# zju3dv/LoFTR

Measured on AMD Instinct MI355X. Metric: image-pairs/sec @640x480 indoor-ds, higher is better.
Workload: dtype f32; 1 GPU; batch=8 640x480 synthetic grayscale pairs per GPU, indoor_ds dual-softmax (BASELINE configs[1]), full LoFTR.forward = ResNet-FPN backbone (HIP implicit-GEMM / patch convolutions incl. the 7x7 stem) + HIP matching path; weights=seeded random init (no checkpoint on the box), conf_matrix_materialised=True, match_type=dual_softmax, global_batch=8, parallelism=dp1 (pairs sharded; RCCL all-gather of match counts)

## Files before the change

### include/loftr_hip.h

```cpp
#ifndef LOFTR_HIP_H_
#define LOFTR_HIP_H_

#include <stddef.h>
#include <stdint.h>

#ifdef __cplusplus
extern "C" {
#endif

typedef enum {
  LOFTR_OK = 0,
  LOFTR_ERR_BAD_ARG = -1,
  LOFTR_ERR_UNSUPPORTED = -2,
  LOFTR_ERR_WORKSPACE = -3,
  LOFTR_ERR_LAUNCH = -4,
  LOFTR_ERR_NO_DEVICE = -5,
  LOFTR_ERR_COMM = -6,
  LOFTR_ERR_RANGE = -7
} loftr_status;

#define LOFTR_HIP_ABI_VERSION 25

int loftr_hip_abi_version(void);
const char* loftr_hip_status_string(int status);
int loftr_hip_device_check(void);

typedef struct {
  const float* data;
  long sn, sc, sh, sw;
  int H, W;
} loftr_fmap;

int loftr_pos_encode_flatten(const loftr_fmap* feat, const float* pe, int pe_h, int pe_w,
                             float* out, int N, int C, void* stream);

typedef struct {
  const float* q_proj;
  const float* k_proj;
  const float* v_proj;
  const float* merge;
  const float* mlp0;
  const float* mlp2;
  const float* norm1_w;
  const float* norm1_b;
  const float* norm2_w;
  const float* norm2_b;
} loftr_layer_weights;

size_t loftr_encoder_workspace_bytes(int nb, int L, int S, int C);

int loftr_encoder_layer_fwd(const float* x, const float* source, const uint8_t* x_mask,
                            const uint8_t* source_mask, const loftr_layer_weights* w, float* out,
                            int nb, int L, int S, int C, int H, void* ws, size_t ws_bytes,
                            void* stream);

typedef struct {
  float* q_proj; float* k_proj; float* v_proj; float* merge; float* mlp0; float* mlp2;
  float* norm1_w; float* norm1_b; float* norm2_w; float* norm2_b;
} loftr_layer_grads;
size_t loftr_encoder_layer_bwd_workspace_bytes(int nb, int L, int S, int C, int H);
int loftr_encoder_layer_bwd(const float* x, const float* source, const uint8_t* x_mask, const uint8_t* source_mask,
                            const loftr_layer_weights* w, const float* grad_out, float* grad_x, float* grad_source,
                            const loftr_layer_grads* gw, int nb, int L, int S, int C, int H, void* ws, size_t ws_bytes,
                            void* stream);

int loftr_transformer_fwd(float* feat0, float* feat1, const uint8_t* mask0, const uint8_t* mask1,
                          const loftr_layer_weights* layers, const int* layer_is_cross,
                          int n_layers, int N, int L, int S, int C, int H, const void* prepared,
                          size_t prepared_bytes, void* ws, size_t ws_bytes, void* stream);
int loftr_transformer_fwd_padded(float* feat0, float* feat1, const uint8_t* mask0, const uint8_t* mask1,
                                 const loftr_layer_weights* layers, const int* layer_is_cross,
                                 int n_layers, int N, int L, int S, int C, int H, const void* prepared,
                                 size_t prepared_bytes, void* ws, size_t ws_bytes, int skip_padded_tiles, void* stream);
size_t loftr_coarse_plan_bytes(const int* layer_is_cross, int n_layers, int N, int L, int S);
int loftr_coarse_plan_build(const int* layer_is_cross, int n_layers, int N, int L, int S, int order, void* plan,
                            size_t plan_bytes, void* stream);
unsigned loftr_coarse_plan_signature(int n_layers, int N, int L, int S, int order);
int loftr_transformer_fwd_planned(float* feat0, float* feat1, const uint8_t* mask0, const uint8_t* mask1,
                                  const loftr_layer_weights* layers, const int* layer_is_cross,
                                  int n_layers, int N, int L, int S, int C, int H, const void* prepared,
                                  size_t prepared_bytes, void* ws, size_t ws_bytes, const void* plan,
                                  size_t plan_bytes, int plan_order, void* diag, size_t diag_bytes, void* stream);

size_t loftr_transformer_prepared_bytes(int n_layers, int C);
int loftr_transformer_prepare(const loftr_layer_weights* layers, int n_layers, int C, void* prepared,
                              size_t prepared_bytes, void* stream);

typedef struct {
  int N, h0c, w0c, h1c, w1c;
  int C;
  float thr;
  int border_rm;
  float scale;
  const uint8_t* mask0;
  const uint8_t* mask1;
  const float* scale0;
  const float* scale1;
} loftr_coarse_params;

typedef struct {
  int64_t* b_ids;
  int64_t* i_ids;
  int64_t* j_ids;
  float* mconf;
  float* mkpts0_c;
  float* mkpts1_c;
  int32_t* counts;
} loftr_match_out;

size_t loftr_coarse_match_workspace_bytes(int N, int L, int S, int C);

int loftr_coarse_match_dual_softmax(const float* feat_c0, const float* feat_c1,
                                    const loftr_coarse_params* p, float temperature,
                                    float* conf_out, const loftr_match_out* out, void* ws,
                                    size_t ws_bytes, void* stream);

int loftr_coarse_match_sinkhorn(const float* feat_c0, const float* feat_c1,
                                const loftr_coarse_params* p, float bin_score, int iters,
                                int prefilter, float* conf_out, float* assign_out,
                                const loftr_match_out* out, void* ws, size_t ws_bytes,
                                void* stream);


size_t loftr_fine_preprocess_workspace_bytes(int M, int W, int Cf);

int loftr_fine_preprocess(const loftr_fmap* feat_f0, const loftr_fmap* feat_f1,
                          const float* feat_c0, const float* feat_c1, int L, int S, int Cc,
                          const int64_t* b_ids, const int64_t* i_ids, const int64_t* j_ids, int M,
                          int w0c, int w1c, int stride, int W, int Cf,
                          const float* down_w, const float* down_b, const float* merge_w,
                          const float* merge_b, float* out0, float* out1, void* ws,
                          size_t ws_bytes, void* stream);

size_t loftr_fine_preprocess_bwd_workspace_bytes(int M, int W, int Cf, int Cc);
int loftr_fine_preprocess_bwd(const loftr_fmap* feat_f0, const loftr_fmap* feat_f1, const float* feat_c0, const float* feat_c1,
                              int L, int S, int Cc, const int64_t* b_ids, const int64_t* i_ids, const int64_t* j_ids, int M,
                              int w0c, int w1c, int stride, int W, int Cf, const float* down_w, const float* down_b,
                              const float* merge_w, const float* grad_out0, const float* grad_out1, const loftr_fmap* grad_f0,
                              const loftr_fmap* grad_f1, float* grad_c0, float* grad_c1, float* grad_down_w, float* grad_down_b,
                              float* grad_merge_w, float* grad_merge_b, void* ws, size_t ws_bytes, void* stream);

int loftr_pos_encode_flatten_gather(const loftr_fmap* bank, int n_slots, const int32_t* slot_ids, int n,
                                    const float* pe, int pe_h, int pe_w, float* out, int C, void* stream);

int loftr_fine_preprocess_gather(const loftr_fmap* bank_f0, int n_slots0, const int32_t* slot0,
                                 const loftr_fmap* bank_f1, int n_slots1, const int32_t* slot1,
                                 const float* feat_c0, const float* feat_c1, int L, int S, int Cc,
                                 const int64_t* b_ids, const int64_t* i_ids, const int64_t* j_ids, int M,
                                 int w0c, int w1c, int stride, int W, int Cf,
                                 const float* down_w, const float* down_b, const float* merge_w,
                                 const float* merge_b, float* out0, float* out1, void* ws,
                                 size_t ws_bytes, void* stream);

int loftr_window_head(const uint32_t* h_sp0, const uint32_t* h_sp1, int N, int H, int Wm, int Cin,
                      const void* prepared, size_t prepared_bytes, int Cout, const int64_t* b_ids,
                      const int64_t* i_ids, const int64_t* j_ids, int M, int w0c, int w1c, int stride, int W,
                      uint32_t* win0_sp, uint32_t* win1_sp, void* stream);
int loftr_fine_preprocess_window_head(const uint32_t* h_sp0, const uint32_t* h_sp1, int N, int H, int Wm, int Cin,
                                      const void* prepared, size_t prepared_bytes,
                                      const float* feat_c0, const float* feat_c1, int L, int S, int Cc,
                                      const int64_t* b_ids, const int64_t* i_ids, const int64_t* j_ids, int M,
                                      int w0c, int w1c, int stride, int W, int Cf,
                                      const float* down_w, const float* down_b, const float* merge_w,
                                      const float* merge_b, float* out0, float* out1, void* ws, size_t ws_bytes,
                                      void* stream);

int loftr_window_head_first(const uint32_t* t_sp0, const uint32_t* t_sp1, int N, int H, int Wm, int Cin,
                            const void* prepared, size_t prepared_bytes, int Cout, const int64_t* b_ids,
                            const int64_t* i_ids, const int64_t* j_ids, int M, int w0c, int w1c, int stride, int W,
                            uint32_t* nb_sp, void* stream);
int loftr_window_head_last(const uint32_t* nb_sp, int H, int Wm, int Cin, const void* prepared, size_t prepared_bytes,
                           int Cout, const int64_t* b_ids, const int64_t* i_ids, const int64_t* j_ids, int M, int w0c,
                           int w1c, int stride, int W, uint32_t* win0_sp, uint32_t* win1_sp, void* stream);
int loftr_fine_preprocess_window_head2(const uint32_t* t_sp0, const uint32_t* t_sp1, int N, int H, int Wm, int Cin,
                                       const void* prepared0, size_t prepared0_bytes, int Cmid,
                                       const void* prepared1, size_t prepared1_bytes,
                                       const float* feat_c0, const float* feat_c1, int L, int S, int Cc,
                                       const int64_t* b_ids, const int64_t* i_ids, const int64_t* j_ids, int M,
                                       int w0c, int w1c, int stride, int W, int Cf,
                                       const float* down_w, const float* down_b, const float* merge_w,
                                       const float* merge_b, float* out0, float* out1, void* ws, size_t ws_bytes,
                                       uint32_t* nb_sp, void* stream);

int loftr_fine_match(const float* feat_f0, const float* feat_f1, int M, int WW, int C,
                     const float* mkpts1_c, const int64_t* b_ids, float scale,
                     const float* scale1, float* expec_f, float* mkpts1_f, void* stream);

size_t loftr_conv_workspace_bytes(int Cin, int Cout, int KH, int KW);
int loftr_conv_bn_act(const uint32_t* x_sp, int B, int H, int W, int Cin, const float* weight,
                      const long* weight_strides, int Cout, int KH, int KW, int stride, int pad, const float* bn_weight, const float* bn_bias,
                      const float* bn_mean, const float* bn_var, float bn_eps, int act,
                      const uint32_t* residual_sp, uint32_t* y_sp, float* y_f32, void* ws, size_t ws_bytes,
                      const float* x_inv_scale, void* stream);
int loftr_conv_prepare(const float* weight, const long* weight_strides, int Cin, int Cout, int KH, int KW,
                       const float* bn_weight, const float* bn_bias, const float* bn_mean, const float* bn_var,
                       float bn_eps, void* prepared, size_t prepared_bytes, void* stream);
#define LOFTR_CONV_SHARED_GPU 0x100
int loftr_conv_bn_act_prepared(const uint32_t* x_sp, int B, int H, int W, int Cin, const void* prepared,
                               size_t prepared_bytes, int Cout, int KH, int KW, int stride, int pad, int act,
                               const uint32_t* residual_sp, const uint32_t* low_sp, uint32_t* y_sp, float* y_f32,
                               const float* x_inv_scale, void* stream);
size_t loftr_conv_scratch_bytes(int B, int H, int W, int Cout, int KH, int KW, int stride);
int loftr_conv_bn_act_prepared_scratch(const uint32_t* x_sp, int B, int H, int W, int Cin, const void* prepared,
                                       size_t prepared_bytes, int Cout, int KH, int KW, int stride, int pad, int act,
                                       const uint32_t* residual_sp, const uint32_t* low_sp, uint32_t* y_sp, float* y_f32,
                                       const float* x_inv_scale, void* scratch, size_t scratch_bytes, void* stream);
int loftr_stem_conv_bn_relu(const float* x, const long* x_strides, int B, int H, int W, const float* weight,
                            const long* weight_strides, int C0, const float* bn_weight, const float* bn_bias,
                            const float* bn_mean, const float* bn_var, float bn_eps, uint32_t* y_sp, void* stream);
int loftr_upsample2x_add(const uint32_t* low_sp, const uint32_t* lateral_sp, uint32_t* out_sp, int B, int Hl,
                         int Wl, int C, void* stream);
int loftr_conv1x1_upsample_add(const uint32_t* x_sp, int B, int H, int W, int Cin, const float* weight,
                               const long* weight_strides, int Cout, const uint32_t* low_sp, uint32_t* y_sp,
                               void* ws, size_t ws_bytes, void* stream);
int loftr_sp_from_f32(const float* src, uint32_t* dst_sp, long rows, int C, void* stream);
int loftr_sp_from_f32_scaled(const float* src, uint32_t* dst_sp, long rows, int C, float* inv_scale_out, void* stream);
int loftr_sp_to_f32(const uint32_t* src_sp, float* dst, long rows, int C, void* stream);

int loftr_epipolar_errors(const float* mkpts0_f, const float* mkpts1_f, const long* m_bids, const float* T_0to1,
                          const float* K0, const float* K1, long M, int N, float* epi_errs, void* stream);

typedef struct {
  int N, H0, W0, H1, W1, scale;
  int dh0, dw0, dh1, dw1;
  const float* depth0; const float* depth1;
  const float* T_0to1; const float* T_1to0;
  const float* K0; const float* K1;
  const float* scale0; const float* scale1;
  const uint8_t* mask0; const uint8_t* mask1;
} loftr_spvs_params;
size_t loftr_spvs_coarse_workspace_bytes(int N, int L, int S);
int loftr_spvs_coarse(const loftr_spvs_params* p, float* w_pt0_i, float* pt1_i, int64_t* spv_b, int64_t* spv_i, int64_t* spv_j,
                      int32_t* count, float* conf_gt, void* ws, size_t ws_bytes, void* stream);
int loftr_spvs_fine(const float* w_pt0_i, const float* pt1_i, int L, int S, const int64_t* b_ids, const int64_t* i_ids,
                    const int64_t* j_ids, long M, float scale, float radius, const float* scale1, float* expec_f_gt, void* stream);
size_t loftr_loss_workspace_bytes(int N, int L, int S);
int loftr_coarse_loss_sums(const float* conf, int N, int L, int S, int kind, const int64_t* gt_b, const int64_t* gt_i,
                           const int64_t* gt_j, long M, const uint8_t* mask0, const uint8_t* mask1, float alpha, float gamma,
                           double* sums, void* ws, size_t ws_bytes, void* stream);
int loftr_fine_loss_sums(const float* expec_f, int ld, const float* expec_f_gt, long M, int with_std, float correct_thr,
                         double* sums, void* ws, size_t ws_bytes, void* stream);

int loftr_coarse_loss_grad(const float* conf, int N, int L, int S, int kind, const int64_t* gt_b, const int64_t* gt_i,
                           const int64_t* gt_j, long M, const uint8_t* mask0, const uint8_t* mask1, float alpha, float gamma,
                           double pos_scale, double neg_scale, float* grad_conf, void* ws, size_t ws_bytes, void* stream);
int loftr_fine_loss_grad(const float* expec_f, int ld, const float* expec_f_gt, long M, int with_std, float correct_thr,
                         int training, const double* sums, float upstream, float* grad_expec, void* stream);
int loftr_dual_softmax_bwd(const float* feat_c0, const float* feat_c1, const loftr_coarse_params* p, float temperature,
                           const float* grad_conf, float* dsim, void* ws, size_t ws_bytes, void* stream);
int loftr_fine_match_bwd(const float* feat_f0, const float* feat_f1, int M, int WW, int C, const float* grad_expec,
                         float* grad_f0, float* grad_f1, void* stream);
int loftr_head_feat_grads(const float* dsim, long dsim_ld, long dsim_bs, const float* feat_c0, const float* feat_c1,
                          int N, int L, int S, int C, float alpha, float* g0, float* g1, void* stream);
size_t loftr_conv_wgrad_workspace_bytes(int B, int Ho, int Wo, int Cin, int Cout, int KH, int KW);
int loftr_conv_wgrad(const float* dy, const float* x, int B, int H, int W, int Cin, int Cout, int KH, int KW, int stride, int pad,
                     float* dw_taps, void* ws, size_t ws_bytes, void* stream);
size_t loftr_sinkhorn_bwd_workspace_bytes(int N, int L, int S, int C, int iters);
int loftr_sinkhorn_bwd(const float* feat_c0, const float* feat_c1, const loftr_coarse_params* p, float bin_score, int iters,
                       const float* grad_assign, float* z_scratch, float* dZ, float* dbin, void* ws, size_t ws_bytes, void* stream);

int loftr_estimate_pose(const float* kpts0, const float* kpts1, long M, const float* K0, const float* K1, float thresh_px,
                        float conf, unsigned seed, float* R_out, float* t_out, uint8_t* inliers_out, long* n_inliers);
int loftr_five_point(const double* q0, const double* q1, int n, double* E_out, int* n_solutions);

size_t loftr_estimate_pose_batched_workspace_bytes(long M, int P);
int loftr_estimate_pose_batched(const float* mkpts0_f, const float* mkpts1_f, const long* m_bids, long M, const float* K0,
                                const float* K1, int P, float thresh_px, float conf, unsigned seed, float* R_out, float* t_out,
                                uint8_t* inliers_out, long* n_inliers, void* ws, size_t ws_bytes, void* stream);

int loftr_estimate_geometry(const float* kpts0, const float* kpts1, long M, int model, float thresh_px, float conf, unsigned seed,
                            float* mat_out, uint8_t* inliers_out, long* n_inliers);
int loftr_geometry_minimal(const double* p0, const double* p1, int model, double* mats_out, int* n_solutions);

size_t loftr_estimate_geometry_batched_workspace_bytes(long M, int P, int model);
int loftr_estimate_geometry_batched(const float* mkpts0_f, const float* mkpts1_f, const long* m_bids, long M, int P, int model,
                                    float thresh_px, float conf, unsigned seed, float* mat_out, uint8_t* inliers_out,
                                    long* n_inliers, void* ws, size_t ws_bytes, void* stream);

int loftr_estimate_absolute_pose(const float* pts3d, const float* kpts, long M, const float* K, float thresh_px, float conf, unsigned seed,
                                 float* R_out, float* t_out, uint8_t* inliers_out, long* n_inliers);
int loftr_p3p(const double* X, const double* bearings, double* R_out, double* t_out, int* n_solutions);

size_t loftr_estimate_absolute_pose_batched_workspace_bytes(long M, int P);
int loftr_estimate_absolute_pose_batched(const float* pts3d, const float* kpts, const long* m_bids, long M, const float* K, int P,
                                         float thresh_px, float conf, unsigned seed, float* R_out, float* t_out, uint8_t* inliers_out,
                                         long* n_inliers, void* ws, size_t ws_bytes, void* stream);

int loftr_lift_keypoints(const float* kpts, const long* m_bids, long M, const float* depth, int dh, int dw, const float* K, const float* T,
                         int P, float* pts3d_out, uint8_t* valid_out, void* stream);

typedef struct {
  long* kp_offsets; float* keypoints; float* score; int* n_obs;
  long* row_offsets; int* matches; float* match_conf;
  int* track_id; int* track_len; uint8_t* track_ok; long* counts;
} LoftrAtlasOut;

int loftr_atlas_host(const float* kpts0, const float* kpts1, const float* conf, const int* rows, const uint8_t* mask, long M,
                     const int* row_images, long R, int n_images, int gh, int gw, float inv, int min_track_len, const LoftrAtlasOut* out);

int loftr_atlas_observe(const float* kpts0, const float* kpts1, const float* conf, const long* m_bids, const uint8_t* mask, long n,
                        int n_rows, long match_base, long row_base, const int* row_images, int n_images, int gh, int gw, float inv,
                        unsigned long long* grid, float* obs_xy, int* obs_cell, float* m_conf, int* m_row, uint8_t* m_reason, int* status,
                        void* stream);

#define LOFTR_ATLAS_STAGES 7
size_t loftr_atlas_finalize_workspace_bytes(long M, int n_images, int gh, int gw);
int loftr_atlas_finalize(unsigned long long* grid, const float* obs_xy, const int* obs_cell, const float* m_conf, const int* m_row,
                         const uint8_t* m_reason, long M, long R, int n_images, int gh, int gw, int min_track_len, const int* status,
                         const LoftrAtlasOut* out, void* ws, size_t ws_bytes, float* stage_ms, void* stream);

int loftr_triangulate_tracks_host(const long* offsets, long T, const int* obs_image, const float* obs_xy, long N, const double* K,
                                  const double* T_cam_from_world, int n_images, double thresh_px, double cos_min_angle, float* xyz,
                                  int* n_inliers, float* rms_px, float* tri_cos, uint8_t* status, uint8_t* obs_inlier, long* counts);
int loftr_triangulation_pairs(int L, int* pairs, int* n);
#define LOFTR_TRIANGULATE_STAGES 3
size_t loftr_triangulate_tracks_workspace_bytes(long T, long N, int n_images);
int loftr_triangulate_tracks(const long* offsets, long T, const int* obs_image, const float* obs_xy, long N, const double* K,
                             const double* T_cam_from_world, int n_images, double thresh_px, double cos_min_angle, float* xyz,
                             int* n_inliers, float* rms_px, float* tri_cos, uint8_t* status, uint8_t* obs_inlier, long* counts, int group,
                             void* ws, size_t ws_bytes, float* stage_ms, void* stream);

typedef struct {
  const long* kp_offsets; const int* kp_cell; const int* kp_point; const float* xyz;
  long K, P;
  int n_images, gh, gw;
  float inv;
} LoftrModel;
typedef struct {
  float* pts3d; float* kpts; long* q_ids; int* match; int* point; float* conf;
  long* q_offsets; uint8_t* match_reason; long* counts;
} LoftrModelLookupOut;

int loftr_model_cells_host(const long* kp_offsets, int n_images, const float* keypoints, const int* kp_point, long K, long P, int gh, int gw,
                           float inv, int* kp_cell, int* status);
int loftr_model_cells(const long* kp_offsets, int n_images, const float* keypoints, const int* kp_point, long K, long P, int gh, int gw,
                      float inv, int* kp_cell, int* status, void* stream);

int loftr_model_lookup_host(const LoftrModel* model, const float* kpts_db, const float* kpts_q, const float* conf, const int* rows,
                            const uint8_t* mask, long M, const int* row_db, const int* row_query, long R, long Q,
                            const LoftrModelLookupOut* out);
#define LOFTR_MODEL_LOOKUP_STAGES 3
size_t loftr_model_lookup_workspace_bytes(long M, long Q);
int loftr_model_lookup(const LoftrModel* model, const float* kpts_db, const float* kpts_q, const float* conf, const int* rows,
                       const uint8_t* mask, long M, const int* row_db, const int* row_query, long R, long Q, const LoftrModelLookupOut* out,
                       void* ws, size_t ws_bytes, float* stage_ms, void* stream);

#define LOFTR_BUNDLE_MAX_ITERS 1000
#define LOFTR_BUNDLE_MAX_PCG 200
int loftr_bundle_adjust_host(const long* offsets, long T, const int* obs_image, const float* obs_xy, const uint8_t* obs_mask, long N,
                             const float* xyz, const double* K, const double* T_cam_from_world, const uint8_t* fixed, int n_images,
                             const long* cam_offsets, const int* cam_obs, double huber_px, int max_iters, int pcg_iters, double pcg_tol,
                             double ftol, double* T_out, float* xyz_out, uint8_t* obs_active, uint8_t* cam_free, uint8_t* point_active,
                             long* counts);
#define LOFTR_BUNDLE_CLASSES 11
size_t loftr_bundle_adjust_workspace_bytes(long T, long N, int n_images);
int loftr_bundle_adjust(const long* offsets, long T, const int* obs_image, const float* obs_xy, const uint8_t* obs_mask, long N,
                        const float* xyz, const double* K, const double* T_cam_from_world, const uint8_t* fixed, int n_images,
                        const long* cam_offsets, const int* cam_obs, double huber_px, int max_iters, int pcg_iters, double pcg_tol,
                        double ftol, double* T_out, float* xyz_out, uint8_t* obs_active, uint8_t* cam_free, uint8_t* point_active,
                        long* counts, void* ws, size_t ws_bytes, float* class_ms, long* class_launches, void* stream);

int loftr_register_corr_host(const long* offsets, long T, const int* obs_image, const float* obs_xy, long N, const float* xyz,
                             const uint8_t* status, const uint8_t* posed, int n_images, const long* cam_offsets, const int* cam_obs,
                             int min_corr, int* n_corr, int* cand_rank, int* cand_image, long* cand_offsets, float* corr_xyz, float* corr_xy,
                             long* corr_bid, int* corr_obs, long* counts);
#define LOFTR_REGISTER_STAGES 4
#define LOFTR_REGISTER_RANK_BLOCK 256
size_t loftr_register_corr_workspace_bytes(long T, long N, int n_images);
int loftr_register_corr(const long* offsets, long T, const int* obs_image, const float* obs_xy, long N, const float* xyz,
                        const uint8_t* status, const uint8_t* posed, int n_images, const long* cam_offsets, const int* cam_obs,
                        int min_corr, int* n_corr, int* cand_rank, int* cand_image, long* cand_offsets, float* corr_xyz, float* corr_xy,
                        long* corr_bid, int* corr_obs, long* counts, void* ws, size_t ws_bytes, float* stage_ms, void* stream);

size_t loftr_bn_train_workspace_bytes(int N, int C, long HW);
int loftr_bn_train_fwd(const float* x, int N, int C, long HW, int channels_last, const float* gamma, const float* beta, float eps, float* y,
                       float* mean, float* invstd, float* var_unbiased, void* ws, size_t ws_bytes, void* stream);
int loftr_bn_train_bwd(const float* dy, const float* x, int N, int C, long HW, int channels_last, const float* mean, const float* invstd,
                       const float* gamma, float* dx, float* dgamma, float* dbeta, void* ws, size_t ws_bytes, void* stream);
int loftr_act_fwd(const float* a, const float* b, long n, int act, float slope, float* y, void* stream);
int loftr_act_bwd(const float* dy, const float* y, long n, int act, float slope, float* dx, void* stream);
int loftr_upsample2x_bilinear_fwd(const float* x, int N, int C, int H, int W, int channels_last, float* y, void* stream);
int loftr_upsample2x_bilinear_bwd(const float* dy, int N, int C, int H, int W, int channels_last, float* dx, void* stream);

int loftr_resize_linear_u8(const uint8_t* src, int sh, int sw, long src_pitch, uint8_t* dst, int dh, int dw,
                           long dst_pitch, void* stream);
// ... 29 lines not shown
```

### loftr_amd/_lib.py

```python
import ctypes as C
import os

HERE = os.path.dirname(os.path.abspath(__file__))
LIB_PATH = os.environ.get("LOFTR_HIP_LIB") or os.path.join(HERE, "libloftr_hip.so")

_p = C.c_void_p
_i = C.c_int
_f = C.c_float
_sz = C.c_size_t
_l = C.c_long


class LayerWeights(C.Structure):
    _fields_ = [(n, _p) for n in ("q_proj", "k_proj", "v_proj", "merge", "mlp0", "mlp2",
                                  "norm1_w", "norm1_b", "norm2_w", "norm2_b")]


class CoarseParams(C.Structure):
    _fields_ = [("N", _i), ("h0c", _i), ("w0c", _i), ("h1c", _i), ("w1c", _i), ("C", _i),
                ("thr", _f), ("border_rm", _i), ("scale", _f),
                ("mask0", _p), ("mask1", _p), ("scale0", _p), ("scale1", _p)]


class MatchOut(C.Structure):
    _fields_ = [(n, _p) for n in ("b_ids", "i_ids", "j_ids", "mconf", "mkpts0_c", "mkpts1_c", "counts")]


class SpvsParams(C.Structure):
    _fields_ = [(n, _i) for n in ("N", "H0", "W0", "H1", "W1", "scale", "dh0", "dw0", "dh1", "dw1")] + \
               [(n, _p) for n in ("depth0", "depth1", "T_0to1", "T_1to0", "K0", "K1", "scale0", "scale1", "mask0", "mask1")]


class FMap(C.Structure):
    _fields_ = [("data", _p), ("sn", _l), ("sc", _l), ("sh", _l), ("sw", _l), ("H", _i), ("W", _i)]


class AtlasOut(C.Structure):
    _fields_ = [(n, _p) for n in ("kp_offsets", "keypoints", "score", "n_obs", "row_offsets", "matches", "match_conf",
                                  "track_id", "track_len", "track_ok", "counts")]


class Model(C.Structure):
    _fields_ = [(n, _p) for n in ("kp_offsets", "kp_cell", "kp_point", "xyz")] + [("K", _l), ("P", _l), ("n_images", _i), ("gh", _i), ("gw", _i),
                                                                                   ("inv", _f)]


class ModelLookupOut(C.Structure):
    _fields_ = [(n, _p) for n in ("pts3d", "kpts", "q_ids", "match", "point", "conf", "q_offsets", "match_reason", "counts")]


SIGNATURES = {
    "loftr_hip_abi_version": (_i, []),
    "loftr_hip_status_string": (C.c_char_p, [_i]),
    "loftr_hip_device_check": (_i, []),
    "loftr_pos_encode_flatten": (_i, [C.POINTER(FMap), _p, _i, _i, _p, _i, _i, _p]),
    "loftr_encoder_workspace_bytes": (_sz, [_i, _i, _i, _i]),
    "loftr_encoder_layer_fwd": (_i, [_p, _p, _p, _p, C.POINTER(LayerWeights), _p, _i, _i, _i, _i, _i, _p, _sz, _p]),
    "loftr_encoder_layer_bwd_workspace_bytes": (_sz, [_i, _i, _i, _i, _i]),
    "loftr_encoder_layer_bwd": (_i, [_p, _p, _p, _p, C.POINTER(LayerWeights), _p, _p, _p, C.POINTER(LayerWeights), _i, _i, _i, _i, _i, _p, _sz, _p]),
    "loftr_transformer_fwd": (_i, [_p, _p, _p, _p, C.POINTER(LayerWeights), C.POINTER(_i), _i, _i, _i, _i, _i, _i,
                                   _p, _sz, _p, _sz, _p]),
    "loftr_transformer_fwd_padded": (_i, [_p, _p, _p, _p, C.POINTER(LayerWeights), C.POINTER(_i), _i, _i, _i, _i, _i, _i,
                                          _p, _sz, _p, _sz, _i, _p]),
    "loftr_coarse_plan_bytes": (_sz, [C.POINTER(_i), _i, _i, _i, _i]),
    "loftr_coarse_plan_build": (_i, [C.POINTER(_i), _i, _i, _i, _i, _i, _p, _sz, _p]),
    "loftr_coarse_plan_signature": (C.c_uint, [_i, _i, _i, _i, _i]),
    "loftr_transformer_fwd_planned": (_i, [_p, _p, _p, _p, C.POINTER(LayerWeights), C.POINTER(_i), _i, _i, _i, _i, _i, _i,
                                           _p, _sz, _p, _sz, _p, _sz, _i, _p, _sz, _p]),
    "loftr_hip_debug_set": (_i, [C.c_char_p, _i]),
    "loftr_hip_debug_get": (_i, [C.c_char_p, C.POINTER(_i), C.POINTER(_i)]),
    "loftr_transformer_prepared_bytes": (_sz, [_i, _i]),
    "loftr_transformer_prepare": (_i, [C.POINTER(LayerWeights), _i, _i, _p, _sz, _p]),
    "loftr_coarse_match_workspace_bytes": (_sz, [_i, _i, _i, _i]),
    "loftr_coarse_match_dual_softmax": (_i, [_p, _p, C.POINTER(CoarseParams), _f, _p, C.POINTER(MatchOut), _p, _sz, _p]),
    "loftr_coarse_match_sinkhorn": (_i, [_p, _p, C.POINTER(CoarseParams), _f, _i, _i, _p, _p, C.POINTER(MatchOut),
                                         _p, _sz, _p]),
    "loftr_fine_preprocess_workspace_bytes": (_sz, [_i, _i, _i]),
    "loftr_fine_preprocess": (_i, [C.POINTER(FMap), C.POINTER(FMap), _p, _p, _i, _i, _i, _p, _p, _p, _i, _i, _i, _i,
                                   _i, _i, _p, _p, _p, _p, _p, _p, _p, _sz, _p]),
    "loftr_fine_preprocess_bwd_workspace_bytes": (_sz, [_i, _i, _i, _i]),
    "loftr_fine_preprocess_bwd": (_i, [C.POINTER(FMap), C.POINTER(FMap), _p, _p, _i, _i, _i, _p, _p, _p, _i, _i, _i, _i, _i, _i,
                                       _p, _p, _p, _p, _p, C.POINTER(FMap), C.POINTER(FMap), _p, _p, _p, _p, _p, _p, _p, _sz, _p]),
    "loftr_fine_match": (_i, [_p, _p, _i, _i, _i, _p, _p, _f, _p, _p, _p, _p]),
    "loftr_pos_encode_flatten_gather": (_i, [C.POINTER(FMap), _i, _p, _i, _p, _i, _i, _p, _i, _p]),
    "loftr_fine_preprocess_gather": (_i, [C.POINTER(FMap), _i, _p, C.POINTER(FMap), _i, _p, _p, _p, _i, _i, _i, _p, _p, _p, _i, _i, _i, _i,
                                          _i, _i, _p, _p, _p, _p, _p, _p, _p, _sz, _p]),
    "loftr_window_head": (_i, [_p, _p, _i, _i, _i, _i, _p, _sz, _i, _p, _p, _p, _i, _i, _i, _i, _i, _p, _p, _p]),
    "loftr_fine_preprocess_window_head": (_i, [_p, _p, _i, _i, _i, _i, _p, _sz, _p, _p, _i, _i, _i, _p, _p, _p, _i, _i, _i, _i,
                                               _i, _i, _p, _p, _p, _p, _p, _p, _p, _sz, _p]),
    "loftr_window_head_first": (_i, [_p, _p, _i, _i, _i, _i, _p, _sz, _i, _p, _p, _p, _i, _i, _i, _i, _i, _p, _p]),
    "loftr_window_head_last": (_i, [_p, _i, _i, _i, _p, _sz, _i, _p, _p, _p, _i, _i, _i, _i, _i, _p, _p, _p]),
    "loftr_fine_preprocess_window_head2": (_i, [_p, _p, _i, _i, _i, _i, _p, _sz, _i, _p, _sz, _p, _p, _i, _i, _i, _p, _p, _p, _i, _i, _i,
                                                _i, _i, _i, _p, _p, _p, _p, _p, _p, _p, _sz, _p, _p]),
    "loftr_conv_workspace_bytes": (_sz, [_i, _i, _i, _i]),
    "loftr_conv_bn_act": (_i, [_p, _i, _i, _i, _i, _p, C.POINTER(_l), _i, _i, _i, _i, _i, _p, _p, _p, _p, _f, _i, _p, _p, _p, _p, _sz, _p, _p]),
    "loftr_stem_conv_bn_relu": (_i, [_p, C.POINTER(_l), _i, _i, _i, _p, C.POINTER(_l), _i, _p, _p, _p, _p, _f, _p, _p]),
    "loftr_upsample2x_add": (_i, [_p, _p, _p, _i, _i, _i, _i, _p]),
    "loftr_bn_train_workspace_bytes": (_sz, [_i, _i, _l]),
    "loftr_bn_train_fwd": (_i, [_p, _i, _i, _l, _i, _p, _p, _f, _p, _p, _p, _p, _p, _sz, _p]),
    "loftr_bn_train_bwd": (_i, [_p, _p, _i, _i, _l, _i, _p, _p, _p, _p, _p, _p, _p, _sz, _p]),
    "loftr_act_fwd": (_i, [_p, _p, _l, _i, _f, _p, _p]),
    "loftr_act_bwd": (_i, [_p, _p, _l, _i, _f, _p, _p]),
    "loftr_upsample2x_bilinear_fwd": (_i, [_p, _i, _i, _i, _i, _i, _p, _p]),
    "loftr_upsample2x_bilinear_bwd": (_i, [_p, _i, _i, _i, _i, _i, _p, _p]),
    "loftr_resize_linear_u8": (_i, [_p, _i, _i, _l, _p, _i, _i, _l, _p]),
    "loftr_pack_gray_u8": (_i, [_p, _l, _l, _p, _i, _i, _i, _p, _p, _p, _i, _p]),
    "loftr_epipolar_errors": (_i, [_p, _p, _p, _p, _p, _p, _l, _i, _p, _p]),
    "loftr_spvs_coarse_workspace_bytes": (_sz, [_i, _i, _i]),
    "loftr_spvs_coarse": (_i, [C.POINTER(SpvsParams), _p, _p, _p, _p, _p, _p, _p, _p, _sz, _p]),
    "loftr_spvs_fine": (_i, [_p, _p, _i, _i, _p, _p, _p, _l, _f, _f, _p, _p, _p]),
    "loftr_loss_workspace_bytes": (_sz, [_i, _i, _i]),
    "loftr_coarse_loss_sums": (_i, [_p, _i, _i, _i, _i, _p, _p, _p, _l, _p, _p, _f, _f, _p, _p, _sz, _p]),
    "loftr_fine_loss_sums": (_i, [_p, _i, _p, _l, _i, _f, _p, _p, _sz, _p]),
    "loftr_coarse_loss_grad": (_i, [_p, _i, _i, _i, _i, _p, _p, _p, _l, _p, _p, _f, _f, C.c_double, C.c_double, _p, _p, _sz, _p]),
    "loftr_conv_wgrad_workspace_bytes": (_sz, [_i, _i, _i, _i, _i, _i, _i]),
    "loftr_conv_wgrad": (_i, [_p, _p, _i, _i, _i, _i, _i, _i, _i, _i, _i, _p, _p, _sz, _p]),
    "loftr_head_feat_grads": (_i, [_p, C.c_long, C.c_long, _p, _p, _i, _i, _i, _i, _f, _p, _p, _p]),
    "loftr_sinkhorn_bwd_workspace_bytes": (_sz, [_i, _i, _i, _i, _i]),
    "loftr_sinkhorn_bwd": (_i, [_p, _p, C.POINTER(CoarseParams), _f, _i, _p, _p, _p, _p, _p, _sz, _p]),
    "loftr_fine_loss_grad": (_i, [_p, _i, _p, _l, _i, _f, _i, _p, _f, _p, _p]),
    "loftr_dual_softmax_bwd": (_i, [_p, _p, C.POINTER(CoarseParams), _f, _p, _p, _p, _sz, _p]),
    "loftr_fine_match_bwd": (_i, [_p, _p, _i, _i, _i, _p, _p, _p, _p]),
    "loftr_estimate_pose": (_i, [_p, _p, _l, _p, _p, _f, _f, C.c_uint, _p, _p, _p, C.POINTER(_l)]),
    "loftr_five_point": (_i, [_p, _p, _i, _p, C.POINTER(_i)]),
    "loftr_estimate_pose_batched_workspace_bytes": (_sz, [_l, _i]),
    "loftr_estimate_pose_batched": (_i, [_p, _p, _p, _l, _p, _p, _i, _f, _f, C.c_uint, _p, _p, _p, _p, _p, _sz, _p]),
    "loftr_estimate_geometry": (_i, [_p, _p, _l, _i, _f, _f, C.c_uint, _p, _p, C.POINTER(_l)]),
    "loftr_geometry_minimal": (_i, [_p, _p, _i, _p, C.POINTER(_i)]),
    "loftr_estimate_geometry_batched_workspace_bytes": (_sz, [_l, _i, _i]),
    "loftr_estimate_geometry_batched": (_i, [_p, _p, _p, _l, _i, _i, _f, _f, C.c_uint, _p, _p, _p, _p, _sz, _p]),
    "loftr_estimate_absolute_pose": (_i, [_p, _p, _l, _p, _f, _f, C.c_uint, _p, _p, _p, C.POINTER(_l)]),
    "loftr_p3p": (_i, [_p, _p, _p, _p, C.POINTER(_i)]),
    "loftr_estimate_absolute_pose_batched_workspace_bytes": (_sz, [_l, _i]),
    "loftr_estimate_absolute_pose_batched": (_i, [_p, _p, _p, _l, _p, _i, _f, _f, C.c_uint, _p, _p, _p, _p, _p, _sz, _p]),
    "loftr_lift_keypoints": (_i, [_p, _p, _l, _p, _i, _i, _p, _p, _i, _p, _p, _p]),
    "loftr_atlas_host": (_i, [_p, _p, _p, _p, _p, _l, _p, _l, _i, _i, _i, _f, _i, C.POINTER(AtlasOut)]),
    "loftr_atlas_observe": (_i, [_p, _p, _p, _p, _p, _l, _i, _l, _l, _p, _i, _i, _i, _f, _p, _p, _p, _p, _p, _p, _p, _p]),
    "loftr_atlas_finalize_workspace_bytes": (_sz, [_l, _i, _i, _i]),
    "loftr_atlas_finalize": (_i, [_p, _p, _p, _p, _p, _p, _l, _l, _i, _i, _i, _i, _p, C.POINTER(AtlasOut), _p, _sz, _p, _p]),
    "loftr_triangulate_tracks_host": (_i, [_p, _l, _p, _p, _l, _p, _p, _i, C.c_double, C.c_double, _p, _p, _p, _p, _p, _p, _p]),
    "loftr_triangulation_pairs": (_i, [_i, _p, C.POINTER(_i)]),
    "loftr_triangulate_tracks_workspace_bytes": (_sz, [_l, _l, _i]),
    "loftr_triangulate_tracks": (_i, [_p, _l, _p, _p, _l, _p, _p, _i, C.c_double, C.c_double, _p, _p, _p, _p, _p, _p, _p, _i, _p, _sz, _p, _p]),
    "loftr_model_cells_host": (_i, [_p, _i, _p, _p, _l, _l, _i, _i, _f, _p, _p]),
    "loftr_model_cells": (_i, [_p, _i, _p, _p, _l, _l, _i, _i, _f, _p, _p, _p]),
    "loftr_model_lookup_host": (_i, [C.POINTER(Model), _p, _p, _p, _p, _p, _l, _p, _p, _l, _l, C.POINTER(ModelLookupOut)]),
    "loftr_model_lookup_workspace_bytes": (_sz, [_l, _l]),
    "loftr_model_lookup": (_i, [C.POINTER(Model), _p, _p, _p, _p, _p, _l, _p, _p, _l, _l, C.POINTER(ModelLookupOut), _p, _sz, _p, _p]),
    "loftr_bundle_adjust_host": (_i, [_p, _l, _p, _p, _p, _l, _p, _p, _p, _p, _i, _p, _p, C.c_double, _i, _i, C.c_double, C.c_double,
                                      _p, _p, _p, _p, _p, _p]),
    "loftr_bundle_adjust_workspace_bytes": (_sz, [_l, _l, _i]),
    "loftr_bundle_adjust": (_i, [_p, _l, _p, _p, _p, _l, _p, _p, _p, _p, _i, _p, _p, C.c_double, _i, _i, C.c_double, C.c_double,
                                 _p, _p, _p, _p, _p, _p, _p, _sz, _p, _p, _p]),
    "loftr_register_corr_host": (_i, [_p, _l, _p, _p, _l, _p, _p, _p, _i, _p, _p, _i, _p, _p, _p, _p, _p, _p, _p, _p, _p]),
    "loftr_register_corr_workspace_bytes": (_sz, [_l, _l, _i]),
    "loftr_register_corr": (_i, [_p, _l, _p, _p, _l, _p, _p, _p, _i, _p, _p, _i, _p, _p, _p, _p, _p, _p, _p, _p, _p, _p, _sz, _p, _p]),
    "loftr_conv_prepare": (_i, [_p, C.POINTER(_l), _i, _i, _i, _i, _p, _p, _p, _p, _f, _p, _sz, _p]),
    "loftr_conv_bn_act_prepared": (_i, [_p, _i, _i, _i, _i, _p, _sz, _i, _i, _i, _i, _i, _i, _p, _p, _p, _p, _p, _p]),
    "loftr_conv_scratch_bytes": (_sz, [_i, _i, _i, _i, _i, _i, _i]),
    "loftr_conv_bn_act_prepared_scratch": (_i, [_p, _i, _i, _i, _i, _p, _sz, _i, _i, _i, _i, _i, _i, _p, _p, _p, _p, _p, _p, _sz, _p]),
    "loftr_conv1x1_upsample_add": (_i, [_p, _i, _i, _i, _i, _p, C.POINTER(_l), _i, _p, _p, _p, _sz, _p]),
    "loftr_sp_from_f32": (_i, [_p, _p, _l, _i, _p]),
    "loftr_sp_from_f32_scaled": (_i, [_p, _p, _l, _i, _p, _p]),
    "loftr_sp_to_f32": (_i, [_p, _p, _l, _i, _p]),
    "loftr_rccl_unique_id": (_i, [C.c_char_p, _sz]),
    "loftr_rccl_comm_create": (_i, [C.c_char_p, _sz, _i, _i, C.POINTER(_p)]),
    "loftr_rccl_comm_info": (_i, [_p, C.POINTER(_i), C.POINTER(_i)]),
    "loftr_rccl_comm_destroy": (_i, [_p]),
    "loftr_rccl_allgather_counts": (_i, [_p, _p, _p, _i, _p]),
    "loftr_hip_timing_enable": (_i, [C.c_uint]),
    "loftr_hip_range_check_enable": (_i, [_i]),
    "loftr_hip_timing_kernel_count": (_i, []),
    "loftr_hip_timing_kernel_name": (C.c_char_p, [_i]),
    "loftr_hip_timing_read": (_i, [_i, C.POINTER(C.c_double), C.POINTER(C.c_longlong), _i]),
    "loftr_linear_workspace_bytes": (_sz, [_i, _i, _i]),
    "loftr_linear_fwd": (_i, [_p, _p, _p, _i, _i, _i, _p, _sz, _p]),
}

ABI_VERSION = 25
_lib = None


class LoftrHipError(RuntimeError):
    pass


def load():
    global _lib
    if _lib is not None:
        return _lib
    if not os.path.exists(LIB_PATH):
        raise LoftrHipError(
            f"{LIB_PATH} not found: the HIP extension is not built. Run `python -m loftr_amd.build` "
            "(needs hipcc). There is no CPU / PyTorch fallback for the matching path.")
    lib = C.CDLL(LIB_PATH)
    for name, (res, args) in SIGNATURES.items():
        fn = getattr(lib, name, None)
        if fn is None:
            raise LoftrHipError(f"{LIB_PATH} does not export {name}: it predates this binding; rebuild "
                                "(`python -m loftr_amd.build --force`)")
        fn.restype = res
        fn.argtypes = args
    if lib.loftr_hip_abi_version() != ABI_VERSION:
        raise LoftrHipError(f"ABI mismatch: library {lib.loftr_hip_abi_version()} != binding {ABI_VERSION}; rebuild")
    _lib = lib
    return lib


def check(status, what=""):
    if status != 0:
        msg = load().loftr_hip_status_string(status).decode()
        raise LoftrHipError(f"{what or 'libloftr_hip'} failed: {msg} (status {status})")
```

### loftr_amd/csrc/coarse_plan.h

```cpp
#pragma once
#include "gemm.h"

struct PctItem { uint32_t what; uint32_t signal; uint32_t dep[4]; uint32_t sig2[2]; };
constexpr uint32_t PCT_NODEP = 0xffffffffu;
constexpr int PCT_X = 0, PCT_K = 1, PCT_F = 2;
constexpr int PCT_MAX_LAYERS = 8, PCT_MAX_CALLS = 2 * PCT_MAX_LAYERS, PCT_TILE = 128, PCT_CNT0 = 4;
constexpr int PCT_MAX_PAIRS = 256, PCT_MAX_TILES = 4095;

struct PctShape {
  int n_layers, N, T[2];
  int n_calls() const { return 2 * n_layers; }
  int tiles(int img) const { return (T[img] + PCT_TILE - 1) / PCT_TILE; }
  int gmax() const { return tiles(0) > tiles(1) ? tiles(0) : tiles(1); }
  uint32_t xflag(int c, int p, int g) const { return (uint32_t)(PCT_CNT0 + (c * N + p) * gmax() + g); }
  uint32_t kcnt(int c, int p) const { return (uint32_t)(PCT_CNT0 + n_calls() * N * gmax() + c * N + p); }
  uint32_t fcnt(int c, int p) const { return kcnt(c, p) + (uint32_t)(n_calls() * N); }
  size_t n_counters() const { return (size_t)PCT_CNT0 + (size_t)n_calls() * N * (gmax() + 2); }
  void call(int c, int& layer, int& x_img, int& s_img) const {
    const int i = c / 4, k = c % 4;
    layer = 2 * i + (k >= 2); x_img = k & 1; s_img = k < 2 ? (k & 1) : 1 - (k & 1);
  }
  bool standalone_k(int c) const { return c < 2; }
  int folds(int c, int (&out)[2]) const {
    const int k = c % 4;
    int n = 0;
    if (k == 1) out[n++] = c + 1;
    if (k == 2) { out[n++] = c + 1; if (c + 2 < n_calls()) out[n++] = c + 2; }
    if (k == 3 && c + 2 < n_calls()) out[n++] = c + 2;
    for (int i = n; i < 2; ++i) out[i] = -1;
    return n;
  }
  size_t n_items() const {
    size_t n = 0;
    for (int c = 0; c < n_calls(); ++c) { int l, x, s; call(c, l, x, s); n += (size_t)N * ((standalone_k(c) ? tiles(s) : 0) + 8 + tiles(x)); }
    return n;
  }
  uint32_t signature(int order) const {
    uint32_t h = 0x9e3779b9u ^ 7u;
    for (uint32_t v : {(uint32_t)n_layers, (uint32_t)N, (uint32_t)T[0], (uint32_t)T[1], (uint32_t)order}) h = (h ^ v) * 0x01000193u + 0x7ed55d16u;
    return h | 1u;
  }
  bool ok() const {
    return n_layers >= 2 && n_layers % 2 == 0 && n_layers <= PCT_MAX_LAYERS && N >= 1 && N <= PCT_MAX_PAIRS && T[0] >= 1 && T[1] >= 1 &&
           gmax() <= PCT_MAX_TILES && n_counters() < (1u << 20);
  }
};
inline size_t pct_plan_bytes(const PctShape& s) { return (1 + s.n_items()) * sizeof(PctItem); }
inline size_t pct_ws_bytes(const PctShape& s) {
  const size_t cp = (size_t)s.n_calls() * s.N;
  return align_up(s.n_counters() * 4, 256) + align_up(cp * 8 * s.gmax() * 33 * 32 * 4, 256) + align_up(cp * 8 * 33 * 32 * 4, 256) +
         align_up(cp * 65536 * 4, 256) + 1024;
}

struct PctLayerPtrs {
  const sp_t *wq, *w0, *w2, *wkv;
  const float *wq_s, *w0_s, *w2_s, *wkv_s, *merge_f32, *g1, *b1, *g2, *b2;
};
struct PctLaunch {
  PctShape shape;
  float* f32[2]; sp_t* sp[2]; const uint8_t* mask[2];
  PctLayerPtrs layer[PCT_MAX_LAYERS];
  const void* plan; size_t plan_bytes; unsigned plan_signature;
  void* ws; size_t ws_bytes;
  unsigned* status;
  unsigned long long* trace;
};
int launch_coarse_persistent(const PctLaunch& p, hipStream_t st);
```

### loftr_amd/csrc/encoder_fused.hip

```cpp
#include "linear.h"
#include "attention.h"
#include "coarse_plan.h"

namespace {
namespace efx {
#ifndef EFX_NST
#define EFX_NST 4
#endif
#ifndef EFX_PROBE_DMA
#define EFX_PROBE_DMA 1
#endif
#ifndef EFX_PROBE_BARRIER
#define EFX_PROBE_BARRIER 1
#endif
#ifndef EFX_PROBE_EPI
#define EFX_PROBE_EPI 1
#endif
constexpr int W = 4, PT = 32, STAGE = 32 * 1024, NST = EFX_NST, BLK = 4096;
constexpr int NPANEL = 16 + 48;
constexpr int DMA_PER_WAVE = 8;
constexpr int T_WQS = 0, T_KSUM = 256, T_G1 = 512, T_B1 = 768, T_W0S = 1024, T_W2S = 1536, T_G2 = 1792, T_B2 = 2048, T_N = 2304;
constexpr int OFF_TAB = NST * STAGE;
constexpr int LDS_BYTES = OFF_TAB + T_N * 4;
static_assert(LDS_BYTES <= 160 * 1024, "one workgroup per CU");

struct Args {
  const sp_t* x_sp; const float* x_f32;
  float* out_f32; sp_t* out_sp;
  const sp_t* wq; const sp_t* pm; long pm_seq_stride;
  const sp_t* w0; const sp_t* w2;
  const float *wq_s, *w0_s, *w2_s;
  const float* kv;
  const uint8_t* mask;
  const float *g1, *b1, *g2, *b2;
  float v_length, attn_eps, p_out_scale, ln_eps;
  int nseq, T, groups;
  int xsplit, gpc;
  int skip_padded;
};

typedef __attribute__((address_space(3))) void* lds_ptr_t;
typedef const __attribute__((address_space(1))) void* gbl_ptr_t;

__device__ __forceinline__ void swap_halves(uint32_t& a, uint32_t& b) {
  const auto r = __builtin_amdgcn_permlane32_swap(a, b, false, false);
  a = r[0]; b = r[1];
}
__device__ __forceinline__ void sp_pack4(float x0, float x1, float x2, float x3, uint2& hi, uint2& lo) {
  sp_pack2(x0, x1, hi.x, lo.x);
  sp_pack2(x2, x3, hi.y, lo.y);
}
__device__ __forceinline__ void pack_panel(const float (&v)[16], h16x8 (&fh)[2], h16x8 (&fl)[2]) {
  if (!EFX_PROBE_EPI) {
    fh[0] = __builtin_bit_cast(h16x8, f32x4{v[0], v[1], v[2], v[3]}); fl[0] = __builtin_bit_cast(h16x8, f32x4{v[4], v[5], v[6], v[7]});
    fh[1] = __builtin_bit_cast(h16x8, f32x4{v[8], v[9], v[10], v[11]}); fl[1] = __builtin_bit_cast(h16x8, f32x4{v[12], v[13], v[14], v[15]});
    return;
  }
  uint2 H[4], L[4];
#pragma unroll
  for (int q = 0; q < 4; ++q) sp_pack4(v[4 * q], v[4 * q + 1], v[4 * q + 2], v[4 * q + 3], H[q], L[q]);
#pragma unroll
  for (int s = 0; s < 2; ++s) {
    swap_halves(H[2 * s].x, H[2 * s + 1].x); swap_halves(H[2 * s].y, H[2 * s + 1].y);
    swap_halves(L[2 * s].x, L[2 * s + 1].x); swap_halves(L[2 * s].y, L[2 * s + 1].y);
    fh[s] = __builtin_bit_cast(h16x8, u32x4{H[2 * s].x, H[2 * s].y, H[2 * s + 1].x, H[2 * s + 1].y});
    fl[s] = __builtin_bit_cast(h16x8, u32x4{L[2 * s].x, L[2 * s].y, L[2 * s + 1].x, L[2 * s + 1].y});
  }
}

__device__ __forceinline__ const sp_t* uniform_ptr(const sp_t* p) {
  const unsigned long long v = (unsigned long long)(size_t)p;
  const unsigned lo = (unsigned)__builtin_amdgcn_readfirstlane((int)(unsigned)v), hi = (unsigned)__builtin_amdgcn_readfirstlane((int)(unsigned)(v >> 32));
  return reinterpret_cast<const sp_t*>((size_t)(((unsigned long long)hi << 32) | lo));
}

__device__ __forceinline__ bool job_tile(const Args& a, const int id, int& seq, int& grp) {
  const int xcd = id % NUM_XCD, slot = id / NUM_XCD;
  const int vs = (slot / a.gpc) * NUM_XCD + xcd;
  seq = vs / a.xsplit; grp = (slot % a.gpc) * a.xsplit + vs % a.xsplit;
  return seq < a.nseq && grp < a.groups;
}

struct KvTile {
  const sp_t* x_sp; const uint8_t* mask; int T;
  const sp_t* wkv; const float* wkv_s;
  float inv_s;
  float* part; long head_stride;
};
struct FoldArgs { int n; KvTile k[2]; };
__device__ __forceinline__ void kv_tile_main(const KvTile& a, char* const lds, const h16x8 (&xh)[16], const h16x8 (&xl)[16],
                                             const float (&mk)[16], const bool live, const int nlive);

template <bool FOLD>
__device__ __forceinline__ void encoder_x_body(const Args& a, const int seq, const int grp, char* const lds, const FoldArgs* fa = nullptr) {
  const int lane = threadIdx.x & 63, wave = threadIdx.x >> 6, g = lane >> 5, li = lane & 31;
  const int T = a.T;
  if constexpr (!FOLD) {
    if (a.skip_padded && a.mask && a.out_f32 == a.x_f32 && a.out_sp == a.x_sp) {
      const int t = grp * W * PT + (int)threadIdx.x;
      const bool valid = (int)threadIdx.x < W * PT && t < T && a.mask[(long)seq * T + t] != 0;
      if (!__syncthreads_or(valid)) return;
    }
  }
  const int tok = (grp * W + wave) * PT + li;
  const bool live = (grp * W + wave) * PT < T;
  const long row = (long)seq * T + min(tok, T - 1);
  float* tab = reinterpret_cast<float*>(lds + OFF_TAB);

  for (int f = threadIdx.x; f < 256; f += W * 64) {
    tab[T_WQS + f] = a.wq_s[f];
    tab[T_KSUM + f] = a.kv[((long)seq * 8 + (f >> 5)) * (33 * 32) + 32 * 32 + (f & 31)];
    tab[T_G1 + f] = a.g1[f]; tab[T_B1 + f] = a.b1[f];
    tab[T_W0S + f] = a.w0_s[f]; tab[T_W0S + 256 + f] = a.w0_s[256 + f];
    tab[T_W2S + f] = a.w2_s[f];
    tab[T_G2 + f] = a.g2[f]; tab[T_B2 + f] = a.b2[f];
  }
  h16x8 xh[16], xl[16];
  {
    const u32x4* src = reinterpret_cast<const u32x4*>(a.x_sp + row * 256);
#pragma unroll
    for (int ks = 0; ks < 16; ++ks) {
      const int c = (ks >> 1) * 8 + 2 * (ks & 1) + g;
      xh[ks] = __builtin_bit_cast(h16x8, src[c]);
      xl[ks] = __builtin_bit_cast(h16x8, src[c + 4]);
    }
  }
  const float mk = (a.mask && !a.mask[row]) ? 0.f : 1.f;

  const sp_t* pm = a.pm + (long)seq * a.pm_seq_stride;
  unsigned doff[4];
#pragma unroll
  for (int oct = 0; oct < 4; ++oct) doff[oct] = ((unsigned)(oct * 8 + (lane >> 3)) * 256u + ((((unsigned)lane & 7u) ^ ((unsigned)(oct * 4 + (lane >> 4)) & 7u)) << 2)) * 4u;
  const unsigned drl = (unsigned)(lane >> 3) * 1024u;
  const int wave_s = __builtin_amdgcn_readfirstlane(wave);
#define EFX_ISSUE_SRC(p_, base_, pitch_, kt_)                                                              \
  {                                                                                                        \
    char* st__ = lds + ((p_) % NST) * STAGE;                                                               \
    const unsigned w512__ = (pitch_) == 512 ? 1u : 0u;                                                     \
    _Pragma("unroll") for (int bi__ = 0; bi__ < 2; ++bi__) {                                               \
      const int b__ = wave_s + 4 * bi__;                                                                   \
      const char* bb__ = reinterpret_cast<const char*>(uniform_ptr((kt_) ? (base_) + (long)b__ * 32 * (pitch_) : (base_) + b__ * 32)); \
      _Pragma("unroll") for (int oct__ = 0; oct__ < 4; ++oct__) {                                          \
        const char* bo__ = bb__ + (size_t)(w512__ * (unsigned)(oct__ * 8192));                             \
        asm volatile("" : "+s"(bo__));                   \
        __builtin_amdgcn_global_load_lds((gbl_ptr_t)(bo__ + (doff[oct__] + w512__ * drl)),                 \
                                         (lds_ptr_t)(st__ + b__ * BLK + oct__ * 1024), 16, 0, 0);          \
      }                                                                                                    \
    }                                                                                                      \
  }
#define EFX_ISSUE(p_)                                                                                      \
  {                                                                                                        \
    const int p__ = (p_);                                                                                  \
    const sp_t* base__; int pitch__; bool kt__;                                                            \
    if (p__ < 16) {                                                                                        \
      const int h__ = p__ >> 1;                                                                            \
      if (p__ & 1) { base__ = pm + h__ * 32; pitch__ = 256; kt__ = true; }                                 \
      else { base__ = a.wq + (long)h__ * 32 * 256; pitch__ = 256; kt__ = false; }                          \
    } else {                                                                                               \
      const int q__ = p__ - 16, hp__ = q__ / 3, i__ = q__ - 3 * hp__;                                      \
      if (i__ == 2) { base__ = a.w2 + hp__ * 32; pitch__ = 512; kt__ = true; }                             \
      else { base__ = a.w0 + (long)hp__ * 32 * 512 + i__ * 256; pitch__ = 512; kt__ = false; }             \
    }                                                                                                      \
    EFX_ISSUE_SRC(p__, base__, pitch__, kt__)                                                              \
  }
#define EFX_BEGIN_G(p_, NP_, ISSUE_)                                                                       \
  {                                                                                                        \
    if (!EFX_PROBE_DMA) LOFTR_WAITCNT_VM(0);                                                               \
    else if (NST >= 4 && (p_) + 2 < (NP_)) LOFTR_WAITCNT_VM(2 * DMA_PER_WAVE);                             \
    else if ((p_) + 1 < (NP_)) LOFTR_WAITCNT_VM(DMA_PER_WAVE);                                             \
    else LOFTR_WAITCNT_VM(0);                                                                              \
    if (EFX_PROBE_BARRIER) __builtin_amdgcn_s_barrier();                                                   \
    if (EFX_PROBE_DMA && (p_) + NST - 1 < (NP_)) ISSUE_((p_) + NST - 1);                                   \
  }
#define EFX_BEGIN(p_) EFX_BEGIN_G(p_, NPANEL, EFX_ISSUE)
  const int a_off = lds_chunk_off(li, g);
#define EFX_RD(st_, blk_, odd_, lo_) (*reinterpret_cast<const h16x8*>((st_) + (blk_) * BLK + (a_off ^ (((odd_) ? 32 : 0) | ((lo_) ? 64 : 0)))))
#define EFX_USE(a_, b_, c_, d_) asm volatile("" :: "v"(a_), "v"(b_), "v"(c_), "v"(d_))
#define EFX_RPANEL_G(st_, bh_, bl_, MF_)                                                                   \
  {                                                                                                        \
    h16x8 eh__ = EFX_RD(st_, 0, 0, 0), el__ = EFX_RD(st_, 0, 0, 1), oh__ = EFX_RD(st_, 0, 1, 0), ol__ = EFX_RD(st_, 0, 1, 1);\
    _Pragma("unroll") for (int u = 0; u < 8; ++u) {                                                        \
      EFX_USE(eh__, el__, oh__, ol__);                                                                     \
      __builtin_amdgcn_sched_barrier(0);                                                                   \
      h16x8 neh__ = eh__, nel__ = el__, noh__ = oh__, nol__ = ol__;                                        \
      acc0 = MF_(eh__, bl_[2 * u], acc0);                                                                  \
      __builtin_amdgcn_sched_barrier(0);                                                                   \
      if (u + 1 < 8) { neh__ = EFX_RD(st_, u + 1, 0, 0); nel__ = EFX_RD(st_, u + 1, 0, 1); }               \
      __builtin_amdgcn_sched_barrier(0);                                                                   \
      acc0 = MF_(el__, bh_[2 * u], acc0);                                                                  \
      __builtin_amdgcn_sched_barrier(0);                                                                   \
      if (u + 1 < 8) { noh__ = EFX_RD(st_, u + 1, 1, 0); nol__ = EFX_RD(st_, u + 1, 1, 1); }               \
      __builtin_amdgcn_sched_barrier(0);                                                                   \
      acc0 = MF_(eh__, bh_[2 * u], acc0);                                                                  \
      acc0 = MF_(oh__, bl_[2 * u + 1], acc0);                                                              \
      acc0 = MF_(ol__, bh_[2 * u + 1], acc0);                                                              \
      acc0 = MF_(oh__, bh_[2 * u + 1], acc0);                                                              \
      __builtin_amdgcn_sched_barrier(0);                                                                   \
      eh__ = neh__; el__ = nel__; oh__ = noh__; ol__ = nol__;                                              \
    }                                                                                                      \
  }
#define EFX_MF_N(w_, x_, c_) __builtin_amdgcn_mfma_f32_32x32x16_f16(w_, x_, c_, 0, 0, 0)
#define EFX_MF_T(w_, x_, c_) __builtin_amdgcn_mfma_f32_32x32x16_f16(x_, w_, c_, 0, 0, 0)
#define EFX_RPANEL(st_, bh_, bl_) EFX_RPANEL_G(st_, bh_, bl_, EFX_MF_N)
#define EFX_KPANEL(st_, fh_, fl_, out_)                                                                    \
  {                                                                                                        \
    h16x8 ah__ = EFX_RD(st_, 0, 0, 0), al__ = EFX_RD(st_, 0, 0, 1), bh__ = EFX_RD(st_, 1, 0, 0), bl__ = EFX_RD(st_, 1, 0, 1); \
    _Pragma("unroll") for (int u = 0; u < 8; ++u) {                                                        \
      const int j2 = u >> 1, s = u & 1;                                                                    \
      const int nj = (u + 1) >> 1, ns = (u + 1) & 1;                                                       \
      EFX_USE(ah__, al__, bh__, bl__);                                                                     \
      __builtin_amdgcn_sched_barrier(0);                                                                   \
      h16x8 nah__ = ah__, nal__ = al__, nbh__ = bh__, nbl__ = bl__;                                        \
      out_[2 * j2] = __builtin_amdgcn_mfma_f32_32x32x16_f16(ah__, fl_[s], out_[2 * j2], 0, 0, 0);          \
      __builtin_amdgcn_sched_barrier(0);                                                                   \
      if (u + 1 < 8) { nah__ = EFX_RD(st_, 2 * nj, ns, 0); nal__ = EFX_RD(st_, 2 * nj, ns, 1); }           \
      __builtin_amdgcn_sched_barrier(0);                                                                   \
      out_[2 * j2 + 1] = __builtin_amdgcn_mfma_f32_32x32x16_f16(bh__, fl_[s], out_[2 * j2 + 1], 0, 0, 0);  \
      __builtin_amdgcn_sched_barrier(0);                                                                   \
      if (u + 1 < 8) { nbh__ = EFX_RD(st_, 2 * nj + 1, ns, 0); nbl__ = EFX_RD(st_, 2 * nj + 1, ns, 1); }   \
      __builtin_amdgcn_sched_barrier(0);                                                                   \
      out_[2 * j2] = __builtin_amdgcn_mfma_f32_32x32x16_f16(al__, fh_[s], out_[2 * j2], 0, 0, 0);          \
      out_[2 * j2 + 1] = __builtin_amdgcn_mfma_f32_32x32x16_f16(bl__, fh_[s], out_[2 * j2 + 1], 0, 0, 0);  \
      out_[2 * j2] = __builtin_amdgcn_mfma_f32_32x32x16_f16(ah__, fh_[s], out_[2 * j2], 0, 0, 0);          \
      out_[2 * j2 + 1] = __builtin_amdgcn_mfma_f32_32x32x16_f16(bh__, fh_[s], out_[2 * j2 + 1], 0, 0, 0);  \
      __builtin_amdgcn_sched_barrier(0);                                                                   \
      ah__ = nah__; al__ = nal__; bh__ = nbh__; bl__ = nbl__;                                              \
    }                                                                                                      \
  }

  LOFTR_WAITCNT_VM(0);
  __syncthreads();
  EFX_ISSUE(0);
  EFX_ISSUE(1);
  if (NST >= 4) EFX_ISSUE(2);

  const int fq = 4 * g;
  f32x16 acc0;
  f32x16 big[8];
#pragma unroll
  for (int j = 0; j < 8; ++j)
#pragma unroll
    for (int r = 0; r < 16; ++r) big[j][r] = 0.f;

#pragma unroll 1
  for (int h = 0; h < 8; ++h) {
    const int p = 2 * h;
    EFX_BEGIN(p);
    h16x8 qh[2], ql[2];
    if (live) {
      const char* st = lds + (p % NST) * STAGE;
#pragma unroll
      for (int r = 0; r < 16; ++r) acc0[r] = 0.f;
      EFX_RPANEL(st, xh, xl);
      float v[16];
      float den = 0.f;
#pragma unroll
      for (int q = 0; q < 4; ++q) {
        const f32x4 ws = *reinterpret_cast<const f32x4*>(tab + T_WQS + 32 * h + fq + 8 * q);
        const f32x4 ks4 = *reinterpret_cast<const f32x4*>(tab + T_KSUM + 32 * h + fq + 8 * q);
#pragma unroll
        for (int e = 0; e < 4; ++e) {
          float x = acc0[4 * q + e] * ws[e];
          if (EFX_PROBE_EPI) x = x > 0.f ? x + 1.f : __expf(x);
          x *= mk;
          v[4 * q + e] = x;
          den = fmaf(x, ks4[e], den);
        }
      }
      den += swap32(den);
      const float z = den == 0.f ? 0.f : a.v_length * __builtin_amdgcn_rcpf(den + a.attn_eps);
#pragma unroll
      for (int r = 0; r < 16; ++r) v[r] *= z;
      pack_panel(v, qh, ql);
    }
    EFX_BEGIN(p + 1);
    if (live) {
      const char* st = lds + ((p + 1) % NST) * STAGE;
      EFX_KPANEL(st, qh, ql, big);
    }
  }
  h16x8 mh[16], ml[16];
  if (live) {
    const float ps = a.p_out_scale;
    float s = 0.f;
#pragma unroll
    for (int j = 0; j < 8; ++j)
#pragma unroll
      for (int r = 0; r < 16; ++r) s += big[j][r];
    s += swap32(s);
    const float mean_a = s * (1.f / 256.f);
    float m2 = 0.f;
#pragma unroll
    for (int j = 0; j < 8; ++j)
#pragma unroll
      for (int r = 0; r < 16; ++r) { const float d = big[j][r] - mean_a; m2 = fmaf(d, d, m2); }
    m2 += swap32(m2);
    const float rstd = ps * rsqrtf(ps * ps * m2 * (1.f / 256.f) + a.ln_eps);
    const float mean = mean_a;
#pragma unroll
    for (int j = 0; j < 8; ++j) {
      float y[16];
#pragma unroll
      for (int q = 0; q < 4; ++q) {
        const f32x4 ga = *reinterpret_cast<const f32x4*>(tab + T_G1 + 32 * j + fq + 8 * q);
        const f32x4 be = *reinterpret_cast<const f32x4*>(tab + T_B1 + 32 * j + fq + 8 * q);
#pragma unroll
        for (int e = 0; e < 4; ++e) y[4 * q + e] = (big[j][4 * q + e] - mean) * rstd * ga[e] + be[e];
      }
      h16x8 fh[2], fl[2];
      pack_panel(y, fh, fl);
      mh[2 * j] = fh[0]; mh[2 * j + 1] = fh[1]; ml[2 * j] = fl[0]; ml[2 * j + 1] = fl[1];
    }
  }
#pragma unroll
  for (int j = 0; j < 8; ++j)
#pragma unroll
    for (int r = 0; r < 16; ++r) big[j][r] = 0.f;

#define EFX_PASS2_HEAD(hp_)                                                                                \
    const int p = 16 + 3 * (hp_);                                                                          \
    h16x8 hh[2], hl[2];                                                                                    \
    EFX_BEGIN(p);                                                                                          \
    if (live) {                                                                                            \
      _Pragma("unroll") for (int r = 0; r < 16; ++r) acc0[r] = 0.f;                     \
      EFX_RPANEL(lds + (p % NST) * STAGE, xh, xl);                                                                 \
    }                                                                                                      \
    EFX_BEGIN(p + 1);                                                                                      \
    if (live) {                                                                                            \
      EFX_RPANEL(lds + ((p + 1) % NST) * STAGE, mh, ml);                                                                 \
      float v[16];                                                                                         \
      _Pragma("unroll") for (int q = 0; q < 4; ++q) {                                                      \
        const f32x4 ws = *reinterpret_cast<const f32x4*>(tab + T_W0S + 32 * (hp_) + fq + 8 * q);           \
        _Pragma("unroll") for (int e = 0; e < 4; ++e)                                                      \
          v[4 * q + e] = fmaxf(acc0[4 * q + e] * ws[e], 0.f);    \
      }                                                                                                    \
      pack_panel(v, hh, hl);                                                                               \
    }                                                                                                      \
    EFX_BEGIN(p + 2);
#pragma unroll 1
  for (int hp = 0; hp < 16; ++hp) {
    EFX_PASS2_HEAD(hp)
    if (live) EFX_KPANEL(lds + ((p + 2) % NST) * STAGE, hh, hl, big);
  }
#undef EFX_PASS2_HEAD

  if (!FOLD && !live) return;
  if (live) {
    float s = 0.f;
#pragma unroll
    for (int j = 0; j < 8; ++j)
#pragma unroll
      for (int q = 0; q < 4; ++q) {
        const f32x4 ws = *reinterpret_cast<const f32x4*>(tab + T_W2S + 32 * j + fq + 8 * q);
#pragma unroll
        for (int e = 0; e < 4; ++e) s = fmaf(big[j][4 * q + e], ws[e], s);
      }
    s += swap32(s);
    const float mean = s * (1.f / 256.f);
    float m2 = 0.f;
    asm volatile("" ::: "memory");
#pragma unroll
    for (int j = 0; j < 8; ++j)
#pragma unroll
      for (int q = 0; q < 4; ++q) {
        const f32x4 ws = *reinterpret_cast<const f32x4*>(tab + T_W2S + 32 * j + fq + 8 * q);
#pragma unroll
        for (int e = 0; e < 4; ++e) { const float d = big[j][4 * q + e] * ws[e] - mean; m2 = fmaf(d, d, m2); }
      }
    m2 += swap32(m2);
    const float rstd = rsqrtf(m2 * (1.f / 256.f) + a.ln_eps);
    asm volatile("" ::: "memory");
    const bool in_seq = tok < T;
    if (FOLD || in_seq) {
      const float* xr = a.x_f32 + row * 256;
      float* of = a.out_f32 + row * 256;
      sp_t* os = a.out_sp + row * 256;
      f32x4 xn[4];
#pragma unroll
      for (int q = 0; q < 4; ++q) xn[q] = *reinterpret_cast<const f32x4*>(xr + fq + 8 * q);
#pragma unroll
      for (int j = 0; j < 8; ++j) {
        f32x4 xc[4];
#pragma unroll
        for (int q = 0; q < 4; ++q) xc[q] = xn[q];
        if (j + 1 < 8) {
#pragma unroll
          for (int q = 0; q < 4; ++q) xn[q] = *reinterpret_cast<const f32x4*>(xr + 32 * (j + 1) + fq + 8 * q);
        }
        float y[16];
#pragma unroll
        for (int q = 0; q < 4; ++q) {
          const int f = 32 * j + fq + 8 * q;
          const f32x4 ga = *reinterpret_cast<const f32x4*>(tab + T_G2 + f);
          const f32x4 be = *reinterpret_cast<const f32x4*>(tab + T_B2 + f);
          const f32x4 ws = *reinterpret_cast<const f32x4*>(tab + T_W2S + f);
          f32x4 o;
#pragma unroll
          for (int e = 0; e < 4; ++e) {
            o[e] = xc[q][e] + ((big[j][4 * q + e] * ws[e] - mean) * rstd * ga[e] + be[e]);
            y[4 * q + e] = o[e];
          }
          if (!FOLD || in_seq) *reinterpret_cast<f32x4*>(of + f) = o;
        }
        if (!FOLD && !a.out_sp) continue;
        h16x8 fh[2], fl[2];
        pack_panel(y, fh, fl);
        if (FOLD) { xh[2 * j] = fh[0]; xh[2 * j + 1] = fh[1]; xl[2 * j] = fl[0]; xl[2 * j + 1] = fl[1]; }
        if (!FOLD || in_seq) {
#pragma unroll
          for (int s2 = 0; s2 < 2; ++s2) {
            *reinterpret_cast<u32x4*>(os + j * 32 + (2 * s2 + g) * 4) = __builtin_bit_cast(u32x4, fh[s2]);
            *reinterpret_cast<u32x4*>(os + j * 32 + 16 + (2 * s2 + g) * 4) = __builtin_bit_cast(u32x4, fl[s2]);
          }
        }
      }
    }
  }
  if constexpr (FOLD) {
    if (fa->n > 0) {
      const int tok0 = (grp * W + wave) * PT;
      const int nlive = min(W, (T - grp * W * PT + PT - 1) / PT);
      float mk[16];
#pragma unroll
      for (int r = 0; r < 16; ++r) {
        const int t = tok0 + (r & 3) + 8 * (r >> 2) + 4 * g;
        mk[r] = (t < T && (!a.mask || a.mask[(long)seq * T + min(t, T - 1)])) ? 1.f : 0.f;
      }
#pragma unroll 1
      for (int s = 0; s < fa->n; ++s) kv_tile_main(fa->k[s], lds, xh, xl, mk, live, nlive);
    }
  }
}

__global__ __launch_bounds__(W * 64, 1) void encoder_x_kernel(Args a) {
  __shared__ __attribute__((aligned(16))) char lds[LDS_BYTES];
  int seq, grp;
  if (job_tile(a, blockIdx.x, seq, grp)) encoder_x_body<false>(a, seq, grp, lds);
}

struct Args2 { Args j[2]; int n0, off0, off1; };
__global__ __launch_bounds__(W * 64, 1) void encoder_x2_kernel(Args2 m) {
  __shared__ __attribute__((aligned(16))) char lds[LDS_BYTES];
  const bool second = (int)blockIdx.x >= m.n0;
  const Args* a = second ? &m.j[1] : &m.j[0];
  int seq, grp;
  if (job_tile(*a, second ? (int)blockIdx.x - m.n0 + m.off1 : (int)blockIdx.x + m.off0, seq, grp)) encoder_x_body<false>(*a, seq, grp, lds);
}

struct PctCall { int layer, x_img, s_img, pad, fold[2], pad2[2]; };
struct PctArgs {
  float* f32[2]; sp_t* sp[2]; const uint8_t* mask[2]; int T[2];
  int N, n_calls, n_items, splits;
  const PctItem* items; unsigned* cnt;
  float* part; float* kv; sp_t* pm;
  unsigned long long* trace;
  unsigned* status;
  unsigned signature; int skip;
  int quota;
  PctLayerPtrs layer[PCT_MAX_LAYERS]; PctCall call[PCT_MAX_CALLS];
};
constexpr int OFF_RED = OFF_TAB + T_N * 4, RED_FLOATS = 33 * 32, OFF_CTRL = OFF_RED + W * RED_FLOATS * 4, LDS_BYTES_P = OFF_CTRL + 64;
static_assert(LDS_BYTES_P <= 160 * 1024, "one workgroup per CU");

__device__ __forceinline__ void kv_tile_body(const KvTile& a, const int tile, char* const lds) {
  const int lane = threadIdx.x & 63, wave = threadIdx.x >> 6, g = lane >> 5, li = lane & 31;
  const int T = a.T;
  const int tok0 = (tile * W + wave) * PT;
  const bool live = tok0 < T;
  const int nlive = min(W, (T - tile * W * PT + PT - 1) / PT);
  h16x8 xh[16], xl[16];
  {
    const u32x4* src = reinterpret_cast<const u32x4*>(a.x_sp + (long)min(tok0 + li, T - 1) * 256);
#pragma unroll
    for (int ks = 0; ks < 16; ++ks) {
      const int c = (ks >> 1) * 8 + 2 * (ks & 1) + g;
      xh[ks] = __builtin_bit_cast(h16x8, src[c]);
      xl[ks] = __builtin_bit_cast(h16x8, src[c + 4]);
    }
  }
  float mk[16];
#pragma unroll
  for (int r = 0; r < 16; ++r) {
    const int t = tok0 + (r & 3) + 8 * (r >> 2) + 4 * g;
    mk[r] = (t < T && (!a.mask || a.mask[min(t, T - 1)])) ? 1.f : 0.f;
  }
  kv_tile_main(a, lds, xh, xl, mk, live, nlive);
}

__device__ __forceinline__ void kv_tile_main(const KvTile& a, char* const lds, const h16x8 (&xh)[16], const h16x8 (&xl)[16],
                                             const float (&mk)[16], const bool live, const int nlive) {
  const int lane = threadIdx.x & 63, wave = threadIdx.x >> 6, g = lane >> 5, li = lane & 31;
  float* tab = reinterpret_cast<float*>(lds + OFF_TAB);
  LOFTR_WAITCNT_VM(0);
  __syncthreads();
  for (int f = threadIdx.x; f < 512; f += W * 64) tab[T_W0S + f] = a.wkv_s[f];
  unsigned doff[4];
#pragma unroll
  for (int oct = 0; oct < 4; ++oct) doff[oct] = ((unsigned)(oct * 8 + (lane >> 3)) * 256u + ((((unsigned)lane & 7u) ^ ((unsigned)(oct * 4 + (lane >> 4)) & 7u)) << 2)) * 4u;
  [[maybe_unused]] const unsigned drl = 0u;
  const int wave_s = __builtin_amdgcn_readfirstlane(wave);
  const int a_off = lds_chunk_off(li, g);
  const sp_t* const wkv = a.wkv;
#define KVX_ISSUE(p_) EFX_ISSUE_SRC((p_), wkv + (long)(p_) * 32 * 256, 256, false)
  const unsigned red_w = (unsigned)(size_t)(lds_ptr_t)(lds + OFF_RED) + (unsigned)((wave * RED_FLOATS + 4 * g * 32 + li) * 4);
  const char* red_r = lds + OFF_RED;
#define KVX_REDUCE(h_)                                                                                     \
  if (wave == ((h_) & 3)) {                                                                                \
    float* out__ = a.part + (long)(h_) * a.head_stride;                                                    \
    _Pragma("unroll") for (int u = 0; u < 5; ++u) {                                                        \
      const int v__ = lane + u * 64;                                                                       \
      if (v__ < RED_FLOATS / 4) {                                                                          \
        f32x4 s__ = *reinterpret_cast<const f32x4*>(red_r + v__ * 16);                                     \
        if (nlive > 1) s__ += *reinterpret_cast<const f32x4*>(red_r + 1 * RED_FLOATS * 4 + v__ * 16);     \
        if (nlive > 2) s__ += *reinterpret_cast<const f32x4*>(red_r + 2 * RED_FLOATS * 4 + v__ * 16);     \
        if (nlive > 3) s__ += *reinterpret_cast<const f32x4*>(red_r + 3 * RED_FLOATS * 4 + v__ * 16);     \
        reinterpret_cast<f32x4*>(out__)[v__] = s__;                                                        \
      }                                                                                                    \
    }                                                                                                      \
  }
  LOFTR_WAITCNT_VM(0);
  __syncthreads();
  KVX_ISSUE(0);
  KVX_ISSUE(1);
  if (NST >= 4) KVX_ISSUE(2);
  f32x16 acc0, acck;
#pragma unroll 1
  for (int h = 0; h < 8; ++h) {
    const int p = 2 * h;
    EFX_BEGIN_G(p, 16, KVX_ISSUE);
    if (h > 0) KVX_REDUCE(h - 1)
    if (live) {
#pragma unroll
      for (int r = 0; r < 16; ++r) acc0[r] = 0.f;
      EFX_RPANEL_G(lds + (p % NST) * STAGE, xh, xl, EFX_MF_T);
      acck = acc0;
    }
    EFX_BEGIN_G(p + 1, 16, KVX_ISSUE);
    if (live) {
#pragma unroll
      for (int r = 0; r < 16; ++r) acc0[r] = 0.f;
      EFX_RPANEL_G(lds + ((p + 1) % NST) * STAGE, xh, xl, EFX_MF_T);
      const float wk = tab[T_W0S + 64 * h + li], wv = tab[T_W0S + 64 * h + 32 + li];
      float ksum = 0.f;
#pragma unroll
      for (int r = 0; r < 16; ++r) {
        const float k = acck[r] * wk;
        acck[r] = (k > 0.f ? k + 1.f : __expf(k)) * mk[r];
        acc0[r] = acc0[r] * (wv * (mk[r] * a.inv_s));
        ksum += acck[r];
      }
      f32x16 kv;
#pragma unroll
      for (int r = 0; r < 16; ++r) kv[r] = 0.f;
#pragma unroll
      for (int r = 0; r < 16; ++r) kv = __builtin_amdgcn_mfma_f32_32x32x2f32(acck[r], acc0[r], kv, 0, 0, 0);
      ksum += swap32(ksum);
#pragma unroll
      for (int r = 0; r < 16; ++r)
        asm volatile("ds_write_b32 %0, %1 offset:%2" :: "v"(red_w), "v"(kv[r]), "i"(((r & 3) + 8 * (r >> 2)) * 128) : "memory");
      if (g == 0) asm volatile("ds_write_b32 %0, %1 offset:%2" :: "v"(red_w), "v"(ksum), "i"(32 * 128) : "memory");
      asm volatile("s_waitcnt lgkmcnt(0)" ::: "memory");
    }
  }
  __builtin_amdgcn_s_barrier();
  KVX_REDUCE(7)
#undef KVX_ISSUE
#undef KVX_REDUCE
}

__device__ __forceinline__ void kv_final_body(const float* part, const int splits, float* kvout, const float* wm, const int h,
                                              sp_t* pm, char* const lds) {
  float* skv = reinterpret_cast<float*>(lds);
  float* sgrp = reinterpret_cast<float*>(lds + 8192);
  {
    constexpr int NV = 33 * 32 / 4;
    const int w = threadIdx.x >> 6, lane = threadIdx.x & 63;
    f32x4 a[5];
#pragma unroll
    for (int u = 0; u < 5; ++u) a[u] = f32x4{0.f, 0.f, 0.f, 0.f};
#pragma unroll 4
    for (int k = w; k < splits; k += 4) {
      const f32x4* pk = reinterpret_cast<const f32x4*>(part + (long)k * (33 * 32));
#pragma unroll
      for (int u = 0; u < 5; ++u) {
        const int v = lane + u * 64;
        if (v < NV) a[u] += pk[v];
      }
    }
#pragma unroll
    for (int u = 0; u < 5; ++u) {
      const int v = lane + u * 64;
      if (v < NV) reinterpret_cast<f32x4*>(sgrp + w * (33 * 32))[v] = a[u];
    }
  }
  __syncthreads();
  for (int e = threadIdx.x; e < 33 * 32; e += 256) {
    const float s = ((sgrp[e] + sgrp[33 * 32 + e]) + sgrp[2 * 33 * 32 + e]) + sgrp[3 * 33 * 32 + e];
    kvout[e] = s;
    skv[e] = s;
  }
  __syncthreads();
  const int q = threadIdx.x & 3;
#pragma unroll 1
  for (int z = 0; z < 4; ++z) {
    const int j = z * 64 + (threadIdx.x >> 2);
    f32x4 w4[8];
#pragma unroll
    for (int i = 0; i < 8; ++i) w4[i] = reinterpret_cast<const f32x4*>(wm + (long)j * 256 + h * 32)[i];
    float r[8];
#pragma unroll
    for (int dd = 0; dd < 8; ++dd) {
      const float* kvrow = &skv[(q * 8 + dd) * 32];
      float s = 0.f;
#pragma unroll
      for (int i = 0; i < 8; ++i) {
        const f32x4 k4 = *reinterpret_cast<const f32x4*>(kvrow + i * 4);
        s += k4.x * w4[i].x + k4.y * w4[i].y + k4.z * w4[i].z + k4.w * w4[i].w;
      }
      r[dd] = s * ATTN_P_SCALE;
    }
    u32x4 hi, lo;
    sp_pack8(r, hi, lo);
    sp_t* dst = pm + (long)j * 256 + h * 32 + q * 4;
    *reinterpret_cast<u32x4*>(dst) = hi;
    *reinterpret_cast<u32x4*>(dst + 16) = lo;
  }
}

typedef __attribute__((address_space(1))) unsigned gu32;
__device__ __forceinline__ unsigned pct_load(unsigned* p) { return __hip_atomic_load(p, __ATOMIC_RELAXED, __HIP_MEMORY_SCOPE_AGENT); }

__global__ __launch_bounds__(W * 64, 1) void coarse_persistent_kernel(PctArgs P) {
  __shared__ __attribute__((aligned(16))) char lds[LDS_BYTES_P];
  int* const ctrl = reinterpret_cast<int*>(lds + OFF_CTRL);
  if (P.items[-1].what != P.signature || P.items[-1].signal != (unsigned)P.n_items) {
    if (threadIdx.x == 0) {
      __hip_atomic_fetch_or(P.cnt + 1, 2u, __ATOMIC_RELAXED, __HIP_MEMORY_SCOPE_AGENT);
      if (P.status) __hip_atomic_fetch_or(P.status, 2u, __ATOMIC_RELAXED, __HIP_MEMORY_SCOPE_AGENT);
    }
    return;
  }
  const int lane0 = (threadIdx.x & 63) == 0;
  const bool wave0 = __builtin_amdgcn_readfirstlane((int)(threadIdx.x >> 6)) == 0;
  for (int mine = 0; P.quota <= 0 || mine < P.quota; ++mine) {
    unsigned long long t_pop = 0, t_rdy = 0;
    if (wave0) {
      unsigned itv = 0;
      if (lane0) itv = __hip_atomic_fetch_add(P.cnt, 1u, __ATOMIC_RELAXED, __HIP_MEMORY_SCOPE_AGENT);
      const unsigned it = __builtin_amdgcn_readfirstlane(itv);
      int go = it < (unsigned)P.n_items ? 1 : 0;
      if (P.trace) t_pop = wall_clock64();
      if (go) {
        const PctItem* pi = P.items + it;
        bool any = false;
#pragma unroll 1
        for (int d = 0; d < 4 && go; ++d) {
          const uint32_t dep = __builtin_amdgcn_readfirstlane(pi->dep[d]);
          if (dep == PCT_NODEP) continue;
          any = true;
          unsigned* c = P.cnt + (dep & 0xfffffu);
          const unsigned target = dep >> 20;
          unsigned spins = 0;
          while (__builtin_amdgcn_readfirstlane(pct_load(c)) < target) {
            __builtin_amdgcn_s_sleep(8);
            if ((++spins & 1023u) == 0 && (__builtin_amdgcn_readfirstlane(pct_load(P.cnt + 1)) != 0 || spins > (1u << 20))) {
              if (lane0) {
                __hip_atomic_fetch_or(P.cnt + 1, 1u + (it << 1), __ATOMIC_RELAXED, __HIP_MEMORY_SCOPE_AGENT);
                if (P.status) __hip_atomic_fetch_or(P.status, 1u + (it << 1), __ATOMIC_RELAXED, __HIP_MEMORY_SCOPE_AGENT);
              }
              go = 0;
              break;
            }
          }
        }
        if (any) __builtin_amdgcn_fence(__ATOMIC_ACQUIRE, "agent");
        if (P.trace) t_rdy = wall_clock64();
      }
      if (lane0) ctrl[0] = go ? (int)it : -1;
    }
    __syncthreads();
    const int it = __builtin_amdgcn_readfirstlane(ctrl[0]);
    if (it < 0) break;
    const PctItem* pi = P.items + it;
    const unsigned what = __builtin_amdgcn_readfirstlane(pi->what), signal = __builtin_amdgcn_readfirstlane(pi->signal);
    const unsigned sig2a = __builtin_amdgcn_readfirstlane(pi->sig2[0]), sig2b = __builtin_amdgcn_readfirstlane(pi->sig2[1]);
    const int type = what & 15, c = (what >> 4) & 255, pair = (what >> 12) & 255, idx = what >> 20;
    const PctCall call = P.call[c];
    const PctLayerPtrs& lw = P.layer[call.layer];
    const int Tx = P.T[call.x_img], Ts = P.T[call.s_img];
    const long cp = (long)c * P.N + pair;
    if ((P.skip >> type) & 1) {
    } else if (type == PCT_X) {
      Args a;
      a.x_sp = P.sp[call.x_img]; a.x_f32 = P.f32[call.x_img]; a.out_f32 = P.f32[call.x_img]; a.out_sp = P.sp[call.x_img];
      a.wq = lw.wq; a.pm = P.pm + (long)c * P.N * 65536; a.pm_seq_stride = 65536; a.w0 = lw.w0; a.w2 = lw.w2;
      a.wq_s = lw.wq_s; a.w0_s = lw.w0_s; a.w2_s = lw.w2_s;
      a.kv = P.kv + (long)c * P.N * (8 * 33 * 32);
      a.mask = P.mask[call.x_img];
      a.g1 = lw.g1; a.b1 = lw.b1; a.g2 = lw.g2; a.b2 = lw.b2;
      a.v_length = (float)Ts; a.attn_eps = 1e-6f; a.p_out_scale = 1.f / ATTN_P_SCALE; a.ln_eps = 1e-5f;
      a.nseq = P.N; a.T = Tx; a.groups = 0; a.xsplit = 1; a.gpc = 0;
      FoldArgs fa;
      fa.n = 0;
#pragma unroll
      for (int i = 0; i < 2; ++i) {
        const int cf = call.fold[i];
        if (cf < 0) continue;
        const PctLayerPtrs& lf = P.layer[P.call[cf].layer];
        KvTile& k = fa.k[fa.n++];
        k.x_sp = nullptr; k.mask = nullptr; k.T = Tx;
        k.wkv = lf.wkv; k.wkv_s = lf.wkv_s; k.inv_s = 1.f / (float)Tx;
        k.part = P.part + (((long)cf * P.N + pair) * 8 * P.splits + idx) * (33 * 32); k.head_stride = (long)P.splits * (33 * 32);
      }
      encoder_x_body<true>(a, pair, idx, lds, &fa);
    } else if (type == PCT_K) {
      KvTile k;
      k.x_sp = P.sp[call.s_img] + (long)pair * Ts * 256;
      k.mask = P.mask[call.s_img] ? P.mask[call.s_img] + (long)pair * Ts : nullptr;
      k.T = Ts; k.wkv = lw.wkv; k.wkv_s = lw.wkv_s; k.inv_s = 1.f / (float)Ts;
      k.part = P.part + (cp * 8 * P.splits + idx) * (33 * 32); k.head_stride = (long)P.splits * (33 * 32);
      kv_tile_body(k, idx, lds);
    } else {
      kv_final_body(P.part + (cp * 8 + idx) * P.splits * (33 * 32), ceil_div(Ts, W * PT), P.kv + (cp * 8 + idx) * (33 * 32), lw.merge_f32, idx,
                    P.pm + cp * 65536, lds);
    }
    asm volatile("s_waitcnt vmcnt(0)" ::: "memory");
    __syncthreads();
    if (wave0) {
      __builtin_amdgcn_fence(__ATOMIC_RELEASE, "agent");
      asm volatile("s_waitcnt vmcnt(0)" ::: "memory");
      if (lane0) {
        __hip_atomic_fetch_add(P.cnt + signal, 1u, __ATOMIC_RELAXED, __HIP_MEMORY_SCOPE_AGENT);
        if (sig2a != PCT_NODEP) __hip_atomic_fetch_add(P.cnt + sig2a, 1u, __ATOMIC_RELAXED, __HIP_MEMORY_SCOPE_AGENT);
        if (sig2b != PCT_NODEP) __hip_atomic_fetch_add(P.cnt + sig2b, 1u, __ATOMIC_RELAXED, __HIP_MEMORY_SCOPE_AGENT);
        if (P.trace) {
          unsigned long long* tr = P.trace + (long)it * 4;
          tr[0] = t_pop; tr[1] = t_rdy; tr[2] = wall_clock64(); tr[3] = blockIdx.x;
        }
      }
    }
  }
}
#undef EFX_RPANEL
#undef EFX_RPANEL_G
#undef EFX_MF_N
#undef EFX_MF_T
#undef EFX_KPANEL
#undef EFX_RD
#undef EFX_USE
#undef EFX_ISSUE
#undef EFX_ISSUE_SRC
#undef EFX_BEGIN
#undef EFX_BEGIN_G
}
}

static int make_job(const EncoderXArgs& p, efx::Args& a) {
  if (p.C != 256 || p.nseq <= 0 || p.T <= 0 || !p.wq_s || !p.w0_s || !p.w2_s || !p.kv) return 0;
  a = efx::Args{};
  a.x_sp = p.x_sp; a.x_f32 = p.x_f32; a.out_f32 = p.out_f32; a.out_sp = p.out_sp;
  a.wq = p.wq; a.pm = p.pm; a.pm_seq_stride = p.pm_seq_stride; a.w0 = p.w0; a.w2 = p.w2;
  a.wq_s = p.wq_s; a.w0_s = p.w0_s; a.w2_s = p.w2_s; a.kv = p.kv; a.mask = p.mask;
  a.g1 = p.g1; a.b1 = p.b1; a.g2 = p.g2; a.b2 = p.b2;
  a.v_length = p.v_length; a.attn_eps = p.attn_eps; a.p_out_scale = p.p_out_scale; a.ln_eps = p.ln_eps;
  a.skip_padded = p.skip_padded;
  a.nseq = p.nseq; a.T = p.T; a.groups = ceil_div(ceil_div(p.T, efx::PT), efx::W);
  a.xsplit = p.nseq < NUM_XCD ? NUM_XCD / p.nseq : 1;
  if (a.xsplit > a.groups) a.xsplit = a.groups;
  a.gpc = ceil_div(a.groups, a.xsplit);
  return NUM_XCD * ceil_div(p.nseq * a.xsplit, NUM_XCD) * a.gpc;
}

int encoder_x_workgroups(const EncoderXArgs& p) {
  efx::Args a;
  return make_job(p, a);
}

int launch_encoder_x2(const EncoderXArgs& p0, int off0, int n0, const EncoderXArgs& p1, int off1, int n1, hipStream_t st) {
  efx::Args2 m;
  const int g0 = make_job(p0, m.j[0]);
  const int g1 = n1 > 0 ? make_job(p1, m.j[1]) : 0;
  if (g0 == 0 || (n1 > 0 && g1 == 0)) return LOFTR_ERR_UNSUPPORTED;
  if (off0 < 0 || n0 <= 0 || off0 + n0 > g0 || off0 % NUM_XCD || n0 % NUM_XCD || n1 < 0) return LOFTR_ERR_BAD_ARG;
  if (n1 > 0 && (off1 < 0 || off1 + n1 > g1 || off1 % NUM_XCD)) return LOFTR_ERR_BAD_ARG;
  if (n1 == 0) m.j[1] = m.j[0];
  m.n0 = n0; m.off0 = off0; m.off1 = off1;
  TimedLaunch tl(LOFTR_T_ENCODER_X, st);
  hipLaunchKernelGGL(efx::encoder_x2_kernel, dim3(n0 + n1), dim3(efx::W * 64), 0, st, m);
  LOFTR_CHECK_LAUNCH();
  return LOFTR_OK;
}

int launch_encoder_x(const EncoderXArgs& p, hipStream_t st) {
  efx::Args a;
  const int grid = make_job(p, a);
  if (grid == 0) return LOFTR_ERR_UNSUPPORTED;
  TimedLaunch tl(LOFTR_T_ENCODER_X, st);
  hipLaunchKernelGGL(efx::encoder_x_kernel, dim3(grid), dim3(efx::W * 64), 0, st, a);
  LOFTR_CHECK_LAUNCH();
  return LOFTR_OK;
}

int launch_coarse_persistent(const PctLaunch& p, hipStream_t st) {
  const PctShape& s = p.shape;
  if (!s.ok() || !p.plan) return LOFTR_ERR_UNSUPPORTED;
  if (p.plan_bytes < pct_plan_bytes(s) || p.ws_bytes < pct_ws_bytes(s)) return LOFTR_ERR_WORKSPACE;
  const size_t cp = (size_t)s.n_calls() * s.N;
  WsAlloc wa(p.ws, p.ws_bytes);
  efx::PctArgs a{};
  a.cnt = wa.take<unsigned>(s.n_counters());
  a.part = wa.take<float>(cp * 8 * s.gmax() * 33 * 32);
  a.kv = wa.take<float>(cp * 8 * 33 * 32);
  a.pm = wa.take<sp_t>(cp * 65536);
  if (!wa.ok()) return LOFTR_ERR_WORKSPACE;
  for (int i = 0; i < 2; ++i) { a.f32[i] = p.f32[i]; a.sp[i] = p.sp[i]; a.mask[i] = p.mask[i]; a.T[i] = s.T[i]; }
  a.N = s.N; a.n_calls = s.n_calls(); a.n_items = (int)s.n_items(); a.splits = s.gmax();
  a.items = reinterpret_cast<const PctItem*>(p.plan) + 1;
  a.trace = p.trace; a.status = p.status; a.signature = p.plan_signature;
  for (int l = 0; l < s.n_layers; ++l) a.layer[l] = p.layer[l];
  for (int c = 0; c < s.n_calls(); ++c) { s.call(c, a.call[c].layer, a.call[c].x_img, a.call[c].s_img); s.folds(c, a.call[c].fold); }
  if (hipMemsetAsync(a.cnt, 0, s.n_counters() * 4, st) != hipSuccess) return LOFTR_ERR_LAUNCH;
  TimedLaunch tl(LOFTR_T_ENCODER_X, st);
  a.skip = loftr_debug_value(LOFTR_DBG_PCT_SKIP);
  const int cap = loftr_debug_value(LOFTR_DBG_PCT_GRID) > 0 ? loftr_debug_value(LOFTR_DBG_PCT_GRID) : 256;
  int grid = a.n_items < cap ? a.n_items : cap;
  a.quota = loftr_debug_value(LOFTR_DBG_PCT_QUOTA);
  if (a.quota > 0) grid = ceil_div(a.n_items, a.quota) + 8;
  hipLaunchKernelGGL(efx::coarse_persistent_kernel, dim3(grid), dim3(efx::W * 64), 0, st, a);
  LOFTR_CHECK_LAUNCH();
  return LOFTR_OK;
}
```

### loftr_amd/csrc/transformer.hip

```cpp
#include "linear.h"
#include "attention.h"
#include "coarse_plan.h"

namespace {

constexpr int MAX_LAYERS = 16;

struct LayerSp {
  const sp_t *q, *k, *v, *merge, *mlp0, *mlp2;
  const sp_t* kv;
  const float *q_s, *k_s, *v_s, *merge_s, *mlp0_s, *mlp2_s, *kv_s;
  const float* merge_f32;
  const float *n1w, *n1b, *n2w, *n2b;
};

struct EncoderWs {
  sp_t* q;
  float *k, *v;
  sp_t *msg, *msgn, *hid;
  void* attn; size_t attn_bytes;
  void* attn2;
  bool ok;
};

size_t weights_sp_dwords(int C) { return (size_t)12 * C * C + (size_t)16 * C; }
constexpr int JOBS_PER_LAYER = 6 + 16;

size_t encoder_ws_bytes(int nb, int L, int S, int C) {
  size_t rows_l = (size_t)nb * L, rows_s = (size_t)nb * S;
  size_t b = 0;
  b += 3 * align_up(rows_l * C * 4, 256);
  b += 2 * align_up(rows_s * C * 4, 256);
  b += align_up(rows_l * 2 * C * 4, 256);
  b += 2 * align_up(attention_workspace_bytes(nb, S, C), 256);
  return b + 2048;
}

EncoderWs carve(WsAlloc& wa, int nb, int L, int S, int C) {
  EncoderWs e;
  size_t rows_l = (size_t)nb * L, rows_s = (size_t)nb * S;
  e.q = wa.take<sp_t>(rows_l * C);
  e.msg = wa.take<sp_t>(rows_l * C);
  e.msgn = wa.take<sp_t>(rows_l * C);
  e.k = wa.take<float>(rows_s * C);
  e.v = wa.take<float>(rows_s * C);
  e.hid = wa.take<sp_t>(rows_l * 2 * C);
  e.attn_bytes = attention_workspace_bytes(nb, S, C);
  e.attn = wa.take<char>(e.attn_bytes);
  e.attn2 = wa.take<char>(e.attn_bytes);
  e.ok = wa.ok();
  return e;
}

bool weights_ok(const loftr_layer_weights& w) {
  return w.q_proj && w.k_proj && w.v_proj && w.merge && w.mlp0 && w.mlp2 && w.norm1_w && w.norm1_b &&
         w.norm2_w && w.norm2_b;
}

LayerSp stage_layer(const loftr_layer_weights& w, sp_t* dst, int C, SpJobs& jobs) {
  LayerSp l;
  float* sc = reinterpret_cast<float*>(dst + (size_t)12 * C * C);
  auto add = [&](const float* src, int rows, int K, float* inv) {
    const int i = jobs.n++;
    jobs.src[i] = src; jobs.dst[i] = dst; jobs.rows[i] = rows; jobs.K[i] = K; jobs.ld[i] = K; jobs.inv_scale[i] = inv;
    sp_t* r = dst;
    dst += (size_t)rows * K;
    return r;
  };
  l.q_s = sc; l.k_s = sc + C; l.v_s = sc + 2 * C; l.merge_s = sc + 3 * C; l.mlp0_s = sc + 4 * C; l.mlp2_s = sc + 6 * C;
  l.kv_s = sc + 7 * C;
  l.q = add(w.q_proj, C, C, sc);
  l.k = add(w.k_proj, C, C, sc + C);
  l.v = add(w.v_proj, C, C, sc + 2 * C);
  l.merge = add(w.merge, C, C, sc + 3 * C);
  l.mlp0 = add(w.mlp0, 2 * C, 2 * C, sc + 4 * C);
  l.mlp2 = add(w.mlp2, C, 2 * C, sc + 6 * C);
  l.kv = nullptr;
  if (C == 256) {
    l.kv = dst;
    for (int h = 0; h < 8; ++h) {
      add(w.k_proj + (size_t)h * 32 * C, 32, C, sc + 7 * C + h * 64);
      add(w.v_proj + (size_t)h * 32 * C, 32, C, sc + 7 * C + h * 64 + 32);
    }
  }
  l.merge_f32 = w.merge;
  l.n1w = w.norm1_w; l.n1b = w.norm1_b; l.n2w = w.norm2_w; l.n2b = w.norm2_b;
  return l;
}

int coarse_kv(const sp_t* src_sp, const uint8_t* src_mask, const LayerSp& w, int nb, int S, int C, int H, void* attn, size_t attn_bytes,
              const float** kv, const sp_t** pm, hipStream_t st) {
  float* part = attention_part_buffer(attn, attn_bytes, nb, S);
  if (!part) return LOFTR_ERR_WORKSPACE;
  int rc;
  ProjKVArgs pkv{src_sp, S, C, nb, w.kv, src_mask, 1.f / (float)S, part, ceil_div(S, 128), w.kv_s};
  if ((rc = launch_proj_kv(pkv, st))) return rc;
  return launch_attention_finalize(w.merge_f32, nb, S, C, H, attn, attn_bytes, kv, pm, st);
}
EncoderXArgs coarse_x(float* x_f32, sp_t* x_sp, const uint8_t* x_mask, const LayerSp& w, int nb, int L, int S, int C, const float* kv,
                      const sp_t* pm, int skip_padded = 0) {
  return EncoderXArgs{x_sp, x_f32, x_f32, x_sp, nb, L, C, w.q, pm, (long)C * C, w.mlp0, w.mlp2, w.q_s, w.mlp0_s, w.mlp2_s,
                      kv, x_mask, w.n1w, w.n1b, w.n2w, w.n2b, (float)S, 1e-6f, 1.f / ATTN_P_SCALE, 1e-5f, skip_padded};
}

int coarse_transformer_scheduled(float* feat0, float* feat1, sp_t* sp0, sp_t* sp1, const uint8_t* mask0, const uint8_t* mask1,
                                 const LayerSp* lw, int P, bool stacked, int N, int L, int S, int C, int H, const EncoderWs& e,
                                 hipStream_t st, int skip = 0) {
  int rc;
  const float* kvA; const sp_t* pmA; const float* kvB; const sp_t* pmB;
  {
    EncoderXArgs probe = coarse_x(feat0, sp0, mask0, lw[0], N, L, L, C, reinterpret_cast<const float*>(e.attn), reinterpret_cast<const sp_t*>(e.attn));
    if (encoder_x_workgroups(probe) == 0) return LOFTR_ERR_UNSUPPORTED;
  }
  if (stacked) {
    if ((rc = coarse_kv(sp0, mask0, lw[0], 2 * N, L, C, H, e.attn, e.attn_bytes, &kvA, &pmA, st))) return rc;
    if ((rc = launch_encoder_x(coarse_x(feat0, sp0, mask0, lw[0], 2 * N, L, L, C, kvA, pmA, skip), st))) return rc;
  } else {
    if ((rc = coarse_kv(sp0, mask0, lw[0], N, L, C, H, e.attn, e.attn_bytes, &kvA, &pmA, st))) return rc;
    if ((rc = coarse_kv(sp1, mask1, lw[0], N, S, C, H, e.attn2, e.attn_bytes, &kvB, &pmB, st))) return rc;
    const EncoderXArgs a = coarse_x(feat0, sp0, mask0, lw[0], N, L, L, C, kvA, pmA, skip), b = coarse_x(feat1, sp1, mask1, lw[0], N, S, S, C, kvB, pmB, skip);
    if ((rc = launch_encoder_x2(a, 0, encoder_x_workgroups(a), b, 0, encoder_x_workgroups(b), st))) return rc;
  }
  for (int i = 0; i < P; ++i) {
    const LayerSp& wc = lw[2 * i + 1];
    if ((rc = coarse_kv(sp1, mask1, wc, N, S, C, H, e.attn, e.attn_bytes, &kvA, &pmA, st))) return rc;
    if ((rc = launch_encoder_x(coarse_x(feat0, sp0, mask0, wc, N, L, S, C, kvA, pmA, skip), st))) return rc;
    if ((rc = coarse_kv(sp0, mask0, wc, N, L, C, H, e.attn, e.attn_bytes, &kvA, &pmA, st))) return rc;
    const EncoderXArgs d = coarse_x(feat1, sp1, mask1, wc, N, S, L, C, kvA, pmA, skip);
    const int nd = encoder_x_workgroups(d);
    if (i + 1 == P) {
      if ((rc = launch_encoder_x(d, st))) return rc;
      break;
    }
    const LayerSp& ws = lw[2 * i + 2];
    if ((rc = coarse_kv(sp0, mask0, ws, N, L, C, H, e.attn2, e.attn_bytes, &kvB, &pmB, st))) return rc;
    const EncoderXArgs a = coarse_x(feat0, sp0, mask0, ws, N, L, L, C, kvB, pmB, skip);
    const int na = encoder_x_workgroups(a);
    int head = (256 - nd % 256) % 256 / 8 * 8;
    if (head > na) head = na;
    if ((rc = launch_encoder_x2(d, 0, nd, a, 0, head, st))) return rc;
    if ((rc = coarse_kv(sp1, mask1, ws, N, S, C, H, e.attn, e.attn_bytes, &kvA, &pmA, st))) return rc;
    const EncoderXArgs b = coarse_x(feat1, sp1, mask1, ws, N, S, S, C, kvA, pmA, skip);
    if ((rc = launch_encoder_x2(b, 0, encoder_x_workgroups(b), a, head, na - head, st))) return rc;
  }
  return LOFTR_OK;
}

int encoder_layer(const float* x_f32, const sp_t* x_sp, const sp_t* src_sp, bool self,
                  const uint8_t* x_mask, const uint8_t* src_mask, const LayerSp& w,
                  float* out_f32, sp_t* out_sp, int nb, int L, int S, int C, int H,
                  const EncoderWs& e, hipStream_t st, int skip_padded = 0) {
  if (nb <= 0) return LOFTR_OK;
  const int Ml = nb * L, Ms = nb * S;
  const float inv_s = 1.f / (float)S;
  const float attn_eps = 1e-6f;
  int rc;
  if (C == 256) {
    float* part = attention_part_buffer(e.attn, e.attn_bytes, nb, S);
    if (!part) return LOFTR_ERR_WORKSPACE;
    ProjKVArgs pkv{src_sp, S, C, nb, w.kv, src_mask, inv_s, part, ceil_div(S, 128), w.kv_s};
    if ((rc = launch_proj_kv(pkv, st))) return rc;
    const float* kv = nullptr; const sp_t* pm = nullptr;
    if ((rc = launch_attention_finalize(w.merge_f32, nb, S, C, H, e.attn, e.attn_bytes, &kv, &pm, st))) return rc;
    (void)Ms;
    {
      EncoderXArgs fx{x_sp, x_f32, out_f32, out_sp, nb, L, C, w.q, pm, (long)C * C, w.mlp0, w.mlp2, w.q_s, w.mlp0_s, w.mlp2_s,
                      kv, x_mask, w.n1w, w.n1b, w.n2w, w.n2b, (float)S, attn_eps, 1.f / ATTN_P_SCALE, 1e-5f, skip_padded};
      return launch_encoder_x(fx, st);
    }
  } else {
    float* qf = reinterpret_cast<float*>(e.q);
    if (self) {
      ProjArgs p{x_sp, Ml, C, 1, 3, {w.q, w.k, w.v}, {qf, e.k, e.v}, {0, 1, 2}, x_mask, inv_s, nullptr, 0.f, 0.f,
                 {w.q_s, w.k_s, w.v_s}};
      if ((rc = launch_proj(p, st))) return rc;
    } else {
      ProjArgs pq{x_sp, Ml, C, 1, 1, {w.q, nullptr, nullptr}, {qf, nullptr, nullptr}, {0, 0, 0}, x_mask, inv_s,
                  nullptr, 0.f, 0.f, {w.q_s, nullptr, nullptr}};
      if ((rc = launch_proj(pq, st))) return rc;
      ProjArgs pkv{src_sp, Ms, C, 1, 2, {w.k, w.v, nullptr}, {e.k, e.v, nullptr}, {1, 2, 0}, src_mask, inv_s,
                   nullptr, 0.f, 0.f, {w.k_s, w.v_s, nullptr}};
      if ((rc = launch_proj(pkv, st))) return rc;
    }
    if ((rc = launch_attention_small(qf, e.k, e.v, e.msg, nb, L, S, C, H, st))) return rc;
    LinearLNArgs m{asrc_plain(e.msg, C), w.merge, C, w.n1w, w.n1b, nullptr, nullptr, e.msgn, Ml, C, C, 1e-5f, 1, 0,
                   w.merge_s, 0.f};
    if ((rc = launch_linear_ln(m, st))) return rc;
  }
  LinearArgs h{asrc_cat(x_sp, e.msgn, C, C), w.mlp0, 2 * C, nullptr, e.hid, 2 * C, Ml, 2 * C, 2 * C, nullptr, 0, 1, true,
               w.mlp0_s, nullptr};
  if ((rc = launch_linear(h, st))) return rc;
  LinearLNArgs o{asrc_plain(e.hid, 2 * C), w.mlp2, 2 * C, w.n2w, w.n2b, x_f32, out_f32, out_sp, Ml, C, 2 * C, 1e-5f, 1, 0,
                 w.mlp2_s, 0.f};
  return launch_linear_ln(o, st);
}

}

extern "C" size_t loftr_encoder_workspace_bytes(int nb, int L, int S, int C) {
  if (nb <= 0 || L <= 0 || S <= 0 || C <= 0) return 0;
  const int m = L > S ? L : S;
  size_t b = encoder_ws_bytes(nb, m, m, C) + 2 * align_up((size_t)nb * m * C * 4, 256) +
             align_up(weights_sp_dwords(C) * 4 * MAX_LAYERS, 256) + 4096;
  const PctShape ps{PCT_MAX_LAYERS, nb / 2, {L, S}};
  if (C == 256 && ps.ok()) b += align_up(pct_ws_bytes(ps), 256);
  return b;
}

extern "C" int loftr_encoder_layer_fwd(const float* x, const float* source, const uint8_t* x_mask,
                                       const uint8_t* source_mask, const loftr_layer_weights* w,
                                       float* out, int nb, int L, int S, int C, int H, void* ws,
                                       size_t ws_bytes, void* stream) {
  LOFTR_CHECK_ARG(x && source && w && out && nb >= 0 && L > 0 && S > 0 && (ws || nb == 0));
  LOFTR_CHECK_ARG(weights_ok(*w));
  if (!((C == 256 || C == 128) && H == 8)) return LOFTR_ERR_UNSUPPORTED;
  if (nb == 0) return LOFTR_OK;
  hipStream_t st = (hipStream_t)stream;
  WsAlloc wa(ws, ws_bytes);
  sp_t* x_sp = wa.take<sp_t>((size_t)nb * L * C);
  sp_t* s_sp = wa.take<sp_t>((size_t)nb * S * C);
  sp_t* w_sp = wa.take<sp_t>(weights_sp_dwords(C));
  EncoderWs e = carve(wa, nb, L, S, C);
  if (!e.ok) return LOFTR_ERR_WORKSPACE;
  const bool self = (x == source) && (x_mask == source_mask);
  SpJobs jobs; jobs.n = 0;
  auto add = [&](const float* src, sp_t* dst, long rows) {
    const int i = jobs.n++;
    jobs.src[i] = src; jobs.dst[i] = dst; jobs.rows[i] = (int)rows; jobs.K[i] = C; jobs.ld[i] = C;
  };
  add(x, x_sp, (long)nb * L);
  if (!self) add(source, s_sp, (long)nb * S);
  const LayerSp lw = stage_layer(*w, w_sp, C, jobs);
  int rc;
  if ((rc = launch_sp_convert(jobs, st))) return rc;
  return encoder_layer(x, x_sp, self ? x_sp : s_sp, self, x_mask, source_mask, lw, out, nullptr, nb, L, S, C, H, e, st);
}

namespace {
int convert_layers(const loftr_layer_weights* layers, int n_layers, int C, sp_t* w_sp, SpJobs& jobs, LayerSp* lw, hipStream_t st) {
  int rc;
  for (int i = 0; i < n_layers; ++i) {
    if (jobs.n + JOBS_PER_LAYER > SP_MAX_JOBS) {
      if ((rc = launch_sp_convert(jobs, st))) return rc;
      jobs = SpJobs();
    }
    lw[i] = stage_layer(layers[i], w_sp + weights_sp_dwords(C) * i, C, jobs);
  }
  return launch_sp_convert(jobs, st);
}
void view_layers(const loftr_layer_weights* layers, int n_layers, int C, sp_t* w_sp, LayerSp* lw) {
  for (int i = 0; i < n_layers; ++i) {
    SpJobs scratch;
    lw[i] = stage_layer(layers[i], w_sp + weights_sp_dwords(C) * i, C, scratch);
  }
}
}

extern "C" size_t loftr_transformer_prepared_bytes(int n_layers, int C) {
  if (n_layers <= 0 || C <= 0) return 0;
  return align_up(weights_sp_dwords(C) * 4 * (size_t)n_layers, 256) + 256;
}

extern "C" int loftr_transformer_prepare(const loftr_layer_weights* layers, int n_layers, int C, void* prepared,
                                         size_t prepared_bytes, void* stream) {
  LOFTR_CHECK_ARG(layers && prepared && n_layers > 0);
  if (!(C == 256 || C == 128) || n_layers > MAX_LAYERS) return LOFTR_ERR_UNSUPPORTED;
  for (int i = 0; i < n_layers; ++i) LOFTR_CHECK_ARG(weights_ok(layers[i]));
  if (prepared_bytes < loftr_transformer_prepared_bytes(n_layers, C)) return LOFTR_ERR_WORKSPACE;
  LayerSp lw[MAX_LAYERS];
  SpJobs jobs;
  return convert_layers(layers, n_layers, C, reinterpret_cast<sp_t*>(prepared), jobs, lw, (hipStream_t)stream);
}

static int transformer_fwd(float* feat0, float* feat1, const uint8_t* mask0,
                           const uint8_t* mask1, const loftr_layer_weights* layers,
                           const int* layer_is_cross, int n_layers, int N, int L, int S,
                           int C, int H, const void* prepared, size_t prepared_bytes, void* ws, size_t ws_bytes,
                           const void* plan, size_t plan_bytes, int plan_order, void* diag, size_t diag_bytes, void* stream,
                           int skip_padded = 0) {
  LOFTR_CHECK_ARG(feat0 && feat1 && layers && layer_is_cross && n_layers >= 0 && N >= 0 && L > 0 && S > 0);
  LOFTR_CHECK_ARG((mask0 == nullptr) == (mask1 == nullptr));
  if (!((C == 256 || C == 128) && H == 8) || n_layers > MAX_LAYERS) return LOFTR_ERR_UNSUPPORTED;
  if (N == 0 || n_layers == 0) return LOFTR_OK;
  LOFTR_CHECK_ARG(ws != nullptr);
  if (prepared && prepared_bytes < loftr_transformer_prepared_bytes(n_layers, C)) return LOFTR_ERR_WORKSPACE;
  hipStream_t st = (hipStream_t)stream;
  for (int i = 0; i < n_layers; ++i) LOFTR_CHECK_ARG(weights_ok(layers[i]));
  const bool stacked = (L == S) && (feat1 == feat0 + (size_t)N * L * C) &&
                       (mask0 == nullptr || mask1 == mask0 + (size_t)N * L);
  WsAlloc wa(ws, ws_bytes);
  sp_t* sp0 = wa.take<sp_t>((size_t)N * (L + S) * C);
  sp_t* sp1 = sp0 + (size_t)N * L * C;
  sp_t* w_sp = wa.take<sp_t>(weights_sp_dwords(C) * n_layers);
  EncoderWs e = carve(wa, 2 * N, L > S ? L : S, L > S ? L : S, C);
  if (!e.ok) return LOFTR_ERR_WORKSPACE;
  int rc;
  LayerSp lw[MAX_LAYERS];
  bool weights_ready = false;
  if (prepared) {
    view_layers(layers, n_layers, C, reinterpret_cast<sp_t*>(const_cast<void*>(prepared)), lw);
    weights_ready = true;
  }
  if (C == 128 && n_layers == 2 && !layer_is_cross[0] && layer_is_cross[1] && L == S && L <= 32 && !mask0) {
    if (!weights_ready) {
      SpJobs wj;
      if ((rc = convert_layers(layers, n_layers, C, w_sp, wj, lw, st))) return rc;
      weights_ready = true;
    }
    FinePairArgs fp{};
    fp.f0 = feat0; fp.f1 = feat1; fp.M = N; fp.T = L; fp.C = C; fp.attn_eps = 1e-6f; fp.ln_eps = 1e-5f;
    for (int l = 0; l < 2; ++l) {
      fp.wq[l] = lw[l].q; fp.wk[l] = lw[l].k; fp.wv[l] = lw[l].v; fp.wm[l] = lw[l].merge; fp.w0[l] = lw[l].mlp0; fp.w2[l] = lw[l].mlp2;
      fp.sq[l] = lw[l].q_s; fp.sk[l] = lw[l].k_s; fp.sv[l] = lw[l].v_s; fp.sm[l] = lw[l].merge_s; fp.s0[l] = lw[l].mlp0_s; fp.s2[l] = lw[l].mlp2_s;
      fp.g1[l] = lw[l].n1w; fp.b1[l] = lw[l].n1b; fp.g2[l] = lw[l].n2w; fp.b2[l] = lw[l].n2b;
    }
    if ((rc = launch_fine_pair(fp, st)) != LOFTR_ERR_UNSUPPORTED) return rc;
  }
  {
    SpJobs jobs;
    auto add = [&](const float* src, sp_t* dst, long rows) {
      const int i = jobs.n++;
      jobs.src[i] = src; jobs.dst[i] = dst; jobs.rows[i] = (int)rows; jobs.K[i] = C; jobs.ld[i] = C;
    };
    add(feat0, sp0, (long)N * L);
    add(feat1, sp1, (long)N * S);
    if (weights_ready) {
      if ((rc = launch_sp_convert(jobs, st))) return rc;
    } else if ((rc = convert_layers(layers, n_layers, C, w_sp, jobs, lw, st))) return rc;
  }
  {
    bool pattern = C == 256 && n_layers >= 2 && n_layers % 2 == 0;
    for (int i = 0; pattern && i < n_layers; ++i) pattern = (layer_is_cross[i] != 0) == ((i & 1) != 0);
    if (plan && pattern && n_layers <= PCT_MAX_LAYERS) {
      PctLaunch pl{};
      pl.shape = PctShape{n_layers, N, {L, S}};
      if (!pl.shape.ok()) return LOFTR_ERR_UNSUPPORTED;
      pl.f32[0] = feat0; pl.f32[1] = feat1; pl.sp[0] = sp0; pl.sp[1] = sp1; pl.mask[0] = mask0; pl.mask[1] = mask1;
      for (int i = 0; i < n_layers; ++i) {
        const LayerSp& w = lw[i];
        pl.layer[i] = PctLayerPtrs{w.q, w.mlp0, w.mlp2, w.kv, w.q_s, w.mlp0_s, w.mlp2_s, w.kv_s, w.merge_f32, w.n1w, w.n1b, w.n2w, w.n2b};
      }
      pl.plan = plan; pl.plan_bytes = plan_bytes; pl.plan_signature = pl.shape.signature(plan_order);
      pl.ws = wa.take<char>(pct_ws_bytes(pl.shape)); pl.ws_bytes = pct_ws_bytes(pl.shape);
      if (!wa.ok()) return LOFTR_ERR_WORKSPACE;
      if (diag && diag_bytes >= 16) {
        pl.status = reinterpret_cast<unsigned*>(diag);
        if (diag_bytes >= 16 + 32 * pl.shape.n_items()) pl.trace = reinterpret_cast<unsigned long long*>(reinterpret_cast<char*>(diag) + 16);
      }
      return launch_coarse_persistent(pl, st);
    }
    const bool sched_on = loftr_debug_value(LOFTR_DBG_ENCODER_SCHEDULE) != 0;
    if (sched_on && pattern) {
      rc = coarse_transformer_scheduled(feat0, feat1, sp0, sp1, mask0, mask1, lw, n_layers / 2, stacked, N, L, S, C, H, e, st, skip_padded);
      if (rc != LOFTR_ERR_UNSUPPORTED) return rc;
    }
  }
  for (int i = 0; i < n_layers; ++i) {
    if (!layer_is_cross[i]) {
      if (stacked) {
        if ((rc = encoder_layer(feat0, sp0, sp0, true, mask0, mask0, lw[i], feat0, sp0, 2 * N, L, L, C, H, e, st, skip_padded))) return rc;
      } else {
        if ((rc = encoder_layer(feat0, sp0, sp0, true, mask0, mask0, lw[i], feat0, sp0, N, L, L, C, H, e, st, skip_padded))) return rc;
        if ((rc = encoder_layer(feat1, sp1, sp1, true, mask1, mask1, lw[i], feat1, sp1, N, S, S, C, H, e, st, skip_padded))) return rc;
      }
    } else {
      if ((rc = encoder_layer(feat0, sp0, sp1, false, mask0, mask1, lw[i], feat0, sp0, N, L, S, C, H, e, st, skip_padded))) return rc;
      if ((rc = encoder_layer(feat1, sp1, sp0, false, mask1, mask0, lw[i], feat1, sp1, N, S, L, C, H, e, st, skip_padded))) return rc;
    }
  }
  return LOFTR_OK;
}

extern "C" int loftr_transformer_fwd(float* feat0, float* feat1, const uint8_t* mask0,
                                     const uint8_t* mask1, const loftr_layer_weights* layers,
                                     const int* layer_is_cross, int n_layers, int N, int L, int S,
                                     int C, int H, const void* prepared, size_t prepared_bytes, void* ws, size_t ws_bytes,
                                     void* stream) {
  return transformer_fwd(feat0, feat1, mask0, mask1, layers, layer_is_cross, n_layers, N, L, S, C, H, prepared, prepared_bytes, ws, ws_bytes,
                         nullptr, 0, 0, nullptr, 0, stream);
}

extern "C" int loftr_transformer_fwd_padded(float* feat0, float* feat1, const uint8_t* mask0,
                                            const uint8_t* mask1, const loftr_layer_weights* layers,
                                            const int* layer_is_cross, int n_layers, int N, int L, int S,
                                            int C, int H, const void* prepared, size_t prepared_bytes, void* ws, size_t ws_bytes,
                                            int skip_padded_tiles, void* stream) {
  return transformer_fwd(feat0, feat1, mask0, mask1, layers, layer_is_cross, n_layers, N, L, S, C, H, prepared, prepared_bytes, ws, ws_bytes,
                         nullptr, 0, 0, nullptr, 0, stream, skip_padded_tiles != 0 && mask0 != nullptr);
}

extern "C" int loftr_transformer_fwd_planned(float* feat0, float* feat1, const uint8_t* mask0,
                                             const uint8_t* mask1, const loftr_layer_weights* layers,
                                             const int* layer_is_cross, int n_layers, int N, int L, int S,
                                             int C, int H, const void* prepared, size_t prepared_bytes, void* ws, size_t ws_bytes,
                                             const void* plan, size_t plan_bytes, int plan_order, void* diag, size_t diag_bytes,
                                             void* stream) {
  LOFTR_CHECK_ARG(plan != nullptr && (plan_order == 0 || plan_order == 1));
  return transformer_fwd(feat0, feat1, mask0, mask1, layers, layer_is_cross, n_layers, N, L, S, C, H, prepared, prepared_bytes, ws, ws_bytes,
                         plan, plan_bytes, plan_order, diag, diag_bytes, stream);
}

extern "C" size_t loftr_linear_workspace_bytes(int M, int N, int K) {
  if (M <= 0 || N <= 0 || K <= 0) return 0;
  return align_up((size_t)M * ceil32(K) * 4, 256) + align_up((size_t)N * ceil32(K) * 4, 256) +
         align_up((size_t)M * 4, 256) + align_up((size_t)N * 4, 256) + 1024;
}

extern "C" int loftr_linear_fwd(const float* a, const float* w, float* out, int M, int N, int K,
                                void* ws, size_t ws_bytes, void* stream) {
  LOFTR_CHECK_ARG(a && w && out && M >= 0 && N > 0 && K > 0);
  if (M == 0) return LOFTR_OK;
  LOFTR_CHECK_ARG(ws != nullptr);
  hipStream_t st = (hipStream_t)stream;
  const int Kp = ceil32(K);
  WsAlloc wa(ws, ws_bytes);
  sp_t* a_sp = wa.take<sp_t>((size_t)M * Kp);
  sp_t* w_sp = wa.take<sp_t>((size_t)N * Kp);
  float* a_inv = wa.take<float>((size_t)M);
  float* w_inv = wa.take<float>((size_t)N);
  if (!wa.ok()) return LOFTR_ERR_WORKSPACE;
  SpJobs jobs; jobs.n = 2;
  jobs.src[0] = a; jobs.dst[0] = a_sp; jobs.rows[0] = M; jobs.K[0] = K; jobs.ld[0] = K; jobs.inv_scale[0] = a_inv;
  jobs.src[1] = w; jobs.dst[1] = w_sp; jobs.rows[1] = N; jobs.K[1] = K; jobs.ld[1] = K; jobs.inv_scale[1] = w_inv;
  int rc;
  if ((rc = launch_sp_convert(jobs, st))) return rc;
  LinearArgs p{asrc_plain(a_sp, Kp), w_sp, Kp, out, nullptr, N, M, N, Kp, nullptr, 0, 1, false, w_inv, a_inv};
  return launch_linear(p, st);
}
```

### loftr_amd/loftr.py

```python
import contextlib
import math
import warnings
import weakref

import torch
import torch.nn as nn

from . import autograd, ops
from .backbone import build_backbone


class PositionEncodingSine(nn.Module):

    def __init__(self, d_model, max_shape=(256, 256), temp_bug_fix=True):
        super().__init__()
        ys = torch.arange(1, max_shape[0] + 1, dtype=torch.float32).view(1, -1, 1).expand(1, *max_shape)
        xs = torch.arange(1, max_shape[1] + 1, dtype=torch.float32).view(1, 1, -1).expand(1, *max_shape)
        idx = torch.arange(0, d_model // 2, 2).float()
        if temp_bug_fix:
            freq = torch.exp(idx * (-math.log(10000.0) / (d_model // 2)))
        else:
            freq = torch.exp(idx * (-math.log(10000.0) / d_model // 2))
        freq = freq[:, None, None]
        pe = torch.zeros((d_model, *max_shape))
        pe[0::4] = torch.sin(xs * freq)
        pe[1::4] = torch.cos(xs * freq)
        pe[2::4] = torch.sin(ys * freq)
        pe[3::4] = torch.cos(ys * freq)
        self.register_buffer("pe", pe.unsqueeze(0), persistent=False)

    def forward(self, x):
        if autograd.wants_grad(x):
            return autograd.pos_encode_flatten(x, self.pe[0])
        return ops.pos_encode_flatten(x, self.pe[0])


class LoFTREncoderLayer(nn.Module):

    def __init__(self, d_model, nhead, attention="linear"):
        super().__init__()
        if attention != "linear":
            raise NotImplementedError("only attention='linear' is on the HIP path (no shipped config uses 'full')")
        self.dim = d_model // nhead
        self.nhead = nhead
        self.q_proj = nn.Linear(d_model, d_model, bias=False)
        self.k_proj = nn.Linear(d_model, d_model, bias=False)
        self.v_proj = nn.Linear(d_model, d_model, bias=False)
        self.merge = nn.Linear(d_model, d_model, bias=False)
        self.mlp = nn.Sequential(
            nn.Linear(d_model * 2, d_model * 2, bias=False),
            nn.ReLU(True),
            nn.Linear(d_model * 2, d_model, bias=False),
        )
        self.norm1 = nn.LayerNorm(d_model)
        self.norm2 = nn.LayerNorm(d_model)

    def weight_tensors(self):
        return {"q_proj": self.q_proj.weight, "k_proj": self.k_proj.weight, "v_proj": self.v_proj.weight,
                "merge": self.merge.weight, "mlp0": self.mlp[0].weight, "mlp2": self.mlp[2].weight,
                "norm1_w": self.norm1.weight, "norm1_b": self.norm1.bias,
                "norm2_w": self.norm2.weight, "norm2_b": self.norm2.bias}

    def weight_struct(self):
        sd = self.weight_tensors()
        for k, v in sd.items():
            if not v.is_contiguous() or v.dtype != torch.float32 or not v.is_cuda:
                raise ops._lib.LoftrHipError(f"{k}: parameters must be contiguous float32 GPU tensors "
                                             f"(got {v.dtype}, {v.device}); the HIP path computes in fp32")
        return ops.layer_weights_struct(sd)

    def forward(self, x, source, x_mask=None, source_mask=None):
        wants = autograd.wants_grad(x, source, *self.parameters())
        if wants and not self.training and autograd.wants_grad(x, source):
            import warnings
            warnings.warn("LoFTREncoderLayer in .eval() mode returns a tensor WITHOUT a graph although its inputs require grad: "
                          "call .train() for the differentiable HIP nodes", stacklevel=2)
        if self.training and wants:
            self.weight_struct()
            return autograd.encoder_layer(x, source, self.weight_tensors(), self.nhead, x_mask, source_mask)
        return ops.encoder_layer(x.contiguous(), source.contiguous(), self.weight_struct(), self.nhead,
                                 x_mask, source_mask)


class LocalFeatureTransformer(nn.Module):

    def __init__(self, config):
        super().__init__()
        self.config = config
        self.d_model = config["d_model"]
        self.nhead = config["nhead"]
        self.layer_names = config["layer_names"]
        self.layers = nn.ModuleList([LoFTREncoderLayer(config["d_model"], config["nhead"], config["attention"])
                                     for _ in range(len(self.layer_names))])
        self._reset_parameters()

    def _reset_parameters(self):
        first = self.layers[0].state_dict() if len(self.layers) else {}
        for p in self.layers[0].parameters() if len(self.layers) else []:
            if p.dim() > 1:
                nn.init.xavier_uniform_(p)
        for layer in self.layers[1:]:
            for p in layer.parameters():
                if p.dim() > 1:
                    nn.init.xavier_uniform_(p)
        del first

    def forward(self, feat0, feat1, mask0=None, mask1=None, inplace=False, mode=None, skip_padded=False):
        assert self.d_model == feat0.size(2), "the feature number of src and transformer must be equal"
        for name in self.layer_names:
            if name not in ("self", "cross"):
                raise KeyError
        if not self.training and autograd.wants_grad(feat0, feat1):
            import warnings
            warnings.warn("LocalFeatureTransformer in .eval() mode returns tensors WITHOUT a graph although its inputs require grad: "
                          "call .train() for the differentiable HIP nodes", stacklevel=2)
        if self.training and autograd.wants_grad(feat0, feat1, *self.parameters()):
            for layer, name in zip(self.layers, self.layer_names):
                if name == "self":
                    feat0 = layer(feat0, feat0, mask0, mask0)
                    feat1 = layer(feat1, feat1, mask1, mask1)
                else:
                    feat0 = layer(feat0, feat1, mask0, mask1)
                    feat1 = layer(feat1, feat0, mask1, mask0)
            return feat0, feat1
        structs = [layer.weight_struct() for layer in self.layers]
        return ops.transformer(feat0.contiguous(), feat1.contiguous(), structs, self.layer_names, self.nhead,
                               mask0, mask1, inplace=inplace, prepared=self._prepared(structs, feat0.device), mode=mode,
                               skip_padded=skip_padded)

    def _prepared(self, structs, device):
        if self.training or not str(device).startswith("cuda"):
            return None
        mats = [getattr(getattr(layer, n) if "." not in n else layer.mlp[int(n.split(".")[1])], "weight")
                for layer in self.layers for n in ("q_proj", "k_proj", "v_proj", "merge", "mlp.0", "mlp.2")]
        key = tuple((t.data_ptr(), t._version) for t in mats) + (str(device),)
        cached = ops._PREPARED.get(self)
        if cached is None or cached[0] != key or not all(r() is t for r, t in zip(cached[2], mats)):
            cached = (key, ops.transformer_prepare(structs, self.d_model, device), [weakref.ref(t) for t in mats])
            ops._PREPARED[self] = cached
        return cached[1]


def _valid_cells(mask):
    return mask.sum(dim=1).amax(dim=-1) * mask.sum(dim=2).amax(dim=-1)


def compute_max_candidates(p_m0, p_m1):
    return torch.minimum(_valid_cells(p_m0), _valid_cells(p_m1)).sum()


def _cell_points(ids, width, scale, image_scale, b_ids):
    xy = torch.stack((ids.remainder(width), ids.div(width, rounding_mode="floor")), dim=1)
    return xy * (scale if image_scale is None else scale * image_scale[b_ids])


class CoarseMatching(nn.Module):

    def __init__(self, config):
        super().__init__()
        self.config = config
        self.thr = config["thr"]
        self.border_rm = config["border_rm"]
        self.train_coarse_percent = config["train_coarse_percent"]
        self.train_pad_num_gt_min = config["train_pad_num_gt_min"]
        self.match_type = config["match_type"]
        self.materialize_conf = True
        if self.match_type == "dual_softmax":
            self.temperature = config["dsmax_temperature"]
        elif self.match_type == "sinkhorn":
            self.bin_score = nn.Parameter(torch.tensor(config["skh_init_bin_score"], requires_grad=True))
            self.skh_iters = config["skh_iters"]
            self.skh_prefilter = config["skh_prefilter"]
        else:
            raise NotImplementedError()

    def forward(self, feat_c0, feat_c1, data, mask_c0=None, mask_c1=None):
        scale = data["hw0_i"][0] / data["hw0_c"][0]
        kw = dict(thr=self.thr, border_rm=self.border_rm, scale=scale, match_type=self.match_type,
                  mask0=mask_c0, mask1=mask_c1, scale0=data.get("scale0"), scale1=data.get("scale1"))
        if self.match_type == "dual_softmax":
            kw.update(temperature=self.temperature, want_conf=self.materialize_conf)
        else:
            sparse = self.config["sparse_spvs"]
            kw.update(bin_score=float(self.bin_score.detach()), skh_iters=self.skh_iters,
                      skh_prefilter=self.skh_prefilter and not self.training,
                      want_assign=bool(sparse))
        hw = (tuple(data["hw0_c"]), tuple(data["hw1_c"]))
        if self.match_type == "dual_softmax" and autograd.wants_grad(feat_c0, feat_c1):
            r = autograd.dual_softmax_match(feat_c0, feat_c1, *hw, **dict(kw, want_conf=True))
        elif (self.match_type == "sinkhorn" and not kw["skh_prefilter"] and
              (autograd.wants_grad(feat_c0, feat_c1) or (self.training and autograd.wants_grad(self.bin_score)))):
            r = autograd.sinkhorn_match(feat_c0, feat_c1, self.bin_score, *hw, **{k: v for k, v in kw.items() if k != "bin_score"})
            if not kw["want_assign"]:
                r.pop("conf_matrix_with_bin")
        else:
            if self.match_type == "sinkhorn" and kw["skh_prefilter"] and autograd.wants_grad(feat_c0, feat_c1, self.bin_score):
                warnings.warn("CoarseMatching: eval-mode skh_prefilter=True returns conf_matrix WITHOUT an autograd graph "
                              "(inputs require grad); use .train() or skh_prefilter=False for a differentiable Sinkhorn head",
                              RuntimeWarning, stacklevel=2)
            r = ops.coarse_match(feat_c0, feat_c1, *hw, **kw)
        if "conf_matrix_with_bin" in r:
            data.update({"conf_matrix_with_bin": r["conf_matrix_with_bin"]})
        data.update({"conf_matrix": r["conf_matrix"]})
        mconf = r["mconf"]
        if self.training:
            data["_match_counts"] = r["counts"]
            return data.update(**self._train_sample(r, data, scale))
        out = {"b_ids": r["b_ids"], "i_ids": r["i_ids"], "j_ids": r["j_ids"]}
        if self.thr >= 0:
            out.update({"gt_mask": torch.zeros_like(mconf, dtype=torch.bool), "m_bids": r["b_ids"],
                        "mkpts0_c": r["mkpts0_c"], "mkpts1_c": r["mkpts1_c"], "mconf": mconf})
        else:
            keep = mconf != 0
            out.update({"gt_mask": mconf == 0, "m_bids": r["b_ids"][keep], "mkpts0_c": r["mkpts0_c"][keep],
                        "mkpts1_c": r["mkpts1_c"][keep], "mconf": mconf[keep]})
        data.update(**out)
        data["_match_counts"] = r["counts"]


    def _train_sample(self, r, data, scale):
        conf = data["conf_matrix"]
        if conf is None:
            raise ops._lib.LoftrHipError("CoarseMatching.train(): materialize_conf must stay True (the losses read conf_matrix)")
        n_batch, n0, n1 = conf.shape
        cells = compute_max_candidates(data["mask0"], data["mask1"]) if "mask0" in data else n_batch * max(n0, n1)
        budget, pad_min = int(cells * self.train_coarse_percent), self.train_pad_num_gt_min
        assert pad_min < budget, "min-num-gt-pad should be less than num-train-matches"
        pred = (r["b_ids"], r["i_ids"], r["j_ids"])
        truth = (data["spv_b_ids"], data["spv_i_ids"], data["spv_j_ids"])
        n_pred, n_truth, dev = pred[0].numel(), truth[0].numel(), r["mconf"].device
        room = budget - pad_min
        take = torch.arange(n_pred, device=dev) if n_pred <= room else torch.randint(n_pred, (room,), device=dev)
        fill = torch.randint(n_truth, (max(budget - n_pred, pad_min),), device=dev)
        b_ids, i_ids, j_ids = (torch.cat((p[take], t[fill])) for p, t in zip(pred, truth))
        mconf = torch.cat((r["mconf"][take], r["mconf"].new_zeros(fill.numel())))
        predicted = mconf != 0
        pts0 = _cell_points(i_ids, data["hw0_c"][1], scale, data.get("scale0"), b_ids)
        pts1 = _cell_points(j_ids, data["hw1_c"][1], scale, data.get("scale1"), b_ids)
        return {"b_ids": b_ids, "i_ids": i_ids, "j_ids": j_ids, "gt_mask": ~predicted, "m_bids": b_ids[predicted],
                "mkpts0_c": pts0[predicted], "mkpts1_c": pts1[predicted], "mconf": mconf[predicted]}


class FinePreprocess(nn.Module):

    def __init__(self, config):
        super().__init__()
        self.config = config
        self.cat_c_feat = config["fine_concat_coarse_feat"]
        self.W = self.config["fine_window_size"]
        d_model_c = self.config["coarse"]["d_model"]
        d_model_f = self.config["fine"]["d_model"]
        self.d_model_f = d_model_f
        self.last_head = None
        self.last_head_first = None
        if self.cat_c_feat:
            self.down_proj = nn.Linear(d_model_c, d_model_f, bias=True)
            self.merge_feat = nn.Linear(2 * d_model_f, d_model_f, bias=True)
        for p in self.parameters():
            if p.dim() > 1:
                nn.init.kaiming_normal_(p, mode="fan_out", nonlinearity="relu")

    def forward(self, feat_f0, feat_f1, feat_c0, feat_c1, data):
        W = self.W
        stride = data["hw0_f"][0] // data["hw0_c"][0]
        data.update({"W": W})
        if data["b_ids"].shape[0] == 0:
            feat0 = torch.empty(0, self.W ** 2, self.d_model_f, device=feat_f0.device)
            feat1 = torch.empty(0, self.W ** 2, self.d_model_f, device=feat_f0.device)
            return feat0, feat1
        kw = {}
        if self.cat_c_feat:
            kw = dict(down_w=self.down_proj.weight, down_b=self.down_proj.bias,
                      merge_w=self.merge_feat.weight, merge_b=self.merge_feat.bias)
        wants = autograd.wants_grad(feat_f0, feat_f1, feat_c0, feat_c1, *self.parameters())
        if wants and self.training and not self.cat_c_feat:
            raise ops._lib.LoftrHipError("FinePreprocess: gradients requested with fine_concat_coarse_feat=False, whose backward is not "
                                         "implemented (csrc/fine_bwd.hip covers the reference's default, True)")
        if self.training and self.cat_c_feat and wants:
            return autograd.fine_preprocess(feat_f0, feat_f1, feat_c0, feat_c1, (data["b_ids"], data["i_ids"], data["j_ids"]),
                                            (tuple(data["hw0_c"]), tuple(data["hw1_c"]), W, stride), **kw)
        return ops.fine_preprocess(feat_f0, feat_f1, feat_c0, feat_c1, data["b_ids"], data["i_ids"], data["j_ids"],
                                   tuple(data["hw0_c"]), tuple(data["hw1_c"]), W, stride, **kw)

    def forward_windows(self, h_sp0, h_sp1, cin, conv, dense_fn, fine_head, feat_c0, feat_c1, data):
        M = data["b_ids"].shape[0]
        dense_pixels = 2 * h_sp0.shape[0] * h_sp0.shape[1] * h_sp0.shape[2]
        windows = fine_head == "windows" or ops.window_head_wins(M, dense_pixels)
        if M == 0 or not windows or not ops.window_head_supported(self.W, cin, conv.out_channels, h_sp0, h_sp1):
            self.last_head = "dense"
            if M == 0:
                return self.forward(h_sp0, h_sp1, feat_c0, feat_c1, data)
            return self.forward(dense_fn(h_sp0), dense_fn(h_sp1), feat_c0, feat_c1, data)
        self.last_head = "windows"
        W = self.W
        stride = data["hw0_f"][0] // data["hw0_c"][0]
        data.update({"W": W})
        return ops.fine_preprocess_windows(h_sp0, h_sp1, cin, conv, feat_c0, feat_c1, data["b_ids"], data["i_ids"], data["j_ids"],
                                           tuple(data["hw0_c"]), tuple(data["hw1_c"]), W, stride,
                                           down_w=self.down_proj.weight, down_b=self.down_proj.bias,
                                           merge_w=self.merge_feat.weight, merge_b=self.merge_feat.bias)

    def forward_windows2(self, t_sp0, t_sp1, cin, head, first_fn, dense_fn, fine_head, feat_c0, feat_c1, data):
        M = data["b_ids"].shape[0]
        dense_pixels = 2 * t_sp0.shape[0] * t_sp0.shape[1] * t_sp0.shape[2]
        both = (M > 0 and (fine_head == "windows" or ops.window_head_first_wins(M, dense_pixels))
                and ops.window_head_first_supported(self.W, cin, head[0], head[3], t_sp0, t_sp1, M))
        if not both:
            self.last_head_first = "dense"
            if M == 0:
                return self.forward_windows(t_sp0, t_sp1, head[0].out_channels, head[3], dense_fn, fine_head, feat_c0, feat_c1, data)
            stacked = ops.stacked_halves(t_sp0, t_sp1)
            if stacked is not None:
                h_sp0, h_sp1 = first_fn(stacked).split(t_sp0.shape[0])
            else:
                h_sp0, h_sp1 = first_fn(t_sp0), first_fn(t_sp1)
            return self.forward_windows(h_sp0, h_sp1, head[0].out_channels, head[3], dense_fn, fine_head, feat_c0, feat_c1, data)
        self.last_head = self.last_head_first = "windows"
        W = self.W
        stride = data["hw0_f"][0] // data["hw0_c"][0]
        data.update({"W": W})
        return ops.fine_preprocess_windows2(t_sp0, t_sp1, cin, head[0], head[1], head[3], feat_c0, feat_c1, data["b_ids"], data["i_ids"],
                                            data["j_ids"], tuple(data["hw0_c"]), tuple(data["hw1_c"]), W, stride,
                                            down_w=self.down_proj.weight, down_b=self.down_proj.bias,
                                            merge_w=self.merge_feat.weight, merge_b=self.merge_feat.bias)

    def forward_gather(self, bank_f0, slot0, bank_f1, slot1, feat_c0, feat_c1, data):
        W = self.W
        stride = data["hw0_f"][0] // data["hw0_c"][0]
        data.update({"W": W})
        if data["b_ids"].shape[0] == 0:
            feat0 = torch.empty(0, self.W ** 2, self.d_model_f, device=bank_f0.device)
            feat1 = torch.empty(0, self.W ** 2, self.d_model_f, device=bank_f0.device)
            return feat0, feat1
        kw = {}
        if self.cat_c_feat:
            kw = dict(down_w=self.down_proj.weight, down_b=self.down_proj.bias,
                      merge_w=self.merge_feat.weight, merge_b=self.merge_feat.bias)
        return ops.fine_preprocess_gather(bank_f0, slot0, bank_f1, slot1, feat_c0, feat_c1, data["b_ids"], data["i_ids"], data["j_ids"],
                                          tuple(data["hw0_c"]), tuple(data["hw1_c"]), W, stride, **kw)


class FineMatching(nn.Module):

    def forward(self, feat_f0, feat_f1, data):
        M, WW, C = feat_f0.shape
        scale = data["hw0_i"][0] / data["hw0_f"][0]
        if M == 0:
            assert self.training is False, "M is always >0, when training, see coarse_matching.py"
            data.update({"expec_f": torch.empty(0, 3, device=feat_f0.device),
                         "mkpts0_f": data["mkpts0_c"], "mkpts1_f": data["mkpts1_c"]})
            return
        scale1 = data["scale1"] if "scale0" in data else None
        n = len(data["mconf"])
        fine_match = autograd.fine_match if autograd.wants_grad(feat_f0, feat_f1) else ops.fine_match
        if data["mkpts1_c"].shape[0] == M:
            expec, mk1f = fine_match(feat_f0, feat_f1, data["mkpts1_c"], data["b_ids"], scale, scale1)
            mk1f = mk1f[:n]
        else:
            expec, off = fine_match(feat_f0, feat_f1, torch.zeros(M, 2, device=feat_f0.device), data["b_ids"], scale, scale1)
            mk1f = data["mkpts1_c"] + off[:n]
        data.update({"expec_f": expec, "mkpts0_f": data["mkpts0_c"], "mkpts1_f": mk1f})


class LoFTR(nn.Module):

    def __init__(self, config):
        super().__init__()
        self.config = config
        self.backbone = build_backbone(config).to(memory_format=torch.channels_last)
        self.backbone_impl = "hip"
        self.overlap_fine_branch = True
        self.skip_padded_tiles = True
        self.coarse_mode = None
        self.fine_join_late = False
        self._side_stream = None
        self.backbone_halves = None
        self._half_streams = None
        self.fine_head = None
        self.head_grads = False
        self.full_grads = False
        self.pos_encoding = PositionEncodingSine(config["coarse"]["d_model"],
                                                 temp_bug_fix=config["coarse"]["temp_bug_fix"])
        self.loftr_coarse = LocalFeatureTransformer(config["coarse"])
        self.coarse_matching = CoarseMatching(config["match_coarse"])
        self.fine_preprocess = FinePreprocess(config)
        self.loftr_fine = LocalFeatureTransformer(config["fine"])
        self.fine_matching = FineMatching()

    def _window_head_applies(self, data):
        img0, img1 = data["image0"], data["image1"]
        if (self.fine_head == "dense" or self.training or self.backbone_impl != "hip" or not img0.is_cuda
                or img0.shape[2:] != img1.shape[2:] or not hasattr(self.backbone, "WINDOW_HEAD") or not self.fine_preprocess.cat_c_feat):
            return False
        return img0.shape[0] + img1.shape[0] <= self._backbone_cap(img0)

    def _backbone_cap(self, x):
        return getattr(self, "_backbone_chunk_images", None) or max(1, (2 ** 31 - 1) // ((x.shape[2] // 2) * (x.shape[3] // 2) * 256))

    def run_backbone(self, data, head_input=False):
        data.update({"bs": data["image0"].size(0),
                     "hw0_i": data["image0"].shape[2:], "hw1_i": data["image1"].shape[2:]})
        cl = lambda img: img.contiguous(memory_format=torch.channels_last)
        use_hip = self.backbone_impl == "hip" and data["image0"].is_cuda and not self.training
        run = self.backbone.forward_hip if use_hip else self.backbone
        self._fine_join = None
        assert not head_input or (use_hip and data["hw0_i"] == data["hw1_i"])
        hkw = dict(head_input=head_input) if head_input else {}
        if data["hw0_i"] == data["hw1_i"]:
            x = cl(torch.cat([data["image0"], data["image1"]], dim=0))
            cap = self._backbone_cap(x)
            if use_hip and x.shape[0] > cap:
                outs = [run(x[i:i + cap]) for i in range(0, x.shape[0], cap)]
                feats_c, feats_f = torch.cat([o[0] for o in outs]), torch.cat([o[1] for o in outs])
            elif use_hip and self.overlap_fine_branch and (data["bs"] >= 8 if self.backbone_halves is None else self.backbone_halves):
                main = torch.cuda.current_stream(x.device)
                self.backbone.prepare_hip()
                if self._half_streams is None:
                    self._half_streams = [torch.cuda.Stream(device=x.device) for _ in range(2)]
                outs, fines, evs = [], [], []
                for k, st in enumerate(self._half_streams):
                    st.wait_stream(main)
                    xk = data["image0"] if k == 0 else data["image1"]
                    xk.record_stream(st)
                    with torch.cuda.stream(st):
                        fc, fine_fn = run(cl(xk), defer_fine=True, **hkw)
                        ev = torch.cuda.Event(); ev.record(st)
                        ff = fine_fn()
                    outs.append(fc); fines.append(ff); evs.append(ev)
                for k in range(2):
                    main.wait_event(evs[k])
                    outs[k].record_stream(main); fines[k].record_stream(main)
                self._fine_join = list(self._half_streams)
                return outs[0], outs[1], fines[0], fines[1]
            elif use_hip and self.overlap_fine_branch:
                feats_c, fine_fn = run(x, defer_fine=True, **hkw)
                main = torch.cuda.current_stream(x.device)
                if self._side_stream is None:
                    self._side_stream = torch.cuda.Stream(device=x.device)
                side = self._side_stream
                side.wait_stream(main)
                for t in fine_fn.reads:
                    t.record_stream(side)
                with torch.cuda.stream(side):
                    feats_f = fine_fn()
                feats_f.record_stream(main)
                self._fine_join = side
            elif head_input:
                feats_c, fine_fn = run(x, defer_fine=True, **hkw)
                feats_f = fine_fn()
            else:
                feats_c, feats_f = run(x)
            (feat_c0, feat_c1), (feat_f0, feat_f1) = feats_c.split(data["bs"]), feats_f.split(data["bs"])
        else:
            (feat_c0, feat_f0), (feat_c1, feat_f1) = run(cl(data["image0"])), run(cl(data["image1"]))
        return feat_c0, feat_c1, feat_f0, feat_f1

    def _join_fine(self, device):
        j = getattr(self, "_fine_join", None)
        if j is not None:
            for st in (j if isinstance(j, list) else [j]):
                torch.cuda.current_stream(device).wait_stream(st)
            self._fine_join = None

    def match_from_features(self, feat_c0, feat_c1, feat_f0, feat_f1, data, head_input=False):
        data.update({"hw0_c": feat_c0.shape[2:], "hw1_c": feat_c1.shape[2:]})
        if head_input:
            data.update({"hw0_f": feat_f0.shape[1:3], "hw1_f": feat_f1.shape[1:3]})
        else:
            data.update({"hw0_f": feat_f0.shape[2:], "hw1_f": feat_f1.shape[2:]})
        both = (ops.stacked_halves(feat_c0, feat_c1)
                if feat_c0.shape == feat_c1.shape and not autograd.wants_grad(feat_c0, feat_c1) else None)
        if both is not None:
            feat_c0, feat_c1 = self.pos_encoding(both).split(feat_c0.shape[0])
        else:
            feat_c0 = self.pos_encoding(feat_c0)
            feat_c1 = self.pos_encoding(feat_c1)
        if head_input == "t1":
            head = getattr(self.backbone, self.backbone.WINDOW_HEAD)
            fine_pre = lambda c0, c1: self.fine_preprocess.forward_windows2(feat_f0, feat_f1, head[0].in_channels, head, self.backbone.fine_head_first,
                                                                            self.backbone.fine_head_last, self.fine_head, c0, c1, data)
        elif head_input:
            head = getattr(self.backbone, self.backbone.WINDOW_HEAD)
            fine_pre = lambda c0, c1: self.fine_preprocess.forward_windows(feat_f0, feat_f1, head[0].out_channels, head[3], self.backbone.fine_head_last,
                                                                           self.fine_head, c0, c1, data)
        else:
            fine_pre = lambda c0, c1: self.fine_preprocess(feat_f0, feat_f1, c0, c1, data)
        self._match_encoded(feat_c0, feat_c1, data, fine_pre)

    def _match_encoded(self, feat_c0, feat_c1, data, fine_preprocess):
        mask_c0 = mask_c1 = None
        if "mask0" in data:
            mask_c0, mask_c1 = data["mask0"].flatten(-2), data["mask1"].flatten(-2)
        feat_c0, feat_c1 = self.loftr_coarse(feat_c0, feat_c1, mask_c0, mask_c1, inplace=True, mode=self.coarse_mode,
                                             skip_padded=self.skip_padded_tiles and mask_c0 is not None)
        if not self.fine_join_late:
            self._join_fine(feat_c0.device)
        full = self.training and self.full_grads
        grads = self.training and self.head_grads and not full
        if grads:
            feat_c0, feat_c1 = feat_c0.detach().requires_grad_(True), feat_c1.detach().requires_grad_(True)
            data["_head_inputs"] = {"feat_c0": feat_c0, "feat_c1": feat_c1}
        with torch.enable_grad() if grads else contextlib.nullcontext():
            self.coarse_matching(feat_c0, feat_c1, data, mask_c0=mask_c0, mask_c1=mask_c1)
        self._join_fine(feat_c0.device)
        if feat_c0.is_cuda:
            ops.check_transformer_status(feat_c0.device)
        feat_f0_unfold, feat_f1_unfold = fine_preprocess(feat_c0, feat_c1)
        if feat_f0_unfold.size(0) != 0:
            feat_f0_unfold, feat_f1_unfold = self.loftr_fine(feat_f0_unfold, feat_f1_unfold, inplace=True)
        if grads:
            feat_f0_unfold, feat_f1_unfold = feat_f0_unfold.detach().requires_grad_(True), feat_f1_unfold.detach().requires_grad_(True)
            data["_head_inputs"].update({"feat_f0_unfold": feat_f0_unfold, "feat_f1_unfold": feat_f1_unfold})
        with torch.enable_grad() if grads else contextlib.nullcontext():
            self.fine_matching(feat_f0_unfold, feat_f1_unfold, data)

    def forward(self, data):
        graph = self.training and self.full_grads and torch.is_grad_enabled()
        with torch.enable_grad() if graph else torch.no_grad():
            return self._forward(data)

    def _forward(self, data):
        dev = data["image0"].device
        if data["image1"].device != dev:
            raise ops._lib.LoftrHipError(f"image0 on {dev} but image1 on {data['image1'].device}")
        if dev.type != "cuda":
            feat_c0, feat_c1, feat_f0, feat_f1 = self.run_backbone(data)
            return self.match_from_features(feat_c0, feat_c1, feat_f0, feat_f1, data)
        with torch.cuda.device(dev):
            head_input = "t1" if self._window_head_applies(data) else False
            feat_c0, feat_c1, feat_f0, feat_f1 = self.run_backbone(data, head_input=head_input)
            self.match_from_features(feat_c0, feat_c1, feat_f0, feat_f1, data, head_input=head_input)

    def match_pairs(self, bank0, ids0, bank1=None, ids1=None):
        from .pairs import match_pairs
        return match_pairs(self, bank0, ids0, bank1, ids1)

    def load_state_dict(self, state_dict, *args, **kwargs):
        for k in list(state_dict.keys()):
            if k.startswith("matcher."):
                state_dict[k.replace("matcher.", "", 1)] = state_dict.pop(k)
        return super().load_state_dict(state_dict, *args, **kwargs)
```

### loftr_amd/ops.py

```python
import ctypes as C
import os
import weakref
import functools

import torch

from . import _lib
from ._lib import CoarseParams, FMap, LayerWeights, MatchOut, check

_WS = {}

LAYER_FIELDS = (("q_proj", "q_proj.weight"), ("k_proj", "k_proj.weight"), ("v_proj", "v_proj.weight"),
                ("merge", "merge.weight"), ("mlp0", "mlp.0.weight"), ("mlp2", "mlp.2.weight"),
                ("norm1_w", "norm1.weight"), ("norm1_b", "norm1.bias"),
                ("norm2_w", "norm2.weight"), ("norm2_b", "norm2.bias"))


_PREPARED = weakref.WeakKeyDictionary()


def _tensors_in(obj):
    if isinstance(obj, torch.Tensor):
        yield obj
    elif isinstance(obj, (list, tuple)):
        for o in obj:
            yield from _tensors_in(o)
    elif isinstance(obj, dict):
        for o in obj.values():
            yield from _tensors_in(o)
    elif isinstance(obj, torch.nn.Module):
        for prm in obj.parameters():
            yield prm
            break


def _on_device(fn):
    @functools.wraps(fn)
    def wrapped(*args, **kwargs):
        dev = None
        for t in _tensors_in(list(args) + list(kwargs.values())):
            if t.is_cuda:
                if dev is None:
                    dev = t.device
                elif t.device != dev:
                    raise _lib.LoftrHipError(f"{fn.__name__}: tensors on different devices ({dev} and {t.device})")
        if dev is None:
            return fn(*args, **kwargs)
        with torch.cuda.device(dev):
            return fn(*args, **kwargs)
    return wrapped


def _need(t, name, dtype=torch.float32):
    if not isinstance(t, torch.Tensor) or not t.is_cuda:
        raise _lib.LoftrHipError(f"{name}: expected a GPU tensor (the HIP matching path has no CPU fallback)")
    if t.dtype != dtype:
        raise _lib.LoftrHipError(f"{name}: expected {dtype}, got {t.dtype}")
    if not t.is_contiguous():
        raise _lib.LoftrHipError(f"{name}: expected a contiguous tensor")
    return t


def _ptr(t):
    return None if t is None else C.c_void_p(t.data_ptr())


def debug_set(key, value):
    check(_lib.load().loftr_hip_debug_set(key.encode(), int(value)), f"loftr_hip_debug_set({key})")


def debug_get(key):
    v, d = C.c_int(0), C.c_int(0)
    check(_lib.load().loftr_hip_debug_get(key.encode(), C.byref(v), C.byref(d)), f"loftr_hip_debug_get({key})")
    return v.value, d.value


class debug_switch:

    def __init__(self, **kv):
        self.kv, self.old = kv, {}

    def __enter__(self):
        for k, v in self.kv.items():
            self.old[k] = debug_get(k)[0]
            debug_set(k, v)
        return self

    def __exit__(self, *exc):
        for k, v in self.old.items():
            debug_set(k, v)
        return False


def _stream():
    return C.c_void_p(torch.cuda.current_stream().cuda_stream)


def workspace(nbytes, device):
    idx = (device.index if device.index is not None else torch.cuda.current_device(),
           torch.cuda.current_stream(device).cuda_stream)
    buf = _WS.get(idx)
    if buf is None or buf.numel() < nbytes:
        buf = torch.empty(int(nbytes * 1.25) + 4096, dtype=torch.uint8, device=device)
        _WS[idx] = buf
    return buf


def _mask_u8(m, name):
    if m is None:
        return None
    if m.dtype == torch.bool:
        m = m.to(torch.uint8)
    return _need(m.contiguous(), name, torch.uint8)


@_on_device
def linear(a, w):
    _need(a, "a"); _need(w, "w")
    M, K = a.shape
    N = w.shape[0]
    out = torch.empty(M, N, device=a.device, dtype=torch.float32)
    lib = _lib.load()
    ws = workspace(lib.loftr_linear_workspace_bytes(M, N, K), a.device)
    check(lib.loftr_linear_fwd(_ptr(a), _ptr(w), _ptr(out), M, N, K, _ptr(ws), ws.numel(), _stream()), "loftr_linear_fwd")
    return out


@_on_device
def pos_encode_flatten(feat, pe):
    if not feat.is_cuda or feat.dtype != torch.float32:
        raise _lib.LoftrHipError("feat: expected a float32 GPU tensor (the HIP matching path has no CPU fallback)")
    _need(pe, "pe")
    N, Cc, H, W = feat.shape
    out = torch.empty(N, H * W, Cc, device=feat.device, dtype=torch.float32)
    fm = _fmap(feat)
    check(_lib.load().loftr_pos_encode_flatten(C.byref(fm), _ptr(pe), pe.shape[-2], pe.shape[-1], _ptr(out),
                                               N, Cc, _stream()), "loftr_pos_encode_flatten")
    return out


def layer_weights_struct(tensors):
    lw = LayerWeights()
    for field, _ in LAYER_FIELDS:
        setattr(lw, field, tensors[field].data_ptr())
    return lw


@_on_device
def encoder_layer(x, source, w_struct, nhead, x_mask=None, source_mask=None, out=None):
    _need(x, "x"); _need(source, "source")
    nb, L, Cc = x.shape
    S = source.shape[1]
    xm, sm = _mask_u8(x_mask, "x_mask"), _mask_u8(source_mask, "source_mask")
    if x_mask is not None and x_mask is source_mask:
        sm = xm
    out = torch.empty_like(x) if out is None else out
    lib = _lib.load()
    nbytes = lib.loftr_encoder_workspace_bytes(nb, L, S, Cc)
    ws = workspace(nbytes, x.device)
    check(lib.loftr_encoder_layer_fwd(_ptr(x), _ptr(source), _ptr(xm), _ptr(sm), C.byref(w_struct), _ptr(out),
                                      nb, L, S, Cc, nhead, _ptr(ws), ws.numel(), _stream()),
          "loftr_encoder_layer_fwd")
    return out


GRAD_FIELD_SHAPES = lambda Cc: {"q_proj": (Cc, Cc), "k_proj": (Cc, Cc), "v_proj": (Cc, Cc), "merge": (Cc, Cc), "mlp0": (2 * Cc, 2 * Cc),
                                "mlp2": (Cc, 2 * Cc), "norm1_w": (Cc,), "norm1_b": (Cc,), "norm2_w": (Cc,), "norm2_b": (Cc,)}


@_on_device
def encoder_layer_bwd(x, source, weights, grad_out, nhead, x_mask=None, source_mask=None):
    _need(x, "x"); _need(source, "source"); _need(grad_out, "grad_out")
    nb, L, Cc = x.shape
    S = source.shape[1]
    assert tuple(grad_out.shape) == (nb, L, Cc)
    xm, sm = _mask_u8(x_mask, "x_mask"), _mask_u8(source_mask, "source_mask")
    dev = x.device
    gx, gs = torch.empty_like(x), torch.empty_like(source)
    grads = {k: torch.empty(shp, device=dev, dtype=torch.float32) for k, shp in GRAD_FIELD_SHAPES(Cc).items()}
    lib = _lib.load()
    ws = workspace(lib.loftr_encoder_layer_bwd_workspace_bytes(nb, L, S, Cc, nhead), dev)
    wst, gst = layer_weights_struct(weights), layer_weights_struct(grads)
    check(lib.loftr_encoder_layer_bwd(_ptr(x), _ptr(source), _ptr(xm), _ptr(sm), C.byref(wst), _ptr(grad_out), _ptr(gx), _ptr(gs),
                                      C.byref(gst), nb, L, S, Cc, nhead, _ptr(ws), ws.numel(), _stream()), "loftr_encoder_layer_bwd")
    return gx, gs, grads


def stacked_halves(a, b):
    if (a.shape[1:] != b.shape[1:] or a.stride() != b.stride() or a.dtype != b.dtype or a.device != b.device
            or a.untyped_storage().data_ptr() != b.untyped_storage().data_ptr()
            or b.storage_offset() != a.storage_offset() + a.shape[0] * a.stride(0)):
        return None
    return torch.as_strided(a, (a.shape[0] + b.shape[0],) + tuple(a.shape[1:]), a.stride(), a.storage_offset())


@_on_device
def transformer_prepare(layer_structs, Cc, device):
    n_layers = len(layer_structs)
    lib = _lib.load()
    buf = torch.empty(lib.loftr_transformer_prepared_bytes(n_layers, Cc), dtype=torch.uint8, device=device)
    arr = (LayerWeights * n_layers)(*layer_structs)
    with torch.cuda.device(device):
        check(lib.loftr_transformer_prepare(arr, n_layers, Cc, _ptr(buf), buf.numel(), _stream()), "loftr_transformer_prepare")
    return buf


_COARSE_PLANS = {}
COARSE_MODE = os.environ.get("LOFTR_COARSE_MODE", "auto")
COARSE_AUTO_MIN_PAIRS = 8
COARSE_MODES = ("auto", "persistent", "persistent_call_order", "launches")

_STATUS_BUFS = {}
_STATUS_PENDING = {}


def _status_word(device):
    st = torch.cuda.current_stream(device)
    key = (str(device), st.cuda_stream)
    bufs = _STATUS_BUFS.get(key)
    if bufs is None:
        bufs = _STATUS_BUFS[key] = (torch.empty(16, dtype=torch.uint8, device=device), torch.zeros(16, dtype=torch.uint8).pin_memory(),
                                    torch.cuda.Event())
    return key, bufs


def check_transformer_status(device):
    key = (str(device), torch.cuda.current_stream(device).cuda_stream)
    pending = _STATUS_PENDING.pop(key, None)
    if pending is None:
        return
    host, done = pending
    done.synchronize()
    v = int(host.view(torch.int32)[0])
    if v == 0:
        return
    if v == 2:
        why = "its plan was built for another shape or order; nothing was computed"
    elif v % 2 == 1:
        why = f"a workgroup gave up waiting for a dependency at work item {(v - 1) // 2}"
    else:
        why = f"unknown status {v}"
    raise _lib.LoftrHipError(f"persistent coarse transformer (loftr_transformer_fwd_planned) failed: {why}")


def coarse_plan(kinds, N, L, S, device, order=0):
    key = (str(device), tuple(kinds), N, L, S, order)
    if key not in _COARSE_PLANS:
        lib = _lib.load()
        arr = (C.c_int * len(kinds))(*kinds)
        nbytes = lib.loftr_coarse_plan_bytes(arr, len(kinds), N, L, S)
        plan = None
        if nbytes:
            plan = torch.empty(nbytes, dtype=torch.uint8, device=device)
            with torch.cuda.device(device):
                check(lib.loftr_coarse_plan_build(arr, len(kinds), N, L, S, order, _ptr(plan), plan.numel(), _stream()), "loftr_coarse_plan_build")
        _COARSE_PLANS[key] = plan
    return _COARSE_PLANS[key]


@_on_device
def transformer(feat0, feat1, layer_structs, layer_names, nhead, mask0=None, mask1=None, inplace=False, prepared=None, mode=None,
                diag=None, skip_padded=False):
    mode = mode or COARSE_MODE
    if mode not in COARSE_MODES:
        raise ValueError(f"coarse transformer mode {mode!r} (mode= or LOFTR_COARSE_MODE): expected one of {', '.join(COARSE_MODES)}")
    _need(feat0, "feat0"); _need(feat1, "feat1")
    N, L, Cc = feat0.shape
    S = feat1.shape[1]
    m0, m1 = _mask_u8(mask0, "mask0"), _mask_u8(mask1, "mask1")
    if L == S:
        both = stacked_halves(feat0, feat1) if inplace and feat0.shape[0] == feat1.shape[0] else None
        if both is None:
            both = torch.cat([feat0, feat1], 0)
        f0, f1 = both[:N], both[N:]
        if m0 is not None:
            mb = torch.cat([m0, m1], 0)
            m0, m1 = mb[:N], mb[N:]
    else:
        f0, f1 = feat0.clone(), feat1.clone()
    n_layers = len(layer_names)
    arr = (LayerWeights * n_layers)(*layer_structs)
    kind_list = [{"self": 0, "cross": 1}[n] for n in layer_names]
    kinds = (C.c_int * n_layers)(*kind_list)
    lib = _lib.load()
    nbytes = lib.loftr_encoder_workspace_bytes(2 * N, L, S, Cc)
    ws = workspace(nbytes, feat0.device)
    skip_padded = bool(skip_padded) and m0 is not None
    if skip_padded:
        mode = "launches"
    if mode == "auto":
        mode = "persistent" if N >= COARSE_AUTO_MIN_PAIRS else "launches"
    plan = None
    if mode != "launches" and Cc == 256 and nhead == 8 and N > 0:
        order = 1 if mode == "persistent_call_order" else 0
        plan = coarse_plan(kind_list, N, L, S, feat0.device, order)
    if plan is not None:
        own = diag is None
        if own:
            key, (diag, host, done) = _status_word(feat0.device)
            diag.zero_()
        check(lib.loftr_transformer_fwd_planned(_ptr(f0), _ptr(f1), _ptr(m0), _ptr(m1), arr, kinds, n_layers, N, L, S, Cc, nhead,
                                                _ptr(prepared), prepared.numel() if prepared is not None else 0,
                                                _ptr(ws), ws.numel(), _ptr(plan), plan.numel(), order,
                                                _ptr(diag), diag.numel(), _stream()),
              "loftr_transformer_fwd_planned")
        if own:
            host.copy_(diag, non_blocking=True)
            done.record()
            _STATUS_PENDING[key] = (host, done)
    elif skip_padded:
        check(lib.loftr_transformer_fwd_padded(_ptr(f0), _ptr(f1), _ptr(m0), _ptr(m1), arr, kinds, n_layers, N, L, S, Cc, nhead,
                                               _ptr(prepared), prepared.numel() if prepared is not None else 0,
                                               _ptr(ws), ws.numel(), 1, _stream()), "loftr_transformer_fwd_padded")
    else:
        check(lib.loftr_transformer_fwd(_ptr(f0), _ptr(f1), _ptr(m0), _ptr(m1), arr, kinds, n_layers, N, L, S, Cc, nhead,
                                        _ptr(prepared), prepared.numel() if prepared is not None else 0,
                                        _ptr(ws), ws.numel(), _stream()), "loftr_transformer_fwd")
    return f0, f1


@_on_device
def coarse_match(feat_c0, feat_c1, hw0_c, hw1_c, thr, border_rm, scale, match_type="dual_softmax",
                 temperature=0.1, bin_score=None, skh_iters=3, skh_prefilter=False, mask0=None, mask1=None,
                 scale0=None, scale1=None, want_conf=True, want_assign=False):
    _need(feat_c0, "feat_c0"); _need(feat_c1, "feat_c1")
    N, L, Cc = feat_c0.shape
    S = feat_c1.shape[1]
    dev = feat_c0.device
    assert L == hw0_c[0] * hw0_c[1] and S == hw1_c[0] * hw1_c[1]
    m0, m1 = _mask_u8(mask0, "mask0"), _mask_u8(mask1, "mask1")
    s0 = None if scale0 is None else _need(scale0.to(torch.float32).contiguous(), "scale0")
    s1 = None if scale1 is None else _need(scale1.to(torch.float32).contiguous(), "scale1")
    cap = max(N * L, 1)
    b_ids = torch.empty(cap, dtype=torch.int64, device=dev)
    i_ids = torch.empty(cap, dtype=torch.int64, device=dev)
    j_ids = torch.empty(cap, dtype=torch.int64, device=dev)
    mconf = torch.empty(cap, dtype=torch.float32, device=dev)
    mk0 = torch.empty(cap, 2, dtype=torch.float32, device=dev)
    mk1 = torch.empty(cap, 2, dtype=torch.float32, device=dev)
    counts = torch.zeros(1 + N, dtype=torch.int32, device=dev)
    p = CoarseParams(N, hw0_c[0], hw0_c[1], hw1_c[0], hw1_c[1], Cc, float(thr), int(border_rm), float(scale),
                     m0.data_ptr() if m0 is not None else None, m1.data_ptr() if m1 is not None else None,
                     s0.data_ptr() if s0 is not None else None, s1.data_ptr() if s1 is not None else None)
    mo = MatchOut(b_ids.data_ptr(), i_ids.data_ptr(), j_ids.data_ptr(), mconf.data_ptr(), mk0.data_ptr(),
                  mk1.data_ptr(), counts.data_ptr())
    lib = _lib.load()
    ws = workspace(lib.loftr_coarse_match_workspace_bytes(N, L, S, Cc), dev)
    out = {}
    if match_type == "dual_softmax":
        conf = torch.empty(N, L, S, device=dev, dtype=torch.float32) if want_conf else None
        check(lib.loftr_coarse_match_dual_softmax(_ptr(feat_c0), _ptr(feat_c1), C.byref(p), float(temperature),
                                                  _ptr(conf), C.byref(mo), _ptr(ws), ws.numel(), _stream()),
              "loftr_coarse_match_dual_softmax")
    elif match_type == "sinkhorn":
        conf = torch.empty(N, L, S, device=dev, dtype=torch.float32)
        assign = torch.empty(N, L + 1, S + 1, device=dev, dtype=torch.float32) if want_assign else None
        check(lib.loftr_coarse_match_sinkhorn(_ptr(feat_c0), _ptr(feat_c1), C.byref(p), float(bin_score),
                                              int(skh_iters), int(bool(skh_prefilter)), _ptr(conf), _ptr(assign),
                                              C.byref(mo), _ptr(ws), ws.numel(), _stream()),
              "loftr_coarse_match_sinkhorn")
        if want_assign:
            out["conf_matrix_with_bin"] = assign
    else:
        raise NotImplementedError(match_type)
    M = int(counts[0].item()) if N > 0 else 0
    out.update(conf_matrix=conf, b_ids=b_ids[:M], i_ids=i_ids[:M], j_ids=j_ids[:M], mconf=mconf[:M],
               mkpts0_c=mk0[:M], mkpts1_c=mk1[:M], counts=counts)
    return out


def _fmap(t):
    sn, sc, sh, sw = t.stride()
    return FMap(t.data_ptr(), sn, sc, sh, sw, t.shape[2], t.shape[3])


@_on_device
def fine_preprocess(feat_f0, feat_f1, feat_c0, feat_c1, b_ids, i_ids, j_ids, hw0_c, hw1_c, W, stride,
                    down_w=None, down_b=None, merge_w=None, merge_b=None):
    for t, n in ((feat_f0, "feat_f0"), (feat_f1, "feat_f1")):
        if not t.is_cuda or t.dtype != torch.float32:
            raise _lib.LoftrHipError(f"{n}: expected a float32 GPU tensor")
    _need(feat_c0, "feat_c0"); _need(feat_c1, "feat_c1")
    M = b_ids.shape[0]
    Cf = feat_f0.shape[1]
    dev = feat_f0.device
    out = torch.empty(2 * M, W * W, Cf, device=dev, dtype=torch.float32)
    out0, out1 = out[:M], out[M:]
    if M == 0:
        return out0, out1
    lib = _lib.load()
    ws = workspace(lib.loftr_fine_preprocess_workspace_bytes(M, W, Cf), dev)
    f0, f1 = _fmap(feat_f0), _fmap(feat_f1)
    check(lib.loftr_fine_preprocess(C.byref(f0), C.byref(f1), _ptr(feat_c0), _ptr(feat_c1), feat_c0.shape[1],
                                    feat_c1.shape[1], feat_c0.shape[2], _ptr(_need(b_ids, "b_ids", torch.int64)),
                                    _ptr(_need(i_ids, "i_ids", torch.int64)), _ptr(_need(j_ids, "j_ids", torch.int64)),
                                    M, hw0_c[1], hw1_c[1], int(stride), int(W), Cf, _ptr(down_w), _ptr(down_b),
                                    _ptr(merge_w), _ptr(merge_b), _ptr(out0), _ptr(out1), _ptr(ws), ws.numel(),
                                    _stream()), "loftr_fine_preprocess")
    return out0, out1


WINDOW_HEAD_MAX_FILL = 1.8


def window_head_wins(M, dense_pixels):
    return 0 < 2 * M * 49 <= WINDOW_HEAD_MAX_FILL * dense_pixels


def window_head_supported(W, Cin, Cout, h_sp0, h_sp1):
    return (W == 5 and Cout == 128 and h_sp0.shape == h_sp1.shape and h_sp0.shape[3] == ceil32(Cin)
            and h_sp0.numel() < 2 ** 31)


def _window_head_common(h_sp0, h_sp1, Cin, conv, b_ids, i_ids, j_ids):
    for t, n in ((h_sp0, "h_sp0"), (h_sp1, "h_sp1")):
        if not t.is_cuda or t.dtype != torch.int32 or not t.is_contiguous() or t.dim() != 4:
            raise _lib.LoftrHipError(f"{n}: expected a contiguous int32 (SP) GPU tensor [N, H, W, Cp]")
    if h_sp0.shape != h_sp1.shape or h_sp0.shape[3] != ceil32(Cin):
        raise _lib.LoftrHipError(f"window head: SP maps {tuple(h_sp0.shape)} / {tuple(h_sp1.shape)} for {Cin} channels")
    Cout, Cin_w, KH, KW = conv.weight.shape
    if (Cin_w, KH, KW) != (Cin, 3, 3) or conv.stride[0] != 1 or conv.padding[0] != 1:
        raise _lib.LoftrHipError("window head: a 3x3 / stride-1 / pad-1 convolution expected")
    ids = [_ptr(_need(t, n, torch.int64)) for t, n in ((b_ids, "b_ids"), (i_ids, "i_ids"), (j_ids, "j_ids"))]
    return Cout, _prepared_conv(conv, None), ids


@_on_device
def window_head(h_sp0, h_sp1, Cin, conv, b_ids, i_ids, j_ids, hw0_c, hw1_c, W, stride):
    Cout, prepared, ids = _window_head_common(h_sp0, h_sp1, Cin, conv, b_ids, i_ids, j_ids)
    M = b_ids.shape[0]
    win = torch.empty(2, M, W * W, ceil32(Cout), dtype=torch.int32, device=h_sp0.device)
    if M:
        N, H, Wm, _ = h_sp0.shape
        check(_lib.load().loftr_window_head(_ptr(h_sp0), _ptr(h_sp1), N, H, Wm, Cin, _ptr(prepared), prepared.numel(), Cout, *ids,
                                            M, hw0_c[1], hw1_c[1], int(stride), int(W), _ptr(win[0]), _ptr(win[1]),
                                            _stream()), "loftr_window_head")
    return win[0], win[1]


@_on_device
def fine_preprocess_windows(h_sp0, h_sp1, Cin, conv, feat_c0, feat_c1, b_ids, i_ids, j_ids, hw0_c, hw1_c, W, stride,
                            down_w, down_b, merge_w, merge_b):
    Cf, prepared, ids = _window_head_common(h_sp0, h_sp1, Cin, conv, b_ids, i_ids, j_ids)
    _need(feat_c0, "feat_c0"); _need(feat_c1, "feat_c1")
    M = b_ids.shape[0]
    dev = h_sp0.device
    out = torch.empty(2 * M, W * W, Cf, device=dev, dtype=torch.float32)
    out0, out1 = out[:M], out[M:]
    if M == 0:
        return out0, out1
    lib = _lib.load()
    ws = workspace(lib.loftr_fine_preprocess_workspace_bytes(M, W, Cf), dev)
    N, H, Wm, _ = h_sp0.shape
    check(lib.loftr_fine_preprocess_window_head(_ptr(h_sp0), _ptr(h_sp1), N, H, Wm, Cin, _ptr(prepared), prepared.numel(),
                                                _ptr(feat_c0), _ptr(feat_c1), feat_c0.shape[1], feat_c1.shape[1], feat_c0.shape[2],
                                                *ids, M, hw0_c[1], hw1_c[1], int(stride), int(W), Cf, _ptr(down_w), _ptr(down_b),
                                                _ptr(merge_w), _ptr(merge_b), _ptr(out0), _ptr(out1), _ptr(ws), ws.numel(),
                                                _stream()), "loftr_fine_preprocess_window_head")
    return out0, out1


WINDOW_HEAD_FIRST_MAX_FILL = 0.85


def window_head_first_wins(M, dense_pixels):
    return window_head_wins(M, dense_pixels) and 2 * M * 49 <= WINDOW_HEAD_FIRST_MAX_FILL * dense_pixels


def window_head_first_supported(W, Cin, conv0, conv1, t_sp0, t_sp1, M):
    return (window_head_supported(W, Cin, conv1.out_channels, t_sp0, t_sp1) and Cin == 196 and conv0.out_channels == 196
            and conv1.in_channels == 196 and 2 * M * 49 * 224 < 2 ** 31)


def _window_head_first_common(t_sp0, t_sp1, Cin, conv, bn, b_ids, i_ids, j_ids):
    for t, n in ((t_sp0, "t_sp0"), (t_sp1, "t_sp1")):
        if not t.is_cuda or t.dtype != torch.int32 or not t.is_contiguous() or t.dim() != 4:
            raise _lib.LoftrHipError(f"{n}: expected a contiguous int32 (SP) GPU tensor [N, H, W, Cp]")
    if t_sp0.shape != t_sp1.shape or t_sp0.shape[3] != ceil32(Cin):
        raise _lib.LoftrHipError(f"window head: SP maps {tuple(t_sp0.shape)} / {tuple(t_sp1.shape)} for {Cin} channels")
    Cout, Cin_w, KH, KW = conv.weight.shape
    if (Cin_w, KH, KW) != (Cin, 3, 3) or conv.stride[0] != 1 or conv.padding[0] != 1:
        raise _lib.LoftrHipError("window head: a 3x3 / stride-1 / pad-1 convolution expected")
    ids = [_ptr(_need(t, n, torch.int64)) for t, n in ((b_ids, "b_ids"), (i_ids, "i_ids"), (j_ids, "j_ids"))]
    return Cout, _prepared_conv(conv, bn), ids


@_on_device
def window_head_first(t_sp0, t_sp1, Cin, conv, bn, b_ids, i_ids, j_ids, hw0_c, hw1_c, W, stride):
    Cout, prepared, ids = _window_head_first_common(t_sp0, t_sp1, Cin, conv, bn, b_ids, i_ids, j_ids)
    M = b_ids.shape[0]
    nb = torch.empty(2 * M, 49, ceil32(Cout), dtype=torch.int32, device=t_sp0.device)
    if M:
        N, H, Wm, _ = t_sp0.shape
        check(_lib.load().loftr_window_head_first(_ptr(t_sp0), _ptr(t_sp1), N, H, Wm, Cin, _ptr(prepared), prepared.numel(), Cout, *ids,
                                                  M, hw0_c[1], hw1_c[1], int(stride), int(W), _ptr(nb), _stream()),
              "loftr_window_head_first")
    return nb


@_on_device
def window_head_last(nb, hw_f, Cin, conv, b_ids, i_ids, j_ids, hw0_c, hw1_c, W, stride):
    M = b_ids.shape[0]
    if not nb.is_cuda or nb.dtype != torch.int32 or not nb.is_contiguous() or tuple(nb.shape) != (2 * M, 49, ceil32(Cin)):
        raise _lib.LoftrHipError(f"nb: expected a contiguous int32 (SP) GPU tensor [{2 * M}, 49, {ceil32(Cin)}]")
    Cout = conv.weight.shape[0]
    prepared = _prepared_conv(conv, None)
    ids = [_ptr(_need(t, n, torch.int64)) for t, n in ((b_ids, "b_ids"), (i_ids, "i_ids"), (j_ids, "j_ids"))]
    win = torch.empty(2, M, W * W, ceil32(Cout), dtype=torch.int32, device=nb.device)
    if M:
        check(_lib.load().loftr_window_head_last(_ptr(nb), int(hw_f[0]), int(hw_f[1]), Cin, _ptr(prepared), prepared.numel(), Cout, *ids,
                                                 M, hw0_c[1], hw1_c[1], int(stride), int(W), _ptr(win[0]), _ptr(win[1]), _stream()),
              "loftr_window_head_last")
    return win[0], win[1]


@_on_device
def fine_preprocess_windows2(t_sp0, t_sp1, Cin, conv0, bn0, conv1, feat_c0, feat_c1, b_ids, i_ids, j_ids, hw0_c, hw1_c, W, stride,
                             down_w, down_b, merge_w, merge_b):
    Cmid, prepared0, ids = _window_head_first_common(t_sp0, t_sp1, Cin, conv0, bn0, b_ids, i_ids, j_ids)
    Cf = conv1.weight.shape[0]
    if tuple(conv1.weight.shape[1:]) != (Cmid, 3, 3) or conv1.stride[0] != 1 or conv1.padding[0] != 1:
        raise _lib.LoftrHipError("window head: a 3x3 / stride-1 / pad-1 second convolution expected")
    prepared1 = _prepared_conv(conv1, None)
    _need(feat_c0, "feat_c0"); _need(feat_c1, "feat_c1")
    M = b_ids.shape[0]
    dev = t_sp0.device
    out = torch.empty(2 * M, W * W, Cf, device=dev, dtype=torch.float32)
    out0, out1 = out[:M], out[M:]
    if M == 0:
        return out0, out1
    lib = _lib.load()
    ws = workspace(lib.loftr_fine_preprocess_workspace_bytes(M, W, Cf), dev)
    nb = torch.empty(2 * M, 49, ceil32(Cmid), dtype=torch.int32, device=dev)
    N, H, Wm, _ = t_sp0.shape
    check(lib.loftr_fine_preprocess_window_head2(_ptr(t_sp0), _ptr(t_sp1), N, H, Wm, Cin, _ptr(prepared0), prepared0.numel(), Cmid,
                                                 _ptr(prepared1), prepared1.numel(),
                                                 _ptr(feat_c0), _ptr(feat_c1), feat_c0.shape[1], feat_c1.shape[1], feat_c0.shape[2],
                                                 *ids, M, hw0_c[1], hw1_c[1], int(stride), int(W), Cf, _ptr(down_w), _ptr(down_b),
                                                 _ptr(merge_w), _ptr(merge_b), _ptr(out0), _ptr(out1), _ptr(ws), ws.numel(),
                                                 _ptr(nb), _stream()), "loftr_fine_preprocess_window_head2")
    return out0, out1


def _slot_ids(ids, n_slots, name, device):
    host = ids.detach().cpu() if isinstance(ids, torch.Tensor) else torch.as_tensor(ids)
    if host.dim() != 1 or host.dtype.is_floating_point or host.dtype == torch.bool:
        raise _lib.LoftrHipError(f"{name}: expected a 1-D integer tensor of slot ids, got {tuple(host.shape)} {host.dtype}")
    if host.numel() and (int(host.min()) < 0 or int(host.max()) >= n_slots):
        raise _lib.LoftrHipError(f"{name}: slot id out of range [0, {n_slots}) (min {int(host.min())}, max {int(host.max())})")
    if isinstance(ids, torch.Tensor) and ids.is_cuda and ids.dtype == torch.int32 and ids.is_contiguous() and ids.device == device:
        return ids
    return host.to(torch.int32).to(device)


def _bank_map(bank, name):
    if not isinstance(bank, torch.Tensor) or not bank.is_cuda or bank.dtype != torch.float32 or bank.dim() != 4:
        raise _lib.LoftrHipError(f"{name}: expected a 4-D float32 GPU tensor [n_slots, C, H, W]")
    if bank.shape[0] == 0:
        raise _lib.LoftrHipError(f"{name}: empty bank")
    return bank


@_on_device
def pos_encode_flatten_gather(bank, slot_ids, pe, out=None):
    _bank_map(bank, "bank")
    _need(pe, "pe")
    n_slots, Cc, H, W = bank.shape
    ids = _slot_ids(slot_ids, n_slots, "slot_ids", bank.device)
    n = ids.shape[0]
    if out is None:
        out = torch.empty(n, H * W, Cc, device=bank.device, dtype=torch.float32)
    elif tuple(out.shape) != (n, H * W, Cc):
        raise _lib.LoftrHipError(f"out: expected shape {(n, H * W, Cc)}, got {tuple(out.shape)}")
    _need(out, "out")
    fm = _fmap(bank)
    check(_lib.load().loftr_pos_encode_flatten_gather(C.byref(fm), n_slots, _ptr(ids), n, _ptr(pe), pe.shape[-2], pe.shape[-1],
                                                      _ptr(out), Cc, _stream()), "loftr_pos_encode_flatten_gather")
    return out


@_on_device
def fine_preprocess_gather(bank_f0, slot0, bank_f1, slot1, feat_c0, feat_c1, b_ids, i_ids, j_ids, hw0_c, hw1_c, W, stride,
                           down_w=None, down_b=None, merge_w=None, merge_b=None):
    _bank_map(bank_f0, "bank_f0"); _bank_map(bank_f1, "bank_f1")
    _need(feat_c0, "feat_c0"); _need(feat_c1, "feat_c1")
    N = feat_c0.shape[0]
    s0 = _slot_ids(slot0, bank_f0.shape[0], "slot0", bank_f0.device)
    s1 = _slot_ids(slot1, bank_f1.shape[0], "slot1", bank_f1.device)
    if s0.shape[0] != N or s1.shape[0] != N:
        raise _lib.LoftrHipError(f"slot0 / slot1: expected {N} slot ids (one per pair), got {s0.shape[0]} / {s1.shape[0]}")
    M = b_ids.shape[0]
    Cf = bank_f0.shape[1]
    dev = bank_f0.device
    out = torch.empty(2 * M, W * W, Cf, device=dev, dtype=torch.float32)
    out0, out1 = out[:M], out[M:]
    if M == 0:
        return out0, out1
    lib = _lib.load()
    ws = workspace(lib.loftr_fine_preprocess_workspace_bytes(M, W, Cf), dev)
    f0, f1 = _fmap(bank_f0), _fmap(bank_f1)
    check(lib.loftr_fine_preprocess_gather(C.byref(f0), bank_f0.shape[0], _ptr(s0), C.byref(f1), bank_f1.shape[0], _ptr(s1),
                                           _ptr(feat_c0), _ptr(feat_c1), feat_c0.shape[1], feat_c1.shape[1], feat_c0.shape[2],
                                           _ptr(_need(b_ids, "b_ids", torch.int64)), _ptr(_need(i_ids, "i_ids", torch.int64)),
                                           _ptr(_need(j_ids, "j_ids", torch.int64)), M, hw0_c[1], hw1_c[1], int(stride), int(W), Cf,
                                           _ptr(down_w), _ptr(down_b), _ptr(merge_w), _ptr(merge_b), _ptr(out0), _ptr(out1),
                                           _ptr(ws), ws.numel(), _stream()), "loftr_fine_preprocess_gather")
    return out0, out1


@_on_device
def fine_preprocess_bwd(feat_f0, feat_f1, feat_c0, feat_c1, b_ids, i_ids, j_ids, hw0_c, hw1_c, W, stride, down_w, down_b, merge_w,
                        grad_out0, grad_out1):
    _need(feat_c0, "feat_c0"); _need(feat_c1, "feat_c1"); _need(grad_out0, "grad_out0"); _need(grad_out1, "grad_out1")
    M = b_ids.shape[0]
    Cf, Cc = feat_f0.shape[1], feat_c0.shape[2]
    dev = feat_f0.device
    gf0, gf1 = torch.zeros_like(feat_f0), torch.zeros_like(feat_f1)
    gc0, gc1 = torch.zeros_like(feat_c0), torch.zeros_like(feat_c1)
    gdw, gdb = torch.zeros_like(down_w), torch.zeros_like(down_b)
    gmw, gmb = torch.zeros(Cf, 2 * Cf, device=dev), torch.zeros(Cf, device=dev)
    if M == 0:
        return gf0, gf1, gc0, gc1, gdw, gdb, gmw, gmb
    lib = _lib.load()
# ... 874 lines not shown
```

Measured before the change: 457.2 image-pairs/s.

## Fuse positional encoding and flatten into persistent coarse transformer map reads

Adds a maps entry point so the persistent coarse transformer reads channels-last backbone maps directly and adds the positional encoding on the fly in the first-layer X and KV tile loads, instead of running a separate pos-encode/flatten pass and f32-to-split conversion jobs. This removes an extra full read/write of the coarse features and some launches. The half-stream backbone path is also reworked to avoid concatenating image0/image1 when halves are used. The trade-off is extra per-element PE loads inside the hot fragment-loading loop and more addressing arithmetic.

```diff
diff --git a/include/loftr_hip.h b/include/loftr_hip.h
--- a/include/loftr_hip.h
+++ b/include/loftr_hip.h
@@ -81,6 +81,12 @@
                                   int n_layers, int N, int L, int S, int C, int H, const void* prepared,
                                   size_t prepared_bytes, void* ws, size_t ws_bytes, const void* plan,
                                   size_t plan_bytes, int plan_order, void* diag, size_t diag_bytes, void* stream);
+int loftr_transformer_fwd_planned_maps(const loftr_fmap* map0, const loftr_fmap* map1, const float* pe, int pe_h, int pe_w,
+                                       float* feat0, float* feat1, const loftr_layer_weights* layers,
+                                       const int* layer_is_cross, int n_layers, int N, int C, int H,
+                                       const void* prepared, size_t prepared_bytes, void* ws, size_t ws_bytes,
+                                       const void* plan, size_t plan_bytes, int plan_order, void* diag, size_t diag_bytes,
+                                       void* stream);
 
 size_t loftr_transformer_prepared_bytes(int n_layers, int C);
 int loftr_transformer_prepare(const loftr_layer_weights* layers, int n_layers, int C, void* prepared,
diff --git a/loftr_amd/_lib.py b/loftr_amd/_lib.py
--- a/loftr_amd/_lib.py
+++ b/loftr_amd/_lib.py
@@ -67,6 +67,8 @@
     "loftr_coarse_plan_signature": (C.c_uint, [_i, _i, _i, _i, _i]),
     "loftr_transformer_fwd_planned": (_i, [_p, _p, _p, _p, C.POINTER(LayerWeights), C.POINTER(_i), _i, _i, _i, _i, _i, _i,
                                            _p, _sz, _p, _sz, _p, _sz, _i, _p, _sz, _p]),
+    "loftr_transformer_fwd_planned_maps": (_i, [C.POINTER(FMap), C.POINTER(FMap), _p, _i, _i, _p, _p, C.POINTER(LayerWeights), C.POINTER(_i),
+                                                _i, _i, _i, _i, _p, _sz, _p, _sz, _p, _sz, _i, _p, _sz, _p]),
     "loftr_hip_debug_set": (_i, [C.c_char_p, _i]),
     "loftr_hip_debug_get": (_i, [C.c_char_p, C.POINTER(_i), C.POINTER(_i)]),
     "loftr_transformer_prepared_bytes": (_sz, [_i, _i]),
diff --git a/loftr_amd/csrc/coarse_plan.h b/loftr_amd/csrc/coarse_plan.h
--- a/loftr_amd/csrc/coarse_plan.h
+++ b/loftr_amd/csrc/coarse_plan.h
@@ -56,9 +56,11 @@
   const sp_t *wq, *w0, *w2, *wkv;
   const float *wq_s, *w0_s, *w2_s, *wkv_s, *merge_f32, *g1, *b1, *g2, *b2;
 };
+struct PctMap { const float* data; long sn, sh, sw; int W; };
 struct PctLaunch {
   PctShape shape;
   float* f32[2]; sp_t* sp[2]; const uint8_t* mask[2];
+  PctMap map[2]; const float* pe; int pe_h, pe_w;
   PctLayerPtrs layer[PCT_MAX_LAYERS];
   const void* plan; size_t plan_bytes; unsigned plan_signature;
   void* ws; size_t ws_bytes;
diff --git a/loftr_amd/csrc/encoder_fused.hip b/loftr_amd/csrc/encoder_fused.hip
--- a/loftr_amd/csrc/encoder_fused.hip
+++ b/loftr_amd/csrc/encoder_fused.hip
@@ -24,6 +24,8 @@
 constexpr int LDS_BYTES = OFF_TAB + T_N * 4;
 static_assert(LDS_BYTES <= 160 * 1024, "one workgroup per CU");
 
+struct MapSrc { const float* map; long sn, sh, sw; const float* pe; long pe_plane; int W, pe_w; };
+struct MapTok { const float* xp; unsigned poff; };
 struct Args {
   const sp_t* x_sp; const float* x_f32;
   float* out_f32; sp_t* out_sp;
@@ -50,6 +52,31 @@
   sp_pack2(x0, x1, hi.x, lo.x);
   sp_pack2(x2, x3, hi.y, lo.y);
 }
+__device__ __forceinline__ MapTok map_token(const MapSrc& m, const int n, const int t) {
+  const int y = t / m.W, x = t - y * m.W;
+  return MapTok{m.map + (long)n * m.sn + (long)y * m.sh + (long)x * m.sw, (unsigned)(y * m.pe_w + x)};
+}
+__device__ __forceinline__ float map_pe(const MapSrc& m, const int c0, const unsigned poff) { return (m.pe + (long)c0 * m.pe_plane)[poff]; }
+__device__ __forceinline__ void map_frags(const MapSrc& m, const MapTok t, const int g, h16x8 (&xh)[16], h16x8 (&xl)[16]) {
+  const float* xp = t.xp + 8 * g;
+  const unsigned poff = t.poff + (unsigned)(8 * g) * (unsigned)m.pe_plane;
+#pragma unroll
+  for (int ks = 0; ks < 16; ++ks) {
+    if (ks == 8) __builtin_amdgcn_sched_barrier(0);
+    const f32x4 a = *reinterpret_cast<const f32x4*>(xp + 16 * ks), b = *reinterpret_cast<const f32x4*>(xp + 16 * ks + 4);
+    float v[8];
+#pragma unroll
+    for (int e = 0; e < 4; ++e) {
+      v[e] = a[e] + map_pe(m, 16 * ks + e, poff);
+      v[4 + e] = b[e] + map_pe(m, 16 * ks + 4 + e, poff);
+    }
+    uint2 H0, L0, H1, L1;
+    sp_pack4(v[0], v[1], v[2], v[3], H0, L0);
+    sp_pack4(v[4], v[5], v[6], v[7], H1, L1);
+    xh[ks] = __builtin_bit_cast(h16x8, u32x4{H0.x, H0.y, H1.x, H1.y});
+    xl[ks] = __builtin_bit_cast(h16x8, u32x4{L0.x, L0.y, L1.x, L1.y});
+  }
+}
 __device__ __forceinline__ void pack_panel(const float (&v)[16], h16x8 (&fh)[2], h16x8 (&fl)[2]) {
   if (!EFX_PROBE_EPI) {
     fh[0] = __builtin_bit_cast(h16x8, f32x4{v[0], v[1], v[2], v[3]}); fl[0] = __builtin_bit_cast(h16x8, f32x4{v[4], v[5], v[6], v[7]});
@@ -92,7 +119,8 @@
                                              const float (&mk)[16], const bool live, const int nlive);
 
 template <bool FOLD>
-__device__ __forceinline__ void encoder_x_body(const Args& a, const int seq, const int grp, char* const lds, const FoldArgs* fa = nullptr) {
+__device__ __forceinline__ void encoder_x_body(const Args& a, const int seq, const int grp, char* const lds, const FoldArgs* fa = nullptr,
+                                               const MapSrc* ms = nullptr) {
   const int lane = threadIdx.x & 63, wave = threadIdx.x >> 6, g = lane >> 5, li = lane & 31;
   const int T = a.T;
   if constexpr (!FOLD) {
@@ -116,7 +144,9 @@
     tab[T_G2 + f] = a.g2[f]; tab[T_B2 + f] = a.b2[f];
   }
   h16x8 xh[16], xl[16];
-  {
+  const bool from_map = FOLD && ms && ms->map != nullptr;
+  if (from_map) map_frags(*ms, map_token(*ms, seq, min(tok, T - 1)), g, xh, xl);
+  else {
     const u32x4* src = reinterpret_cast<const u32x4*>(a.x_sp + row * 256);
 #pragma unroll
     for (int ks = 0; ks < 16; ++ks) {
@@ -373,11 +403,22 @@
     const bool in_seq = tok < T;
     if (FOLD || in_seq) {
       const float* xr = a.x_f32 + row * 256;
+      unsigned poff = 0;
+      if (from_map) {
+        const MapTok t = map_token(*ms, seq, min(tok, T - 1));
+        xr = t.xp; poff = t.poff + (unsigned)fq * (unsigned)ms->pe_plane;
+      }
       float* of = a.out_f32 + row * 256;
       sp_t* os = a.out_sp + row * 256;
       f32x4 xn[4];
 #pragma unroll
       for (int q = 0; q < 4; ++q) xn[q] = *reinterpret_cast<const f32x4*>(xr + fq + 8 * q);
+      if (from_map) {
+#pragma unroll
+        for (int q = 0; q < 4; ++q)
+#pragma unroll
+          for (int e = 0; e < 4; ++e) xn[q][e] += map_pe(*ms, 8 * q + e, poff);
+      }
 #pragma unroll
       for (int j = 0; j < 8; ++j) {
         f32x4 xc[4];
@@ -386,6 +427,12 @@
         if (j + 1 < 8) {
 #pragma unroll
           for (int q = 0; q < 4; ++q) xn[q] = *reinterpret_cast<const f32x4*>(xr + 32 * (j + 1) + fq + 8 * q);
+          if (from_map) {
+#pragma unroll
+            for (int q = 0; q < 4; ++q)
+#pragma unroll
+              for (int e = 0; e < 4; ++e) xn[q][e] += map_pe(*ms, 32 * (j + 1) + 8 * q + e, poff);
+          }
         }
         float y[16];
 #pragma unroll
@@ -450,6 +497,7 @@
 struct PctCall { int layer, x_img, s_img, pad, fold[2], pad2[2]; };
 struct PctArgs {
   float* f32[2]; sp_t* sp[2]; const uint8_t* mask[2]; int T[2];
+  MapSrc map[3];
   int N, n_calls, n_items, splits;
   const PctItem* items; unsigned* cnt;
   float* part; float* kv; sp_t* pm;
@@ -462,14 +510,15 @@
 constexpr int OFF_RED = OFF_TAB + T_N * 4, RED_FLOATS = 33 * 32, OFF_CTRL = OFF_RED + W * RED_FLOATS * 4, LDS_BYTES_P = OFF_CTRL + 64;
 static_assert(LDS_BYTES_P <= 160 * 1024, "one workgroup per CU");
 
-__device__ __forceinline__ void kv_tile_body(const KvTile& a, const int tile, char* const lds) {
+__device__ __forceinline__ void kv_tile_body(const KvTile& a, const int tile, char* const lds, const MapSrc& ms, const int seq) {
   const int lane = threadIdx.x & 63, wave = threadIdx.x >> 6, g = lane >> 5, li = lane & 31;
   const int T = a.T;
   const int tok0 = (tile * W + wave) * PT;
   const bool live = tok0 < T;
   const int nlive = min(W, (T - tile * W * PT + PT - 1) / PT);
   h16x8 xh[16], xl[16];
-  {
+  if (ms.map) map_frags(ms, map_token(ms, seq, min(tok0 + li, T - 1)), g, xh, xl);
+  else {
     const u32x4* src = reinterpret_cast<const u32x4*>(a.x_sp + (long)min(tok0 + li, T - 1) * 256);
 #pragma unroll
     for (int ks = 0; ks < 16; ++ks) {
@@ -689,6 +738,7 @@
     const PctLayerPtrs& lw = P.layer[call.layer];
     const int Tx = P.T[call.x_img], Ts = P.T[call.s_img];
     const long cp = (long)c * P.N + pair;
+    const MapSrc& ms = P.map[c < 2 ? call.x_img : 2];
     if ((P.skip >> type) & 1) {
     } else if (type == PCT_X) {
       Args a;
@@ -712,14 +762,14 @@
         k.wkv = lf.wkv; k.wkv_s = lf.wkv_s; k.inv_s = 1.f / (float)Tx;
         k.part = P.part + (((long)cf * P.N + pair) * 8 * P.splits + idx) * (33 * 32); k.head_stride = (long)P.splits * (33 * 32);
       }
-      encoder_x_body<true>(a, pair, idx, lds, &fa);
+      encoder_x_body<true>(a, pair, idx, lds, &fa, &ms);
     } else if (type == PCT_K) {
       KvTile k;
       k.x_sp = P.sp[call.s_img] + (long)pair * Ts * 256;
       k.mask = P.mask[call.s_img] ? P.mask[call.s_img] + (long)pair * Ts : nullptr;
       k.T = Ts; k.wkv = lw.wkv; k.wkv_s = lw.wkv_s; k.inv_s = 1.f / (float)Ts;
       k.part = P.part + (cp * 8 * P.splits + idx) * (33 * 32); k.head_stride = (long)P.splits * (33 * 32);
-      kv_tile_body(k, idx, lds);
+      kv_tile_body(k, idx, lds, ms, pair);
     } else {
       kv_final_body(P.part + (cp * 8 + idx) * P.splits * (33 * 32), ceil_div(Ts, W * PT), P.kv + (cp * 8 + idx) * (33 * 32), lw.merge_f32, idx,
                     P.pm + cp * 65536, lds);
@@ -814,6 +864,17 @@
   a.pm = wa.take<sp_t>(cp * 65536);
   if (!wa.ok()) return LOFTR_ERR_WORKSPACE;
   for (int i = 0; i < 2; ++i) { a.f32[i] = p.f32[i]; a.sp[i] = p.sp[i]; a.mask[i] = p.mask[i]; a.T[i] = s.T[i]; }
+  if (p.map[0].data) {
+    if (!p.map[1].data || !p.pe || p.mask[0] || p.mask[1] || p.pe_h <= 0 || p.pe_w <= 0) return LOFTR_ERR_BAD_ARG;
+    if ((long)p.pe_h * p.pe_w > 0x7fffffffL / 256) return LOFTR_ERR_UNSUPPORTED;
+    for (int i = 0; i < 2; ++i) {
+      const PctMap& m = p.map[i];
+      if (m.W <= 0 || s.T[i] % m.W || m.W > p.pe_w || s.T[i] / m.W > p.pe_h) return LOFTR_ERR_BAD_ARG;
+      if (((size_t)m.data & 15) || (m.sn & 3) || (m.sh & 3) || (m.sw & 3)) return LOFTR_ERR_UNSUPPORTED;
+    }
+    for (int i = 0; i < 2; ++i)
+      a.map[i] = efx::MapSrc{p.map[i].data, p.map[i].sn, p.map[i].sh, p.map[i].sw, p.pe, (long)p.pe_h * p.pe_w, p.map[i].W, p.pe_w};
+  }
   a.N = s.N; a.n_calls = s.n_calls(); a.n_items = (int)s.n_items(); a.splits = s.gmax();
   a.items = reinterpret_cast<const PctItem*>(p.plan) + 1;
   a.trace = p.trace; a.status = p.status; a.signature = p.plan_signature;
diff --git a/loftr_amd/csrc/transformer.hip b/loftr_amd/csrc/transformer.hip
--- a/loftr_amd/csrc/transformer.hip
+++ b/loftr_amd/csrc/transformer.hip
@@ -277,7 +277,7 @@
                            const int* layer_is_cross, int n_layers, int N, int L, int S,
                            int C, int H, const void* prepared, size_t prepared_bytes, void* ws, size_t ws_bytes,
                            const void* plan, size_t plan_bytes, int plan_order, void* diag, size_t diag_bytes, void* stream,
-                           int skip_padded = 0) {
+                           int skip_padded = 0, const PctMap* maps = nullptr, const float* pe = nullptr, int pe_h = 0, int pe_w = 0) {
   LOFTR_CHECK_ARG(feat0 && feat1 && layers && layer_is_cross && n_layers >= 0 && N >= 0 && L > 0 && S > 0);
   LOFTR_CHECK_ARG((mask0 == nullptr) == (mask1 == nullptr));
   if (!((C == 256 || C == 128) && H == 8) || n_layers > MAX_LAYERS) return LOFTR_ERR_UNSUPPORTED;
@@ -301,7 +301,7 @@
     view_layers(layers, n_layers, C, reinterpret_cast<sp_t*>(const_cast<void*>(prepared)), lw);
     weights_ready = true;
   }
-  if (C == 128 && n_layers == 2 && !layer_is_cross[0] && layer_is_cross[1] && L == S && L <= 32 && !mask0) {
+  if (!maps && C == 128 && n_layers == 2 && !layer_is_cross[0] && layer_is_cross[1] && L == S && L <= 32 && !mask0) {
     if (!weights_ready) {
       SpJobs wj;
       if ((rc = convert_layers(layers, n_layers, C, w_sp, wj, lw, st))) return rc;
@@ -316,7 +316,10 @@
     }
     if ((rc = launch_fine_pair(fp, st)) != LOFTR_ERR_UNSUPPORTED) return rc;
   }
-  {
+  if (maps) {
+    SpJobs jobs;
+    if (!weights_ready && (rc = convert_layers(layers, n_layers, C, w_sp, jobs, lw, st))) return rc;
+  } else {
     SpJobs jobs;
     auto add = [&](const float* src, sp_t* dst, long rows) {
       const int i = jobs.n++;
@@ -336,6 +339,7 @@
       pl.shape = PctShape{n_layers, N, {L, S}};
       if (!pl.shape.ok()) return LOFTR_ERR_UNSUPPORTED;
       pl.f32[0] = feat0; pl.f32[1] = feat1; pl.sp[0] = sp0; pl.sp[1] = sp1; pl.mask[0] = mask0; pl.mask[1] = mask1;
+      if (maps) { pl.map[0] = maps[0]; pl.map[1] = maps[1]; pl.pe = pe; pl.pe_h = pe_h; pl.pe_w = pe_w; }
       for (int i = 0; i < n_layers; ++i) {
         const LayerSp& w = lw[i];
         pl.layer[i] = PctLayerPtrs{w.q, w.mlp0, w.mlp2, w.kv, w.q_s, w.mlp0_s, w.mlp2_s, w.kv_s, w.merge_f32, w.n1w, w.n1b, w.n2w, w.n2b};
@@ -349,6 +353,7 @@
       }
       return launch_coarse_persistent(pl, st);
     }
+    if (maps) return LOFTR_ERR_UNSUPPORTED;
     const bool sched_on = loftr_debug_value(LOFTR_DBG_ENCODER_SCHEDULE) != 0;
     if (sched_on && pattern) {
       rc = coarse_transformer_scheduled(feat0, feat1, sp0, sp1, mask0, mask1, lw, n_layers / 2, stacked, N, L, S, C, H, e, st, skip_padded);
@@ -398,6 +403,22 @@
   LOFTR_CHECK_ARG(plan != nullptr && (plan_order == 0 || plan_order == 1));
   return transformer_fwd(feat0, feat1, mask0, mask1, layers, layer_is_cross, n_layers, N, L, S, C, H, prepared, prepared_bytes, ws, ws_bytes,
                          plan, plan_bytes, plan_order, diag, diag_bytes, stream);
+}
+
+extern "C" int loftr_transformer_fwd_planned_maps(const loftr_fmap* map0, const loftr_fmap* map1, const float* pe, int pe_h, int pe_w,
+                                                  float* feat0, float* feat1, const loftr_layer_weights* layers,
+                                                  const int* layer_is_cross, int n_layers, int N, int C, int H,
+                                                  const void* prepared, size_t prepared_bytes, void* ws, size_t ws_bytes,
+                                                  const void* plan, size_t plan_bytes, int plan_order, void* diag, size_t diag_bytes,
+                                                  void* stream) {
+  LOFTR_CHECK_ARG(plan != nullptr && (plan_order == 0 || plan_order == 1));
+  LOFTR_CHECK_ARG(map0 && map1 && map0->data && map1->data && pe && map0->H > 0 && map0->W > 0 && map1->H > 0 && map1->W > 0);
+  LOFTR_CHECK_ARG(map0->H <= pe_h && map0->W <= pe_w && map1->H <= pe_h && map1->W <= pe_w);
+  if (C != 256 || n_layers <= 0 || map0->sc != 1 || map1->sc != 1) return LOFTR_ERR_UNSUPPORTED;
+  if ((long)map0->H * map0->W > 0x7fffffffL / 256 || (long)map1->H * map1->W > 0x7fffffffL / 256) return LOFTR_ERR_UNSUPPORTED;
+  const PctMap maps[2] = {{map0->data, map0->sn, map0->sh, map0->sw, map0->W}, {map1->data, map1->sn, map1->sh, map1->sw, map1->W}};
+  return transformer_fwd(feat0, feat1, nullptr, nullptr, layers, layer_is_cross, n_layers, N, map0->H * map0->W, map1->H * map1->W, C, H,
+                         prepared, prepared_bytes, ws, ws_bytes, plan, plan_bytes, plan_order, diag, diag_bytes, stream, 0, maps, pe, pe_h, pe_w);
 }
 
 extern "C" size_t loftr_linear_workspace_bytes(int M, int N, int K) {
diff --git a/loftr_amd/loftr.py b/loftr_amd/loftr.py
--- a/loftr_amd/loftr.py
+++ b/loftr_amd/loftr.py
@@ -127,6 +127,25 @@
         return ops.transformer(feat0.contiguous(), feat1.contiguous(), structs, self.layer_names, self.nhead,
                                mask0, mask1, inplace=inplace, prepared=self._prepared(structs, feat0.device), mode=mode,
                                skip_padded=skip_padded)
+
+    def maps_mode(self, map0, map1, mode=None):
+        if self.training or self.d_model != 256 or autograd.wants_grad(map0, map1):
+            return None
+        if any(n not in ("self", "cross") for n in self.layer_names):
+            return None
+        mode = ops.transformer_maps_mode(map0, map1, self.nhead, mode)
+        if mode is None:
+            return None
+        kinds = [int(n == "cross") for n in self.layer_names]
+        L, S = map0.shape[2] * map0.shape[3], map1.shape[2] * map1.shape[3]
+        if not ops.coarse_plan_exists(kinds, map0.shape[0], L, S):
+            return None
+        return mode
+
+    def forward_maps(self, map0, map1, pe, mode):
+        structs = [layer.weight_struct() for layer in self.layers]
+        return ops.transformer_maps(map0, map1, pe, structs, self.layer_names, self.nhead,
+                                    prepared=self._prepared(structs, map0.device), mode=mode)
 
     def _prepared(self, structs, device):
         if self.training or not str(device).startswith("cuda"):
@@ -372,6 +391,7 @@
         self.overlap_fine_branch = True
         self.skip_padded_tiles = True
         self.coarse_mode = None
+        self.coarse_from_maps = True
         self.fine_join_late = False
         self._side_stream = None
         self.backbone_halves = None
@@ -407,12 +427,15 @@
         assert not head_input or (use_hip and data["hw0_i"] == data["hw1_i"])
         hkw = dict(head_input=head_input) if head_input else {}
         if data["hw0_i"] == data["hw1_i"]:
-            x = cl(torch.cat([data["image0"], data["image1"]], dim=0))
-            cap = self._backbone_cap(x)
-            if use_hip and x.shape[0] > cap:
+            n_images = data["image0"].shape[0] + data["image1"].shape[0]
+            cap = self._backbone_cap(data["image0"])
+            halves = (use_hip and n_images <= cap and self.overlap_fine_branch
+                      and (data["bs"] >= 8 if self.backbone_halves is None else self.backbone_halves))
+            x = data["image0"] if halves else cl(torch.cat([data["image0"], data["image1"]], dim=0))
+            if use_hip and n_images > cap:
                 outs = [run(x[i:i + cap]) for i in range(0, x.shape[0], cap)]
                 feats_c, feats_f = torch.cat([o[0] for o in outs]), torch.cat([o[1] for o in outs])
-            elif use_hip and self.overlap_fine_branch and (data["bs"] >= 8 if self.backbone_halves is None else self.backbone_halves):
+            elif halves:
                 main = torch.cuda.current_stream(x.device)
                 self.backbone.prepare_hip()
                 if self._half_streams is None:
@@ -468,9 +491,14 @@
             data.update({"hw0_f": feat_f0.shape[1:3], "hw1_f": feat_f1.shape[1:3]})
         else:
             data.update({"hw0_f": feat_f0.shape[2:], "hw1_f": feat_f1.shape[2:]})
+        maps_mode = None
+        if self.coarse_from_maps and "mask0" not in data and not self.training and feat_c0.is_cuda:
+            maps_mode = self.loftr_coarse.maps_mode(feat_c0, feat_c1, self.coarse_mode)
         both = (ops.stacked_halves(feat_c0, feat_c1)
                 if feat_c0.shape == feat_c1.shape and not autograd.wants_grad(feat_c0, feat_c1) else None)
-        if both is not None:
+        if maps_mode is not None:
+            coarse = lambda: self.loftr_coarse.forward_maps(feat_c0, feat_c1, self.pos_encoding.pe[0], maps_mode)
+        elif both is not None:
             feat_c0, feat_c1 = self.pos_encoding(both).split(feat_c0.shape[0])
         else:
             feat_c0 = self.pos_encoding(feat_c0)
@@ -485,14 +513,17 @@
                                                                            self.fine_head, c0, c1, data)
         else:
             fine_pre = lambda c0, c1: self.fine_preprocess(feat_f0, feat_f1, c0, c1, data)
-        self._match_encoded(feat_c0, feat_c1, data, fine_pre)
-
-    def _match_encoded(self, feat_c0, feat_c1, data, fine_preprocess):
+        self._match_encoded(feat_c0, feat_c1, data, fine_pre, coarse=coarse if maps_mode is not None else None)
+
+    def _match_encoded(self, feat_c0, feat_c1, data, fine_preprocess, coarse=None):
         mask_c0 = mask_c1 = None
         if "mask0" in data:
             mask_c0, mask_c1 = data["mask0"].flatten(-2), data["mask1"].flatten(-2)
-        feat_c0, feat_c1 = self.loftr_coarse(feat_c0, feat_c1, mask_c0, mask_c1, inplace=True, mode=self.coarse_mode,
-                                             skip_padded=self.skip_padded_tiles and mask_c0 is not None)
+        if coarse is not None:
+            feat_c0, feat_c1 = coarse()
+        else:
+            feat_c0, feat_c1 = self.loftr_coarse(feat_c0, feat_c1, mask_c0, mask_c1, inplace=True, mode=self.coarse_mode,
+                                                 skip_padded=self.skip_padded_tiles and mask_c0 is not None)
         if not self.fine_join_late:
             self._join_fine(feat_c0.device)
         full = self.training and self.full_grads
diff --git a/loftr_amd/ops.py b/loftr_amd/ops.py
--- a/loftr_amd/ops.py
+++ b/loftr_amd/ops.py
@@ -241,6 +241,10 @@
     else:
         why = f"unknown status {v}"
     raise _lib.LoftrHipError(f"persistent coarse transformer (loftr_transformer_fwd_planned) failed: {why}")
+
+
+def coarse_plan_exists(kinds, N, L, S):
+    return _lib.load().loftr_coarse_plan_bytes((C.c_int * len(kinds))(*kinds), len(kinds), N, L, S) != 0
 
 
 def coarse_plan(kinds, N, L, S, device, order=0):
@@ -319,6 +323,64 @@
     return f0, f1
 
 
+def transformer_maps_mode(map0, map1, nhead, mode=None):
+    mode = mode or COARSE_MODE
+    if mode not in COARSE_MODES:
+        raise ValueError(f"coarse transformer mode {mode!r} (mode= or LOFTR_COARSE_MODE): expected one of {', '.join(COARSE_MODES)}")
+    if mode == "auto":
+        mode = "persistent" if map0.shape[0] >= COARSE_AUTO_MIN_PAIRS else "launches"
+    if mode == "launches" or nhead != 8 or map0.shape[0] != map1.shape[0] or map0.shape[0] == 0:
+        return None
+    for m in (map0, map1):
+        if (not m.is_cuda or m.dtype != torch.float32 or m.dim() != 4 or m.shape[1] != 256 or m.stride(1) != 1 or m.data_ptr() % 16
+                or any(st % 4 for st in (m.stride(0), m.stride(2), m.stride(3)))):
+            return None
+    return mode
+
+
+@_on_device
+def transformer_maps(map0, map1, pe, layer_structs, layer_names, nhead, prepared=None, mode="persistent", diag=None):
+    if mode not in ("persistent", "persistent_call_order"):
+        raise ValueError(f"transformer_maps: mode {mode!r}: only the persistent forms read maps")
+    if transformer_maps_mode(map0, map1, nhead, mode) is None:
+        raise _lib.LoftrHipError("transformer_maps: expected two channels-last float32 GPU maps [N,256,H,W] with 16-byte aligned tokens and 8 heads")
+    _need(pe, "pe")
+    N, Cc = map0.shape[:2]
+    L, S = map0.shape[2] * map0.shape[3], map1.shape[2] * map1.shape[3]
+    dev = map0.device
+    if L == S:
+        both = torch.empty(2 * N, L, Cc, device=dev, dtype=torch.float32)
+        f0, f1 = both[:N], both[N:]
+    else:
+        f0, f1 = (torch.empty(N, T, Cc, device=dev, dtype=torch.float32) for T in (L, S))
+    n_layers = len(layer_names)
+    arr = (LayerWeights * n_layers)(*layer_structs)
+    kind_list = [{"self": 0, "cross": 1}[n] for n in layer_names]
+    kinds = (C.c_int * n_layers)(*kind_list)
+    lib = _lib.load()
+    ws = workspace(lib.loftr_encoder_workspace_bytes(2 * N, L, S, Cc), dev)
+    order = 1 if mode == "persistent_call_order" else 0
+    plan = coarse_plan(kind_list, N, L, S, dev, order)
+    if plan is None:
+        raise _lib.LoftrHipError("transformer_maps: these layers / shapes have no persistent form")
+    own = diag is None
+    if own:
+        key, (diag, host, done) = _status_word(dev)
+        diag.zero_()
+    fm0, fm1 = _fmap(map0), _fmap(map1)
+    check(lib.loftr_transformer_fwd_planned_maps(C.byref(fm0), C.byref(fm1), _ptr(pe), pe.shape[-2], pe.shape[-1], _ptr(f0), _ptr(f1),
+                                                 arr, kinds, n_layers, N, Cc, nhead,
+                                                 _ptr(prepared), prepared.numel() if prepared is not None else 0,
+                                                 _ptr(ws), ws.numel(), _ptr(plan), plan.numel(), order,
+                                                 _ptr(diag), diag.numel(), _stream()),
+          "loftr_transformer_fwd_planned_maps")
+    if own:
+        host.copy_(diag, non_blocking=True)
+        done.record()
+        _STATUS_PENDING[key] = (host, done)
+    return f0, f1
+
+
 @_on_device
 def coarse_match(feat_c0, feat_c1, hw0_c, hw1_c, thr, border_rm, scale, match_type="dual_softmax",
                  temperature=0.1, bin_score=None, skh_iters=3, skh_prefilter=False, mask0=None, mask1=None,
```

Result: no change. 456.2 image-pairs/s (-0.2%).
